# zyj0021200/simpleImageCaptionZoo

Measured on AMD Instinct MI355X. Metric: captions/sec (SCST step), BUTDDetection COCO14-size vocab, higher is better.
Workload: dtype f32

## Files before the change

### include/icz.h

```cpp
#ifndef ICZ_H_
#define ICZ_H_
#include <stddef.h>
#include <stdint.h>

#ifdef __cplusplus
extern "C" {
#endif

typedef enum {
    ICZ_OK = 0,
    ICZ_ERR_INVALID = -1,
    ICZ_ERR_HIP = -2,
    ICZ_ERR_STATE = -3,
    ICZ_ERR_NOMEM = -4
} icz_status;

const char* icz_last_error(void);
const char* icz_version(void);

typedef struct icz_butd icz_butd_t;

typedef struct {
    int32_t R;
    int32_t D;
// ... 105 lines not shown
                       const icz_rng* rng, int32_t train, float* packed_logits_out, void* stream);
int icz_nic_xe_backward(icz_nic_t* h, float smoothing, const icz_nic_params* grads, float* dfeatures_out, float* loss_out,
                        float n_tokens_global, void* stream);
int icz_nic_set_norm_global(icz_nic_t* h, const float* norm_dev, void* stream);
int icz_nic_set_option(icz_nic_t* h, const char* name, int32_t value);
int icz_nic_set_scheduled_sampling(icz_nic_t* h, float ss_prob, const float* gate_uniforms, const float* draw_uniforms);
int icz_nic_beam_search(icz_nic_t* h, const float* features, int32_t n_img, int32_t beam, int32_t max_steps, float* seqs_out,
                        int32_t* lens_out, void* stream);
int icz_nic_beam_search_opts(icz_nic_t* h, const float* features, int32_t n_img, int32_t beam, int32_t max_steps,
                             const icz_beam_opts* opts, float* seqs_out, int32_t* lens_out, float* scores_out, void* stream);
int icz_nic_beam_search_diverse(icz_nic_t* h, const float* features, int32_t n_img, int32_t beam, int32_t max_steps,
                                const icz_beam_opts* opts, const icz_beam_diversity* div, float* seqs_out, int32_t* lens_out,
                                float* scores_out, void* stream);

typedef struct icz_aoa icz_aoa_t;
typedef struct { int32_t R, D, Hd, E, V, NH, max_rows, max_len; } icz_aoa_dims;
typedef struct {
    float *q_w, *q_b, *k_w, *k_b, *v_w, *v_b, *aoa_w, *aoa_b, *ln_g, *ln_b;
} icz_aoa_block;
typedef struct {
    float *proj_w, *proj_b;
    icz_aoa_block layer[6];
    float *ref_ln_g, *ref_ln_b;
    float *lstm_w_ih, *lstm_w_hh, *lstm_b_ih, *lstm_b_hh;
    icz_aoa_block dec;
    float* embed_weight;
    float *predict_v, *predict_g, *predict_b;
} icz_aoa_params;
typedef struct {
    uint64_t seed;
    const float* uniforms;
    const uint8_t *proj_mask, *ref_att_mask, *ref_aoa_mask, *ref_sc_mask, *emb_mask, *ctx_mask, *att_mask, *out_mask;
} icz_aoa_rng;
int icz_aoa_create(const icz_aoa_dims* dims, icz_aoa_t** out);
int icz_aoa_destroy(icz_aoa_t* h);
int icz_aoa_bind_params(icz_aoa_t* h, const icz_aoa_params* params);
int icz_aoa_refresh_weights(icz_aoa_t* h, void* stream);
int icz_aoa_set_regions(icz_aoa_t* h, int32_t regions, const int32_t* counts_dev, const int32_t* counts_host, int32_t n_img);
int icz_aoa_set_option(icz_aoa_t* h, const char* name, int32_t value);
int icz_aoa_refine(icz_aoa_t* h, const float* feats, int32_t B, float* refined_out, void* stream);
int icz_aoa_greedy(icz_aoa_t* h, const float* feats, int32_t B, int32_t max_len, int64_t* ids_out, void* stream);
int icz_aoa_beam_search(icz_aoa_t* h, const float* feats, int32_t n_img, int32_t beam, int32_t max_steps, float* seqs_out,
                        int32_t* lens_out, void* stream);
int icz_aoa_beam_search_opts(icz_aoa_t* h, const float* feats, int32_t n_img, int32_t beam, int32_t max_steps,
                             const icz_beam_opts* opts, float* seqs_out, int32_t* lens_out, float* scores_out, void* stream);
int icz_aoa_beam_search_diverse(icz_aoa_t* h, const float* feats, int32_t n_img, int32_t beam, int32_t max_steps,
                                const icz_beam_opts* opts, const icz_beam_diversity* div, float* seqs_out, int32_t* lens_out,
                                float* scores_out, void* stream);
int icz_aoa_sample(icz_aoa_t* h, const float* feats, int32_t B, int32_t max_len, const icz_aoa_rng* rng, int64_t* seq_out,
                   float* logprobs_out, void* stream);
int icz_aoa_scst_rollouts(icz_aoa_t* h, const float* feats, int32_t B, int32_t max_len, const icz_aoa_rng* rng, int64_t* ids_out,
                          int64_t* seq_out, float* logprobs_out, void* stream);
int icz_aoa_sample_backward(icz_aoa_t* h, const float* reward, const icz_aoa_params* grads, float* loss_out, float* mask_sum_out,
                            float mask_sum_global, void* stream);
int icz_aoa_xe_forward(icz_aoa_t* h, const float* feats, const int64_t* captions, int32_t B, int32_t L, const int32_t* lengths_host,
                       const icz_aoa_rng* rng, int32_t train, float* packed_logits_out, void* stream);
int icz_aoa_xe_backward(icz_aoa_t* h, float smoothing, const icz_aoa_params* grads, float* loss_out, float n_tokens_global,
                        void* stream);
int icz_aoa_set_norm_global(icz_aoa_t* h, const float* norm_dev, void* stream);
int icz_aoa_set_grad_callback(icz_aoa_t* h, icz_grad_ready_cb cb, void* user);
int icz_aoa_saved_alphas(icz_aoa_t* h, float* alphas_out, void* stream);
int icz_aoa_set_scheduled_sampling(icz_aoa_t* h, float ss_prob, const float* gate_uniforms, const float* draw_uniforms);

typedef struct icz_ensemble icz_ensemble_t;
int icz_ensemble_create(const int32_t* kinds, void* const* members, const float* weights, int32_t M, icz_ensemble_t** out);
int icz_ensemble_destroy(icz_ensemble_t* h);
int icz_ensemble_greedy(icz_ensemble_t* h, const float* const* feats, int32_t B, int32_t max_len, int64_t* ids_out, void* stream);
int icz_ensemble_beam_search_diverse(icz_ensemble_t* h, const float* const* feats, int32_t n_img, int32_t beam, int32_t max_steps,
                                     const icz_beam_opts* opts, const icz_beam_diversity* div, float* seqs_out, int32_t* lens_out,
                                     float* scores_out, void* stream);
int icz_ensemble_logprob(int32_t M, const float* const* logits, const float* const* bias, const int32_t* nsplit, const int32_t* ld,
                         const float* weights, int32_t rows, int32_t V, float* lp_out, int32_t ldo, int64_t* argmax_out, void* stream);

typedef struct {
    float temperature;
    int32_t top_k;
    float top_p;
} icz_sample_opts;
int icz_sample_decode_check(const icz_sample_opts* opts, int32_t n_img, int32_t n, int32_t V, int32_t max_rows);
int icz_butd_sample_decode(icz_butd_t* h, const float* feats, int32_t n_img, int32_t n, int32_t max_len, const icz_sample_opts* opts,
                           uint64_t seed, const float* uniforms, int64_t* ids_out, float* logp_out, float* score_out, void* stream);
int icz_aoa_sample_decode(icz_aoa_t* h, const float* feats, int32_t n_img, int32_t n, int32_t max_len, const icz_sample_opts* opts,
                          uint64_t seed, const float* uniforms, int64_t* ids_out, float* logp_out, float* score_out, void* stream);
int icz_nic_sample_decode(icz_nic_t* h, const float* features, int32_t n_img, int32_t n, int32_t max_len, const icz_sample_opts* opts,
                          uint64_t seed, const float* uniforms, int64_t* ids_out, float* logp_out, float* score_out, void* stream);
int icz_sample_filter_draw(const float* logits, const float* bias, int32_t nsplit, int32_t ld, int32_t rows, int32_t V,
                           const icz_sample_opts* opts, const float* uniforms, int64_t* tok_out, float* logp_out, uint8_t* keep_out,
                           void* stream);

int icz_adam_clamp_step(float* param, const float* grad, float* exp_avg, float* exp_avg_sq, int64_t n,
                        float lr, float clip, int32_t step, void* stream);
int icz_adam_clamp_multi(int32_t count, float* const* params, const float* const* grads, float* const* exp_avg,
                         float* const* exp_avg_sq, const int64_t* numel, float lr, float clip, int32_t step, void* stream);

typedef struct icz_ciderd icz_ciderd_t;

int icz_ciderd_create(const int32_t* df_keys, const double* df_idf, int64_t cap, double default_idf,
                      const double* penalty, icz_ciderd_t** out);
int icz_ciderd_destroy(icz_ciderd_t* h);

int icz_ciderd_reward(icz_ciderd_t* h, const int64_t* gen, const int64_t* greedy, int32_t B, int32_t T,
                      const int32_t* img_ref_ptr, const int32_t* ref_ent_ptr, const int32_t* ent_key,
                      const int32_t* ent_order, const double* ent_w, const double* ref_norm,
                      const int32_t* ref_len, float* reward_out, double* scores_out, void* stream);
int icz_ciderd_cook_host(const int32_t* df_keys_host, const double* df_idf_host, int64_t cap, double default_idf,
                         const int32_t* tokens, const int32_t* ref_tok_ptr, int32_t n_refs, int64_t max_ent,
                         int32_t* ent_key_out, int32_t* ent_order_out, double* ent_w_out, int32_t* ref_ent_ptr_out,
                         double* ref_norm_out, int32_t* ref_len_out, int64_t* n_ent_out);
typedef struct icz_ciderd_vocab icz_ciderd_vocab_t;
int icz_ciderd_vocab_create(const char* words, const int64_t* word_off, const int32_t* word_id, int32_t n_words, int32_t V,
                            icz_ciderd_vocab_t** out);
int icz_ciderd_vocab_destroy(icz_ciderd_vocab_t* v);
int icz_ciderd_vocab_oov_id(icz_ciderd_vocab_t* v, const char* word, int32_t len, int32_t* id_out);
int icz_ciderd_cook_text(icz_ciderd_vocab_t* vocab, const int32_t* df_keys_host, const double* df_idf_host, int64_t cap, double default_idf,
                         const char* text, int64_t text_len, int32_t n_refs, int64_t max_ent,
                         int32_t* ent_key_out, int32_t* ent_order_out, double* ent_w_out, int32_t* ref_ent_ptr_out,
                         double* ref_norm_out, int32_t* ref_len_out, int64_t* n_ent_out);
int icz_ciderd_reward_indexed(icz_ciderd_t* h, const int64_t* gen, const int64_t* greedy, int32_t B, int32_t T,
                              const int32_t* img_slot, const int32_t* img_ref_ptr, const int32_t* ref_ent_ptr,
                              const int32_t* ent_key, const int32_t* ent_order, const double* ent_w, const double* ref_norm,
                              const int32_t* ref_len, float* reward_out, double* scores_out, void* stream);
int icz_ciderd_reward_loo(icz_ciderd_t* h, const int64_t* gen, int32_t B, int32_t K, int32_t T, const int32_t* img_slot,
                          const int32_t* img_ref_ptr, const int32_t* ref_ent_ptr, const int32_t* ent_key, const int32_t* ent_order,
                          const double* ent_w, const double* ref_norm, const int32_t* ref_len, float* reward_out, double* scores_out,
                          void* stream);

int icz_ciderd_cook_device(icz_ciderd_t* h, const int32_t* tok, const int32_t* ptr, int32_t n_cand, int32_t* ent_key_out,
                           int32_t* ent_order_out, double* ent_w_out, int32_t* ent_ptr_out, double* norm_out, int32_t* len_out, void* stream);
size_t icz_ciderd_pairwise_workspace_bytes(int32_t n_img, int32_t K);
int icz_ciderd_pairwise(icz_ciderd_t* h, const int32_t* tok, const int32_t* ptr, int32_t n_img, int32_t K, double* pair_out,
                        double* consensus_out, int32_t* best_out, void* workspace, size_t workspace_bytes, void* stream);
int icz_ciderd_scores_csr(icz_ciderd_t* h, const int32_t* tok, const int32_t* ptr, int32_t n_img, int32_t K, const int32_t* img_slot,
                          const int32_t* img_ref_ptr, const int32_t* ref_ent_ptr, const int32_t* ent_key, const int32_t* ent_order,
                          const double* ent_w, const double* ref_norm, const int32_t* ref_len, double* scores_out, void* stream);
int icz_ngram_diversity(const int32_t* tok, const int32_t* ptr, int32_t n_img, int32_t K, int32_t* counts_out, void* stream);

int icz_bleu_stats(const int32_t* hyp_tok, const int32_t* hyp_ptr, const int32_t* ref_tok, const int32_t* ref_ptr,
                   const int32_t* img_ref_ptr, int32_t n_img, int32_t* stats_out, void* stream);
int icz_rouge_lcs(const int32_t* hyp_tok, const int32_t* hyp_ptr, const int32_t* ref_tok, const int32_t* ref_ptr,
                  const int32_t* img_ref_ptr, int32_t n_img, int32_t* lcs_out, void* stream);

int icz_gemm_f32(int32_t layout, const float* X, int32_t ldx, const float* W, int32_t ldw, const float* bias,
                 float* C, int32_t ldc, int32_t M, int32_t N, int32_t K, int32_t nsplit, float* workspace,
                 size_t workspace_floats, void* stream);
size_t icz_gemm_workspace_floats(int32_t M, int32_t N);
int icz_gemm_set_big_cfg(int32_t cfg);
int icz_gemm_big_cfg_for(int32_t layout, int32_t M, int32_t N, int32_t K, int32_t nsplit);
int icz_gemm_tn_grouped(const float* dY, int32_t ldy, int32_t M, int32_t K, int32_t ngroups, const float* const* X, const int32_t* ldx,
                        const int32_t* cols, float* const* out, const int32_t* ldo, const int32_t* rows_live, void* stream);
int icz_gemm_tn_split_pick(int32_t M, int32_t N, int32_t K);
int icz_gemm_tn_split(const float* dY, int32_t ldy, int32_t M, const float* X, int32_t ldx, int32_t N, int32_t K, float* out, int32_t ldo,
                      float* workspace, size_t workspace_floats, const int32_t* rows_live, void* stream);
int icz_gemm_route_for(int32_t layout, int32_t M, int32_t N, int32_t nseg, const int32_t* K, int32_t nsplit);
int icz_gemm_tn_grouped_fits(int32_t M, int32_t K, int32_t ngroups, const int32_t* cols);
int icz_prof_begin(void);
int icz_prof_select(int32_t which);
int icz_prof_pair_overhead(void* stream, int32_t n, double* avg_us);
int icz_prof_end(double* avg_us, double* bytes_per_launch, double* flops_per_launch, long long* launches);
int icz_kprof_begin(void);
int icz_kprof_end(int32_t group, double* avg_us, long long* pairs);
int icz_prof_stream_rate(const void* buf, size_t bytes, int32_t reps, void* stream, double* gbs);

#ifdef __cplusplus
}
#endif
#endif
```

### simpleimagecaptionzoo_amd/_lib.py

```python
import ctypes as C
import os

_HERE = os.path.dirname(os.path.abspath(__file__))
LIB_PATH = os.path.join(_HERE, "libicz.so")


class IczError(RuntimeError):
    pass


GRAD_READY_CB = C.CFUNCTYPE(None, C.c_void_p, C.c_int32)


class ButdDims(C.Structure):
    _fields_ = [(n, C.c_int32) for n in ("R", "D", "H", "E", "A", "V", "max_rows", "max_len")]


BUTD_PARAM_FIELDS = (
    "embed_weight",
    "td_w_ih", "td_w_hh", "td_b_ih", "td_b_hh",
    "lm_w_ih", "lm_w_hh", "lm_b_ih", "lm_b_hh",
    "enc_att_v", "enc_att_g", "enc_att_b",
    "dec_att_v", "dec_att_g", "dec_att_b",
    "affine_v", "affine_g", "affine_b",
# ... 42 lines not shown
    _fields_ = [("p%d" % i, C.c_void_p) for i in range(len(AOA_PARAM_KEYS))]


class AoaRng(C.Structure):
    _fields_ = [("seed", C.c_uint64), ("uniforms", C.c_void_p)] + [(n, C.c_void_p) for n in (
        "proj_mask", "ref_att_mask", "ref_aoa_mask", "ref_sc_mask", "emb_mask", "ctx_mask", "att_mask", "out_mask")]


class NicParams(C.Structure):
    _fields_ = [(n, C.c_void_p) for n in NIC_PARAM_FIELDS]


class ButdParams(C.Structure):
    _fields_ = [(n, C.c_void_p) for n in BUTD_PARAM_FIELDS]


class Rng(C.Structure):
    _fields_ = [("seed", C.c_uint64), ("uniforms", C.c_void_p), ("emb_mask", C.c_void_p),
                ("att_mask", C.c_void_p), ("out_mask", C.c_void_p)]


class BeamOpts(C.Structure):
    _fields_ = [("n_best", C.c_int32), ("block_ngram", C.c_int32), ("lp_kind", C.c_int32), ("lp_alpha", C.c_float)]


class BeamDiversity(C.Structure):
    _fields_ = [("groups", C.c_int32), ("diversity", C.c_float)]


class SampleOpts(C.Structure):
    _fields_ = [("temperature", C.c_float), ("top_k", C.c_int32), ("top_p", C.c_float)]


_lib = None


def lib():
    global _lib
    if _lib is not None:
        return _lib
    if not os.path.exists(LIB_PATH):
        raise IczError("libicz.so not found at %s -- the HIP extension is required (no fallback); run "
                       "__graft_entry__.build()" % LIB_PATH)
    import torch
    L = C.CDLL(LIB_PATH)
    vp, i32, i64, f32 = C.c_void_p, C.c_int32, C.c_int64, C.c_float
    sig = {
        "icz_last_error": (C.c_char_p, []),
        "icz_version": (C.c_char_p, []),
        "icz_butd_create": (C.c_int, [C.POINTER(ButdDims), C.POINTER(vp)]),
        "icz_butd_destroy": (C.c_int, [vp]),
        "icz_butd_bind_params": (C.c_int, [vp, C.POINTER(ButdParams)]),
        "icz_butd_set_option": (C.c_int, [vp, C.c_char_p, i32]),
        "icz_butd_set_grad_callback": (C.c_int, [vp, GRAD_READY_CB, vp]),
        "icz_aoa_set_grad_callback": (C.c_int, [vp, GRAD_READY_CB, vp]),
        "icz_butd_set_mask_sum_global": (C.c_int, [vp, vp, vp]),
        "icz_butd_refresh_weights": (C.c_int, [vp, vp]),
        "icz_butd_greedy": (C.c_int, [vp, vp, i32, i32, vp, vp, vp]),
        "icz_butd_step": (C.c_int, [vp, vp, i32, vp, vp, vp, vp, vp, vp, vp, vp, vp]),
        "icz_butd_sample": (C.c_int, [vp, vp, i32, i32, C.POINTER(Rng), vp, vp, vp]),
        "icz_butd_scst_rollouts": (C.c_int, [vp, vp, i32, i32, C.POINTER(Rng), vp, vp, vp, vp]),
        "icz_butd_sample_n": (C.c_int, [vp, vp, i32, i32, i32, C.POINTER(Rng), vp, vp, vp]),
        "icz_butd_sample_backward": (C.c_int, [vp, vp, C.POINTER(ButdParams), vp, vp, f32, vp]),
        "icz_butd_sample_backward_dlogp": (C.c_int, [vp, vp, C.POINTER(ButdParams), vp]),
        "icz_butd_xe_backward_dlogits": (C.c_int, [vp, vp, C.POINTER(ButdParams), vp]),
        "icz_butd_beam_search": (C.c_int, [vp, vp, i32, i32, i32, vp, vp, vp]),
        "icz_butd_beam_search_opts": (C.c_int, [vp, vp, i32, i32, i32, C.POINTER(BeamOpts), vp, vp, vp, vp]),
        "icz_butd_beam_search_diverse": (C.c_int, [vp, vp, i32, i32, i32, C.POINTER(BeamOpts), C.POINTER(BeamDiversity), vp, vp, vp, vp]),
        "icz_butd_sample_mask_sum": (C.c_int, [vp, vp, vp]),
        "icz_butd_xe_forward": (C.c_int, [vp, vp, vp, i32, i32, C.POINTER(i32), C.POINTER(Rng), i32, vp, vp]),
        "icz_butd_xe_backward": (C.c_int, [vp, f32, C.POINTER(ButdParams), vp, f32, vp]),
        "icz_butd_set_scheduled_sampling": (C.c_int, [vp, f32, vp, vp]),
        "icz_nic_set_scheduled_sampling": (C.c_int, [vp, f32, vp, vp]),
        "icz_aoa_set_scheduled_sampling": (C.c_int, [vp, f32, vp, vp]),
        "icz_adam_clamp_step": (C.c_int, [vp, vp, vp, vp, i64, f32, f32, i32, vp]),
        "icz_nic_create": (C.c_int, [C.POINTER(NicDims), C.POINTER(vp)]),
        "icz_nic_destroy": (C.c_int, [vp]),
        "icz_nic_bind_params": (C.c_int, [vp, C.POINTER(NicParams)]),
        "icz_nic_refresh_weights": (C.c_int, [vp, vp]),
        "icz_nic_greedy": (C.c_int, [vp, vp, i32, i32, vp, vp]),
        "icz_nic_sample": (C.c_int, [vp, vp, i32, i32, C.POINTER(Rng), vp, vp, vp]),
        "icz_nic_sample_backward": (C.c_int, [vp, vp, C.POINTER(NicParams), vp, vp, vp, f32, vp]),
        "icz_nic_xe_forward": (C.c_int, [vp, vp, vp, i32, i32, C.POINTER(i32), C.POINTER(Rng), i32, vp, vp]),
        "icz_nic_xe_backward": (C.c_int, [vp, f32, C.POINTER(NicParams), vp, vp, f32, vp]),
        "icz_butd_saved_alphas": (C.c_int, [vp, vp, vp]),
        "icz_aoa_saved_alphas": (C.c_int, [vp, vp, vp]),
        "icz_nic_set_norm_global": (C.c_int, [vp, vp, vp]),
        "icz_aoa_set_norm_global": (C.c_int, [vp, vp, vp]),
        "icz_nic_beam_search": (C.c_int, [vp, vp, i32, i32, i32, vp, vp, vp]),
        "icz_nic_beam_search_opts": (C.c_int, [vp, vp, i32, i32, i32, C.POINTER(BeamOpts), vp, vp, vp, vp]),
        "icz_nic_beam_search_diverse": (C.c_int, [vp, vp, i32, i32, i32, C.POINTER(BeamOpts), C.POINTER(BeamDiversity), vp, vp, vp, vp]),
        "icz_aoa_create": (C.c_int, [C.POINTER(AoaDims), C.POINTER(vp)]),
        "icz_aoa_destroy": (C.c_int, [vp]),
        "icz_aoa_bind_params": (C.c_int, [vp, C.POINTER(AoaParams)]),
        "icz_aoa_refresh_weights": (C.c_int, [vp, vp]),
        "icz_aoa_set_regions": (C.c_int, [vp, i32, vp, vp, i32]),
        "icz_aoa_set_option": (C.c_int, [vp, C.c_char_p, i32]),
        "icz_nic_set_option": (C.c_int, [vp, C.c_char_p, i32]),
        "icz_aoa_refine": (C.c_int, [vp, vp, i32, vp, vp]),
        "icz_aoa_greedy": (C.c_int, [vp, vp, i32, i32, vp, vp]),
        "icz_aoa_beam_search": (C.c_int, [vp, vp, i32, i32, i32, vp, vp, vp]),
        "icz_aoa_beam_search_opts": (C.c_int, [vp, vp, i32, i32, i32, C.POINTER(BeamOpts), vp, vp, vp, vp]),
        "icz_aoa_beam_search_diverse": (C.c_int, [vp, vp, i32, i32, i32, C.POINTER(BeamOpts), C.POINTER(BeamDiversity), vp, vp, vp, vp]),
        "icz_ensemble_create": (C.c_int, [C.POINTER(i32), C.POINTER(vp), C.POINTER(f32), i32, C.POINTER(vp)]),
        "icz_ensemble_destroy": (C.c_int, [vp]),
        "icz_ensemble_greedy": (C.c_int, [vp, C.POINTER(vp), i32, i32, vp, vp]),
        "icz_ensemble_beam_search_diverse": (C.c_int, [vp, C.POINTER(vp), i32, i32, i32, C.POINTER(BeamOpts), C.POINTER(BeamDiversity), vp, vp,
                                                       vp, vp]),
        "icz_ensemble_logprob": (C.c_int, [i32, C.POINTER(vp), C.POINTER(vp), C.POINTER(i32), C.POINTER(i32), C.POINTER(f32), i32, i32, vp, i32,
                                           vp, vp]),
        "icz_sample_decode_check": (C.c_int, [C.POINTER(SampleOpts), i32, i32, i32, i32]),
        "icz_butd_sample_decode": (C.c_int, [vp, vp, i32, i32, i32, C.POINTER(SampleOpts), C.c_uint64, vp, vp, vp, vp, vp]),
        "icz_aoa_sample_decode": (C.c_int, [vp, vp, i32, i32, i32, C.POINTER(SampleOpts), C.c_uint64, vp, vp, vp, vp, vp]),
        "icz_nic_sample_decode": (C.c_int, [vp, vp, i32, i32, i32, C.POINTER(SampleOpts), C.c_uint64, vp, vp, vp, vp, vp]),
        "icz_sample_filter_draw": (C.c_int, [vp, vp, i32, i32, i32, i32, C.POINTER(SampleOpts), vp, vp, vp, vp, vp]),
        "icz_aoa_sample": (C.c_int, [vp, vp, i32, i32, C.POINTER(AoaRng), vp, vp, vp]),
        "icz_aoa_scst_rollouts": (C.c_int, [vp, vp, i32, i32, C.POINTER(AoaRng), vp, vp, vp, vp]),
        "icz_aoa_sample_backward": (C.c_int, [vp, vp, C.POINTER(AoaParams), vp, vp, f32, vp]),
        "icz_aoa_xe_forward": (C.c_int, [vp, vp, vp, i32, i32, C.POINTER(i32), C.POINTER(AoaRng), i32, vp, vp]),
        "icz_aoa_xe_backward": (C.c_int, [vp, f32, C.POINTER(AoaParams), vp, f32, vp]),
        "icz_ciderd_create": (C.c_int, [vp, vp, i64, C.c_double, vp, C.POINTER(vp)]),
        "icz_ciderd_destroy": (C.c_int, [vp]),
        "icz_ciderd_reward": (C.c_int, [vp, vp, vp, i32, i32, vp, vp, vp, vp, vp, vp, vp, vp, vp, vp]),
        "icz_ciderd_cook_host": (C.c_int, [vp, vp, i64, C.c_double, vp, vp, i32, i64, vp, vp, vp, vp, vp, vp, C.POINTER(i64)]),
        "icz_ciderd_vocab_create": (C.c_int, [C.c_char_p, vp, vp, i32, i32, C.POINTER(vp)]),
        "icz_ciderd_vocab_destroy": (C.c_int, [vp]),
        "icz_ciderd_vocab_oov_id": (C.c_int, [vp, C.c_char_p, i32, C.POINTER(i32)]),
        "icz_ciderd_cook_text": (C.c_int, [vp, vp, vp, i64, C.c_double, C.c_char_p, i64, i32, i64, vp, vp, vp, vp, vp, vp, C.POINTER(i64)]),
        "icz_ciderd_reward_indexed": (C.c_int, [vp, vp, vp, i32, i32, vp, vp, vp, vp, vp, vp, vp, vp, vp, vp, vp]),
        "icz_ciderd_reward_loo": (C.c_int, [vp, vp, i32, i32, i32, vp, vp, vp, vp, vp, vp, vp, vp, vp, vp, vp]),
        "icz_ciderd_cook_device": (C.c_int, [vp, vp, vp, i32, vp, vp, vp, vp, vp, vp, vp]),
        "icz_ciderd_pairwise_workspace_bytes": (C.c_size_t, [i32, i32]),
        "icz_ciderd_pairwise": (C.c_int, [vp, vp, vp, i32, i32, vp, vp, vp, vp, C.c_size_t, vp]),
        "icz_ciderd_scores_csr": (C.c_int, [vp, vp, vp, i32, i32, vp, vp, vp, vp, vp, vp, vp, vp, vp, vp]),
        "icz_ngram_diversity": (C.c_int, [vp, vp, i32, i32, vp, vp]),
        "icz_bleu_stats": (C.c_int, [vp, vp, vp, vp, vp, i32, vp, vp]),
        "icz_rouge_lcs": (C.c_int, [vp, vp, vp, vp, vp, i32, vp, vp]),
        "icz_prof_begin": (C.c_int, []),
        "icz_prof_select": (C.c_int, [i32]),
        "icz_prof_pair_overhead": (C.c_int, [vp, i32, C.POINTER(C.c_double)]),
        "icz_prof_end": (C.c_int, [C.POINTER(C.c_double), C.POINTER(C.c_double), C.POINTER(C.c_double), C.POINTER(C.c_longlong)]),
        "icz_kprof_begin": (C.c_int, []),
        "icz_kprof_end": (C.c_int, [i32, C.POINTER(C.c_double), C.POINTER(C.c_longlong)]),
        "icz_prof_stream_rate": (C.c_int, [vp, C.c_size_t, i32, vp, C.POINTER(C.c_double)]),
        "icz_adam_clamp_multi": (C.c_int, [i32, C.POINTER(vp), C.POINTER(vp), C.POINTER(vp), C.POINTER(vp), C.POINTER(i64), f32, f32, i32, vp]),
        "icz_gemm_f32": (C.c_int, [i32, vp, i32, vp, i32, vp, vp, i32, i32, i32, i32, i32, vp, C.c_size_t, vp]),
        "icz_gemm_workspace_floats": (C.c_size_t, [i32, i32]),
        "icz_gemm_set_big_cfg": (C.c_int, [i32]),
        "icz_gemm_big_cfg_for": (C.c_int, [i32, i32, i32, i32, i32]),
        "icz_gemm_tn_grouped": (C.c_int, [vp, i32, i32, i32, i32, vp, vp, vp, vp, vp, vp, vp]),
        "icz_gemm_tn_split_pick": (C.c_int, [i32, i32, i32]),
        "icz_gemm_tn_split": (C.c_int, [vp, i32, i32, vp, i32, i32, i32, vp, i32, vp, C.c_size_t, vp, vp]),
        "icz_gemm_route_for": (C.c_int, [i32, i32, i32, i32, vp, i32]),
        "icz_gemm_tn_grouped_fits": (C.c_int, [i32, i32, i32, vp]),
    }
    for name, (res, args) in sig.items():
        try:
            fn = getattr(L, name)
        except AttributeError as e:
            raise IczError("libicz.so lacks symbol %s (stale build?)" % name) from e
        fn.restype, fn.argtypes = res, args
    _lib = L
    return L


def check(status):
    if status != 0:
        raise IczError("libicz status %d: %s" % (status, lib().icz_last_error().decode()))


def ptr(t):
    return None if t is None else C.c_void_p(t.data_ptr())


def stream_ptr():
    import torch
    return C.c_void_p(torch.cuda.current_stream().cuda_stream)
```

### simpleimagecaptionzoo_amd/csrc/butd.hip

```cpp
#include <vector>

#include "butd_impl.h"

namespace icz {

int Butd::init(const icz_butd_dims& d) {
    dims = d;
    ICZ_REQUIRE(d.R > 0 && d.R <= 64, "butd: R=%d must be in 1..64 (36 boxes / 49 grid cells)", d.R);
    ICZ_REQUIRE(d.D % 4 == 0 && d.H % 4 == 0 && d.E % 4 == 0 && d.A % 4 == 0, "butd: D,H,E,A must be multiples of 4");
    ICZ_REQUIRE(d.V > 3 && d.max_rows > 0 && d.max_len > 0, "butd: bad V/max_rows/max_len");
    const size_t rows = d.max_rows, H = d.H, D = d.D, E = d.E, A = d.A, V = d.V, R = d.R;
    ICZ_TRY(alloc((void**)&w_enc, sizeof(float) * A * D));
    ICZ_TRY(alloc((void**)&w_dec, sizeof(float) * A * H));
    ICZ_TRY(alloc((void**)&w_aff, sizeof(float) * A));
    const size_t Vp = pad_vocab(d.V);
    ICZ_TRY(alloc((void**)&w_pred, sizeof(float) * Vp * H));
    ICZ_TRY(alloc((void**)&n_enc, sizeof(float) * A));
    ICZ_TRY(alloc((void**)&n_dec, sizeof(float) * A));
    ICZ_TRY(alloc((void**)&n_aff, sizeof(float) * 4));
    ICZ_TRY(alloc((void**)&n_pred, sizeof(float) * V));
    ICZ_TRY(alloc((void**)&mean, sizeof(float) * rows * D));
    ICZ_TRY(alloc((void**)&premean, sizeof(float) * rows * 4 * H));
    ICZ_TRY(alloc((void**)&enc_ctx, sizeof(float) * rows * R * A));
    for (int i = 0; i < 2; ++i) {
        ICZ_TRY(alloc((void**)&h1[i], sizeof(float) * rows * H));
        ICZ_TRY(alloc((void**)&c1[i], sizeof(float) * rows * H));
        ICZ_TRY(alloc((void**)&h2[i], sizeof(float) * rows * H));
        ICZ_TRY(alloc((void**)&c2[i], sizeof(float) * rows * H));
    }
    ICZ_TRY(alloc((void**)&emb, sizeof(float) * rows * E));
    ICZ_TRY(alloc((void**)&ctx, sizeof(float) * rows * D));
    ICZ_TRY(alloc((void**)&scores, sizeof(float) * rows * R));
    ICZ_TRY(alloc((void**)&alpha, sizeof(float) * rows * R));
    ICZ_TRY(alloc((void**)&h2drop, sizeof(float) * rows * H));
    ICZ_TRY(alloc((void**)&logits, sizeof(float) * rows * Vp));
    ICZ_TRY(alloc((void**)&amax_val, sizeof(float) * rows * ARGMAX_PARTS));
    ICZ_TRY(alloc((void**)&amax_idx, sizeof(int) * rows * ARGMAX_PARTS));
    ICZ_TRY(alloc((void**)&it, sizeof(int64_t) * rows));
    ICZ_TRY(alloc_scalars(mem));
    size_t nmax = 4 * H;
    if (A > nmax) nmax = A;
    if (V > nmax) nmax = V;
    ws_floats = (size_t)TARGET_WGS * 4096 * 2 + rows * nmax;
    {
        const size_t kmax = 2 * H + (E > D ? E : D), r128 = rows < 128 ? rows : 128;
        const size_t need = (kmax / 256 + 1) * r128 * 4 * H;
        if (need > ws_floats) ws_floats = need;
    }
    ICZ_TRY(alloc((void**)&ws, sizeof(float) * ws_floats));
    ICZ_TRY(mem.synced());
    if (const char* e = getenv("ICZ_EARLY_OUT")) early_out = atoi(e) != 0;
    if (const char* e = getenv("ICZ_MERGE_SMALL")) { const int n = atoi(e); if (n >= 0 && n <= 32) merge_small = n; }
    return ICZ_OK;
}

int Butd::refresh(hipStream_t st) {
    ICZ_REQUIRE(bound, "butd: parameters not bound");
    const int A = dims.A, D = dims.D, H = dims.H, V = dims.V;
    WeightNormTable wt = {};
    int nb = 0;
    auto add = [&](const float* v, const float* g, float* w, float* norm, int rows, int cols) {
        wt.j[wt.count++] = {v, g, w, norm, rows, cols, nb};
        nb += cdiv(rows, 4);
    };
    add(P.enc_att_v, P.enc_att_g, w_enc, n_enc, A, D);
    add(P.dec_att_v, P.dec_att_g, w_dec, n_dec, A, H);
    add(P.affine_v, P.affine_g, w_aff, n_aff, 1, A);
    add(P.predict_v, P.predict_g, w_pred, n_pred, V, H);
    hipLaunchKernelGGL(weight_norm_multi_kernel, dim3(nb), dim3(256), 0, st, wt);
    ICZ_CHECK_HIP(hipGetLastError());
    fresh = true;
    wt_fresh = false;
    return ICZ_OK;
}

bool Butd::wt_possible() const {
    GemmArgs g = {};
    g.nseg = 1;
    g.seg[0] = {w_enc, w_enc, 4 * dims.H, 4 * dims.H, 4 * dims.H, nullptr};
    g.M = 64; g.N = dims.D + dims.H;
    GemmArgs p = g, q = g;
    p.N = q.N = dims.H;
    p.nseg = 2; p.seg[1] = p.seg[0];
    return dims.H % 64 == 0 && dims.D % 64 == 0 && gemm_resident_x3_fits(g) && gemm_resident_x3_pair_fits(p, q);
}

int Butd::refresh_transposes(hipStream_t st) {
    ICZ_REQUIRE(bound && wt_lm_ih, "butd: no transposed weight buffers");
    const int H = dims.H, D = dims.D, E = dims.E;
    TransposeTable tt = {};
    int nb = 0;
    auto add = [&](const float* src, int ld, int cols, float* dst) {
        tt.j[tt.count++] = {src, ld, 4 * H, cols, dst, nb};
        nb += (4 * H / 64) * (cols / 64);
    };
    add(P.lm_w_ih, D + H, D + H, wt_lm_ih);
    add(P.lm_w_hh, H, H, wt_lm_hh);
    add(P.td_w_ih, H + D + E, H, wt_td_ih_h2);
    add(P.td_w_hh, H, H, wt_td_hh);
    hipLaunchKernelGGL(transpose_multi_kernel, dim3(nb), dim3(256), 0, st, tt);
    ICZ_CHECK_HIP(hipGetLastError());
    wt_fresh = true;
    return ICZ_OK;
}

int Butd::gemm_nt(GemmArgs& g, int* nsplit_out, hipStream_t st) {
    g.nsplit = gemm_fit_split(GEMM_NT, g, gemm_pick_split(g, TARGET_WGS), ws_floats);
    if (g.nsplit > 1) {
        ICZ_REQUIRE(gemm_slab_floats(g.M, g.N, g.nsplit) <= ws_floats, "butd: workspace too small for %dx%dx%d slabs", g.nsplit, g.M, g.N);
        g.out = ws;
        g.bias = nullptr;
    }
    *nsplit_out = g.nsplit;
    return gemm_f32(GEMM_NT, g, st);
}

int Butd::prologue(const float* feats, int n_img, hipStream_t st) {
    const int R = dims.R, D = dims.D, H = dims.H, E = dims.E, A = dims.A;
    ICZ_REQUIRE(fresh, "butd: call icz_butd_refresh_weights after binding/updating parameters");
    ICZ_REQUIRE(n_img > 0 && n_img <= dims.max_rows, "butd: %d images exceed capacity %d", n_img, dims.max_rows);
    hipLaunchKernelGGL(mean_feats_kernel, dim3(cdiv(D, 1024), n_img), dim3(256), 0, st, feats, mean, R, D);
    {
        GemmArgs g = {};
        g.nseg = 1;
        g.seg[0] = {mean, P.td_w_ih + H, D, H + D + E, D, nullptr};
        g.M = n_img; g.N = 4 * H; g.out = premean; g.ldo = 4 * H;
        int ns;
        ICZ_TRY(gemm_nt(g, &ns, st));
        if (ns > 1) {
            size_t MN = (size_t)n_img * 4 * H;
            hipLaunchKernelGGL(slab_reduce_kernel, dim3(cdiv((int)(MN / 4), 256)), dim3(256), 0, st, ws, ns, MN, 4 * H, (const float*)nullptr, premean);
        }
    }
    {
        GemmArgs g = {};
        g.nseg = 1;
        g.seg[0] = {feats, w_enc, D, D, D, nullptr};
        g.M = n_img * R; g.N = A; g.out = enc_ctx; g.ldo = A; g.bias = P.enc_att_b;
        int ns;
        const float* bias = g.bias;
        ICZ_TRY(gemm_nt(g, &ns, st));
        if (ns > 1) {
            size_t MN = (size_t)n_img * R * A;
            hipLaunchKernelGGL(slab_reduce_kernel, dim3(cdiv((int)(MN / 4), 256)), dim3(256), 0, st, ws, ns, MN, A, bias, enc_ctx);
        }
    }
    ICZ_CHECK_HIP(hipGetLastError());
    return ICZ_OK;
}

int Butd::step(const StepIO& s, hipStream_t st) {
    const int R = dims.R, D = dims.D, H = dims.H, E = dims.E, A = dims.A, V = dims.V;
    const int Vp = pad_vocab(V);
    const int rows = s.rows;
    float* const ws = s.ws_alt ? s.ws_alt : this->ws;
    float* const scores = s.scores_alt ? s.scores_alt : this->scores;
    DropCfg off = {0, nullptr, nullptr, 0, 0};
    if (!s.emb_ready)
        hipLaunchKernelGGL(embed_kernel, dim3(cdiv(E, 1024), rows), dim3(256), 0, st, P.embed_weight, s.it, s.emb_out ? s.emb_out : emb, rows, E, s.drop_emb);
    const float* embp = s.emb_out ? s.emb_out : emb;
    int ns;
    {
        GemmArgs g = {};
        g.nseg = 3;
        g.seg[0] = {s.h2_in, P.td_w_ih, H, H + D + E, H, nullptr};
        g.seg[1] = {embp, P.td_w_ih + H + D, E, H + D + E, E, nullptr};
        g.seg[2] = {s.h1_in, P.td_w_hh, H, H, H, nullptr};
        g.M = rows; g.N = 4 * H; g.out = ws; g.ldo = 4 * H;
        g.live = s.live;
        const size_t ws_cap = s.ws_alt ? (tb.xfloats < ws_floats ? tb.xfloats : ws_floats) : ws_floats;
        g.nsplit = gemm_fit_split(GEMM_NT, g, gemm_pick_split(g, STEP_WGS), ws_cap);
        ns = g.nsplit;
        ICZ_REQUIRE(gemm_slab_floats(rows, 4 * H, ns) <= ws_cap && (size_t)rows * 4 * H <= ws_cap, "butd: workspace too small");
        if (ns == 1) { g.out = ws; }
        ICZ_TRY(gemm_f32(GEMM_NT, g, st));
        LstmPointArgs a = {ws, ns, premean, s.img_of_row, P.td_b_ih, P.td_b_hh, s.c1_in, s.h1_out, s.c1_out, s.gates_td_out, nullptr, rows, H, s.live};
        kprof_mark(KP_LSTM_POINT, true, st);
        launch_lstm_point(a, off, st);
        kprof_mark(KP_LSTM_POINT, false, st);
    }
    {
        kprof_mark(KP_ATTENTION, true, st);
        GemmArgs g = {};
        g.nseg = 1;
        g.seg[0] = {s.h1_out, w_dec, H, H, H, nullptr};
        g.M = rows; g.N = A; g.out = ws; g.ldo = A;
        g.live = s.live;
        g.nsplit = gemm_pick_split(g, STEP_WGS);
        ns = g.nsplit;
        ICZ_TRY(gemm_f32(GEMM_NT, g, st));
        AttScoreArgs a = {enc_ctx, s.img_of_row, ws, ns, P.dec_att_b, w_aff, P.affine_b, s.dec_ctx_out, scores, rows, R, A, s.live};
        const int G = s.rows_per_img;
        const bool grouped = G > 1 && G <= ATT_CTX_MAX_G && rows % G == 0 && sizeof(float) * A * G <= 60 * 1024;
        if (grouped && s.drop_att.mode == 0 && !s.live)
            hipLaunchKernelGGL(att_scores_group_kernel, dim3(rows / G, ATT_PARTS), dim3(256), sizeof(float) * A * G, st, a, G);
        else if (grouped)
            hipLaunchKernelGGL(att_scores_group_train_kernel, dim3(rows / G, ATT_PARTS), dim3(256), sizeof(float) * A * G, st, a, s.drop_att, G);
        else
            hipLaunchKernelGGL(att_scores_kernel, dim3(rows, ATT_PARTS), dim3(256), sizeof(float) * A, st, a, s.drop_att);
        if (G > 1 && G <= ATT_CTX_MAX_G && rows % G == 0 && !s.alpha_out2)
            hipLaunchKernelGGL(att_ctx_group_kernel, dim3(rows / G, cdiv(D, 512)), dim3(256), 0, st, s.feats, (const float*)scores,
                               s.alpha_out ? s.alpha_out : alpha, s.ctx_out ? s.ctx_out : ctx, R, D, G, s.live);
        else
            hipLaunchKernelGGL(att_ctx_kernel, dim3(rows, cdiv(D, 512)), dim3(256), 0, st, s.feats, s.img_of_row, (const float*)scores,
                               s.alpha_out ? s.alpha_out : alpha, s.alpha_out2, s.alpha2_stride, s.ctx_out ? s.ctx_out : ctx, R, D, s.live);
        kprof_mark(KP_ATTENTION, false, st);
    }
    const float* ctxp = s.ctx_out ? s.ctx_out : ctx;
    {
        GemmArgs g = {};
        g.nseg = 3;
        g.seg[0] = {ctxp, P.lm_w_ih, D, D + H, D, nullptr};
        g.seg[1] = {s.h1_out, P.lm_w_ih + D, H, D + H, H, nullptr};
        g.seg[2] = {s.h2_in, P.lm_w_hh, H, H, H, nullptr};
        g.M = rows; g.N = 4 * H; g.out = ws; g.ldo = 4 * H;
        g.live = s.live;
        const size_t ws_cap = s.ws_alt ? (tb.xfloats < ws_floats ? tb.xfloats : ws_floats) : ws_floats;
        g.nsplit = gemm_fit_split(GEMM_NT, g, gemm_pick_split(g, STEP_WGS), ws_cap);
        ns = g.nsplit;
        ICZ_REQUIRE(gemm_slab_floats(rows, 4 * H, ns) <= ws_cap && (size_t)rows * 4 * H <= ws_cap, "butd: workspace too small");
        ICZ_TRY(gemm_f32(GEMM_NT, g, st));
        LstmPointArgs a = {ws, ns, nullptr, nullptr, P.lm_b_ih, P.lm_b_hh, s.c2_in, s.h2_out, s.c2_out, s.gates_lm_out,
                           s.h2drop_out ? s.h2drop_out : h2drop, rows, H, s.live};
        launch_lstm_point(a, s.drop_out, st);
    }
    if (!s.skip_predict) {
        const size_t ws_cap = s.ws_alt ? (tb.xfloats < ws_floats ? tb.xfloats : ws_floats) : ws_floats;
        ICZ_TRY(gemm_predict(s.h2drop_out ? s.h2drop_out : h2drop, H, w_pred, P.predict_b, rows, V, Vp, s.logits_out ? s.logits_out : logits,
                             s.logits_ld ? s.logits_ld : Vp, ws, ws_cap, s.pred_nsplit, st, s.live));
    }
    ICZ_CHECK_HIP(hipGetLastError());
    return ICZ_OK;
}

int Butd::zero_state(int rows, int which, hipStream_t st) {
    ZeroList z = {{h1[which], c1[which], h2[which], c2[which]}, 4};
    const size_t n = (size_t)rows * dims.H;
    hipLaunchKernelGGL(zero_bufs_kernel, dim3(cdiv((int)(n / 4), 256)), dim3(256), 0, st, z, n);
    return ICZ_OK;
}

int Butd::greedy(const float* feats, int B, int max_len, int64_t* ids_out, float* alphas_out, hipStream_t st) {
    ICZ_REQUIRE(feats && ids_out && B > 0 && B <= dims.max_rows && max_len > 0, "butd greedy: bad arguments");
    ICZ_REQUIRE(fresh, "butd: call icz_butd_refresh_weights after binding/updating parameters");
    if (!use_graphs) return greedy_impl(feats, B, max_len, ids_out, alphas_out, st);
    const std::vector<uintptr_t> key = {1, (uintptr_t)feats, (uintptr_t)B, (uintptr_t)max_len, (uintptr_t)ids_out, (uintptr_t)alphas_out, opt_bits()};
    return gc.run(key, st, [&](hipStream_t s) { return greedy_impl(feats, B, max_len, ids_out, alphas_out, s); });
}

int Butd::greedy_impl(const float* feats, int B, int max_len, int64_t* ids_out, float* alphas_out, hipStream_t st) {
    ICZ_TRY(prologue(feats, B, st));
    return greedy_chain(feats, B, max_len, ids_out, alphas_out, st);
}

int Butd::greedy_chain(const float* feats, int B, int max_len, int64_t* ids_out, float* alphas_out, hipStream_t st, bool scst) {
    ICZ_TRY(zero_state(B, 0, st));
    int* const gn = (scst && early_out && gnunf && tb.T >= max_len && tb.B >= B) ? gnunf : nullptr;
    hipLaunchKernelGGL(greedy_init_kernel, dim3(cdiv(B > max_len ? B : max_len, 256)), dim3(256), 0, st, it, B, gn, max_len);
    int cur = 0;
    const int Vp = pad_vocab(dims.V);
    bool track = false;
    for (int t = 0; t < max_len; ++t) {
        StepIO s = {};
        s.rows = B; s.feats = feats; s.it = it;
        s.emb_ready = t > 0;
        s.h1_in = h1[cur]; s.c1_in = c1[cur]; s.h2_in = h2[cur]; s.c2_in = c2[cur];
        s.h1_out = h1[cur ^ 1]; s.c1_out = c1[cur ^ 1]; s.h2_out = h2[cur ^ 1]; s.c2_out = c2[cur ^ 1];
        if (alphas_out) { s.alpha_out2 = alphas_out + (size_t)t * dims.R; s.alpha2_stride = max_len * dims.R; }
        int pns = 1;
        s.pred_nsplit = &pns;
        if (track && t > 0) s.live = gn + (t - 1);
        ICZ_TRY(step(s, st));
        if (t == 0) track = gn && pns > 1;
        kprof_mark(KP_GREEDY_SELECT, true, st);
        launch_greedy_select(logits_view(ws, P.predict_b, logits, B, Vp, pns), emb_slot(), B, dims.V, amax_val, amax_idx, it, ids_out, max_len, t,
                             track ? gunf : nullptr, track ? gn : nullptr, st);
        kprof_mark(KP_GREEDY_SELECT, false, st);
        cur ^= 1;
    }
    ICZ_CHECK_HIP(hipGetLastError());
    return ICZ_OK;
}

int Butd::prologue(const float* feats, int n_img, int k, const int32_t*, hipStream_t st) {
    ICZ_TRY(prologue(feats, n_img, st));
    seam_feats = feats;
    return zero_state(n_img * k, 0, st);
}

int Butd::step(int rows, const int64_t* it_, const int32_t* img_of_row, int rows_per_img, int cur, bool slabs, LogitsView* out,
               hipStream_t st) {
    StepIO s = {};
    s.rows = rows; s.feats = seam_feats; s.img_of_row = img_of_row; s.it = it_;
    s.rows_per_img = rows_per_img;
    s.emb_ready = seam_emb_ready; s.live = seam_live;
    s.h1_in = h1[cur]; s.c1_in = c1[cur]; s.h2_in = h2[cur]; s.c2_in = c2[cur];
    s.h1_out = h1[cur ^ 1]; s.c1_out = c1[cur ^ 1]; s.h2_out = h2[cur ^ 1]; s.c2_out = c2[cur ^ 1];
    int pns = 1;
    if (slabs) s.pred_nsplit = &pns;
    ICZ_TRY(step(s, st));
    if (out) *out = logits_view(ws, P.predict_b, logits, rows, pad_vocab(dims.V), pns);
    return ICZ_OK;
}

void Butd::gather(const int32_t* src_row, int rows, int fan, hipStream_t st) {
    hipLaunchKernelGGL(beam_gather_kernel, dim3(cdiv(dims.H, 1024), rows), dim3(256), 0, st, src_row, dims.H, h1[1], c1[1], h2[1], c2[1],
                       h1[0], c1[0], h2[0], c2[0], fan);
}

DecodeMember* butd_member(void* handle) { return static_cast<DecodeMember*>(reinterpret_cast<Butd*>(handle)); }

}

using namespace icz;

extern "C" {

int icz_butd_create(const icz_butd_dims* dims, icz_butd_t** out) { return abi_create<Butd>("icz_butd_create", dims, out); }

int icz_butd_destroy(icz_butd_t* h) {
    delete reinterpret_cast<Butd*>(h);
    return ICZ_OK;
}

int icz_butd_bind_params(icz_butd_t* h, const icz_butd_params* p) {
    ICZ_REQUIRE(h && p, "icz_butd_bind_params: null argument");
    ICZ_TRY(check_param_table("icz_butd_bind_params", p, sizeof(*p), (1u << 16) | (1u << 17)));
    Butd* b = reinterpret_cast<Butd*>(h);
    if (b->bound && memcmp(&b->P, p, sizeof(*p)) != 0) {
        ICZ_CHECK_HIP(hipDeviceSynchronize());
        b->gc.clear();
    }
    b->P = *p;
    b->bound = true;
    b->fresh = false;
    return ICZ_OK;
}

int icz_butd_set_option(icz_butd_t* h, const char* name, int32_t value) {
    ICZ_REQUIRE(h && name, "icz_butd_set_option: null argument");
    Butd* b = reinterpret_cast<Butd*>(h);
    if (strcmp(name, "graphs") == 0) { b->use_graphs = value != 0; return ICZ_OK; }
    if (strcmp(name, "concurrent") == 0) { b->concurrent = value != 0; return ICZ_OK; }
    if (strcmp(name, "early_out") == 0) { b->early_out = value != 0; return ICZ_OK; }
    if (strcmp(name, "small_nt") == 0) { b->small_nt = value != 0; return ICZ_OK; }
    if (strcmp(name, "group_att") == 0) { b->group_att = value != 0; return ICZ_OK; }
    if (strcmp(name, "merge_small") == 0) {
        ICZ_REQUIRE(value >= 0 && value <= 32, "icz_butd_set_option: merge_small %d outside 0..32", value);
        b->merge_small = value;
        return ICZ_OK;
    }
    set_error("icz_butd_set_option: unknown option '%s'", name);
// ... 48 lines not shown
```

### simpleimagecaptionzoo_amd/csrc/butd_kernels.h

```cpp
#pragma once
#include <stdlib.h>

#include "icz_common.h"
#include "rng.h"

namespace icz {
namespace {

__global__ __launch_bounds__(256) void weight_norm_kernel(const float* __restrict__ v, const float* __restrict__ g,
                                                          float* __restrict__ w, float* __restrict__ norm,
                                                          int rows, int cols) {
    const int lane = threadIdx.x & 63;
    const int row = blockIdx.x * 4 + (threadIdx.x >> 6);
    if (row >= rows) return;
    const float* vr = v + (size_t)row * cols;
    float ss = 0.f;
    for (int c = lane * 4; c < cols; c += 256) {
        f32x4 x = *reinterpret_cast<const f32x4*>(vr + c);
        ss += x[0] * x[0] + x[1] * x[1] + x[2] * x[2] + x[3] * x[3];
    }
    ss = wave_sum(ss);
    const float nrm = sqrtf(ss);
    const float s = g[row] / nrm;
    float* wr = w + (size_t)row * cols;
    for (int c = lane * 4; c < cols; c += 256) {
        f32x4 x = *reinterpret_cast<const f32x4*>(vr + c);
        *reinterpret_cast<f32x4*>(wr + c) = x * s;
    }
    if (lane == 0) norm[row] = nrm;
}

struct WeightNormJob { const float* v; const float* g; float* w; float* norm; int rows, cols, block0; };
struct WeightNormTable { WeightNormJob j[4]; int count; };
__global__ __launch_bounds__(256) void weight_norm_multi_kernel(WeightNormTable tab) {
    int k = 0;
#pragma unroll 1
    for (int i = 1; i < tab.count; ++i)
        if ((int)blockIdx.x >= tab.j[i].block0) k = i;
    const WeightNormJob& jb = tab.j[k];
    const int lane = threadIdx.x & 63;
    const int row = ((int)blockIdx.x - jb.block0) * 4 + (threadIdx.x >> 6);
    if (row >= jb.rows) return;
    const float* vr = jb.v + (size_t)row * jb.cols;
    float ss = 0.f;
    for (int c = lane * 4; c < jb.cols; c += 256) {
        f32x4 x = *reinterpret_cast<const f32x4*>(vr + c);
        ss += x[0] * x[0] + x[1] * x[1] + x[2] * x[2] + x[3] * x[3];
    }
    ss = wave_sum(ss);
    const float nrm = sqrtf(ss);
    const float s = jb.g[row] / nrm;
    float* wr = jb.w + (size_t)row * jb.cols;
    for (int c = lane * 4; c < jb.cols; c += 256) {
        f32x4 x = *reinterpret_cast<const f32x4*>(vr + c);
        *reinterpret_cast<f32x4*>(wr + c) = x * s;
    }
    if (lane == 0) jb.norm[row] = nrm;
}

__global__ __launch_bounds__(256) void mean_feats_kernel(const float* __restrict__ feats, float* __restrict__ mean,
                                                         int R, int D) {
    const int b = blockIdx.y;
    const int d = (blockIdx.x * 256 + threadIdx.x) * 4;
    if (d >= D) return;
    const float* f = feats + (size_t)b * R * D + d;
    f32x4 s = {0.f, 0.f, 0.f, 0.f};
    for (int r = 0; r < R; ++r) s += *reinterpret_cast<const f32x4*>(f + (size_t)r * D);
    const float fr = (float)R;
    f32x4 o = {s[0] / fr, s[1] / fr, s[2] / fr, s[3] / fr};
    *reinterpret_cast<f32x4*>(mean + (size_t)b * D + d) = o;
}

__global__ __launch_bounds__(256) void slab_reduce_kernel(const float* __restrict__ slab, int nsplit, size_t MN, int N,
                                                          const float* __restrict__ bias, float* __restrict__ out) {
    size_t i = ((size_t)blockIdx.x * 256 + threadIdx.x) * 4;
    if (i >= MN) return;
    f32x4 s = *reinterpret_cast<const f32x4*>(slab + i);
    for (int z = 1; z < nsplit; ++z) s += *reinterpret_cast<const f32x4*>(slab + (size_t)z * MN + i);
    if (bias) {
        int n = (int)(i % N);
        s += *reinterpret_cast<const f32x4*>(bias + n);
    }
    *reinterpret_cast<f32x4*>(out + i) = s;
}

__global__ __launch_bounds__(256) void embed_kernel(const float* __restrict__ table, const int64_t* __restrict__ it,
                                                    float* __restrict__ emb, int rows, int E, DropCfg dc, int relu = 1,
                                                    const int* __restrict__ live = nullptr) {
    if (step_dead(live)) return;
    const int row = blockIdx.y;
    const int e = (blockIdx.x * 256 + threadIdx.x) * 4;
    if (e >= E) return;
    f32x4 x = *reinterpret_cast<const f32x4*>(table + (size_t)it[row] * E + e);
    const int drow = row - dc.row0;
    if (drow < 0) dc.mode = 0;
    uint32_t k = dc.mode ? dc.keep4((uint64_t)drow * E + e) : 0xFu;
    const float sc = dc.mode ? 2.0f : 1.0f;
#pragma unroll
    for (int j = 0; j < 4; ++j) x[j] = ((k >> j) & 1u) ? (relu ? fmaxf(x[j], 0.f) : x[j]) * sc : 0.f;
    *reinterpret_cast<f32x4*>(emb + (size_t)row * E + e) = x;
}

constexpr int EMB_MAX_T = 128;
struct EmbRows { int n[EMB_MAX_T]; };
__global__ __launch_bounds__(256) void embed_steps_kernel(const float* __restrict__ table, const int64_t* __restrict__ tok,
                                                          float* __restrict__ emb, int B, int E, EmbRows rows, DropCfg dc) {
    const int t = blockIdx.y / B, b = blockIdx.y % B;
    if (b >= rows.n[t]) return;
    const int e = (blockIdx.x * 256 + threadIdx.x) * 4;
    if (e >= E) return;
    dc.step = (uint32_t)t;
    if (dc.mode == 1) dc.mask += (size_t)t * B * E;
    f32x4 x = *reinterpret_cast<const f32x4*>(table + (size_t)tok[blockIdx.y] * E + e);
    uint32_t k = dc.mode ? dc.keep4((uint64_t)b * E + e) : 0xFu;
    const float sc = dc.mode ? 2.0f : 1.0f;
#pragma unroll
    for (int j = 0; j < 4; ++j) x[j] = ((k >> j) & 1u) ? fmaxf(x[j], 0.f) * sc : 0.f;
    *reinterpret_cast<f32x4*>(emb + (size_t)blockIdx.y * E + e) = x;
}

struct LstmPointArgs {
    const float* slab; int nsplit;
    const float* pre; const int32_t* pre_row;
    const float* b_ih; const float* b_hh;
    const float* c_prev; float* h_out; float* c_out;
    float* gates_out;
    float* hdrop_out;
    int rows, H;
    const int* live;
};
__device__ __forceinline__ float sum_slabs1(const float* __restrict__ p, int ns, size_t stride, size_t off) {
    float s = 0.f;
    int z = 0;
    for (; z + 4 <= ns; z += 4) {
        const float a = p[(size_t)z * stride + off], b = p[(size_t)(z + 1) * stride + off];
        const float c = p[(size_t)(z + 2) * stride + off], d = p[(size_t)(z + 3) * stride + off];
        s += a; s += b; s += c; s += d;
    }
    for (; z < ns; ++z) s += p[(size_t)z * stride + off];
    return s;
}

__global__ __launch_bounds__(256) void lstm_point_kernel(LstmPointArgs a, DropCfg dc) {
    if (step_dead(a.live)) return;
    const int row = blockIdx.y;
    const int j = blockIdx.x * 256 + threadIdx.x;
    if (j >= a.H) return;
    const int H = a.H, G = 4 * H;
    const size_t MN = (size_t)a.rows * G;
    float gt[4];
    const int pr = (a.pre && a.pre_row) ? a.pre_row[row] : row;
#pragma unroll
    for (int q = 0; q < 4; ++q) {
        const size_t off = (size_t)row * G + q * H + j;
        float s = sum_slabs1(a.slab, a.nsplit, MN, off);
        if (a.pre) s += a.pre[(size_t)pr * G + q * H + j];
        s += a.b_ih[q * H + j];
        s += a.b_hh[q * H + j];
        gt[q] = s;
    }
    const float cp = a.c_prev[(size_t)row * H + j];
    const float gi = sigmoidf_(gt[0]), gf = sigmoidf_(gt[1]), gg = tanhf(gt[2]), go = sigmoidf_(gt[3]);
    const float cn = gf * cp + gi * gg;
    const float hn = go * tanhf(cn);
    a.h_out[(size_t)row * H + j] = hn;
    a.c_out[(size_t)row * H + j] = cn;
    if (a.gates_out) {
        float* go_ = a.gates_out + (size_t)row * G + j;
        go_[0] = gi; go_[H] = gf; go_[2 * H] = gg; go_[3 * H] = go;
    }
    if (a.hdrop_out) {
        float hd = hn;
        const int drow = row - dc.row0;
        if (dc.mode && drow >= 0) hd = dc.keep((uint64_t)drow * H + j) ? hn * 2.0f : 0.f;
        a.hdrop_out[(size_t)row * H + j] = hd;
    }
}

__global__ __launch_bounds__(256) void lstm_point_gw_kernel(LstmPointArgs a, DropCfg dc) {
    __shared__ __attribute__((aligned(16))) float sg[4][256];
    const int row = blockIdx.y, tid = threadIdx.x, lane = tid & 63, q = tid >> 6;
    const int H = a.H, G = 4 * H;
    const int j0 = blockIdx.x * 256, j4 = j0 + lane * 4;
    const size_t MN = (size_t)a.rows * G;
    const int lflag = live_flag(a.live);
    bool tested = false;
#define ICZ_LIVE_TEST() do { if (!tested) { if (flag_dead(lflag)) return; tested = true; } } while (0)
    if (j4 < H) {
        const size_t off = (size_t)row * G + (size_t)q * H + j4;
        const float* p = a.slab + off;
        f32x4 s = {0.f, 0.f, 0.f, 0.f};
        int z = 0;
        for (; z + 8 <= a.nsplit; z += 8) {
            f32x4 v[8];
#pragma unroll
            for (int i = 0; i < 8; ++i) v[i] = *reinterpret_cast<const f32x4*>(p + (size_t)(z + i) * MN);
            ICZ_LIVE_TEST();
#pragma unroll
            for (int i = 0; i < 8; ++i) s += v[i];
        }
        for (; z + 4 <= a.nsplit; z += 4) {
            f32x4 v[4];
#pragma unroll
            for (int i = 0; i < 4; ++i) v[i] = *reinterpret_cast<const f32x4*>(p + (size_t)(z + i) * MN);
            ICZ_LIVE_TEST();
#pragma unroll
            for (int i = 0; i < 4; ++i) s += v[i];
        }
        for (; z < a.nsplit; ++z) {
            const f32x4 v = *reinterpret_cast<const f32x4*>(p + (size_t)z * MN);
            ICZ_LIVE_TEST();
            s += v;
        }
        if (a.pre) {
            const int pr = a.pre_row ? a.pre_row[row] : row;
            s += *reinterpret_cast<const f32x4*>(a.pre + (size_t)pr * G + (size_t)q * H + j4);
        }
        s += *reinterpret_cast<const f32x4*>(a.b_ih + (size_t)q * H + j4);
        s += *reinterpret_cast<const f32x4*>(a.b_hh + (size_t)q * H + j4);
        *reinterpret_cast<f32x4*>(&sg[q][lane * 4]) = s;
    }
    ICZ_LIVE_TEST();
#undef ICZ_LIVE_TEST
    __syncthreads();
    const int j = j0 + tid;
    if (j >= H) return;
    const float cp = a.c_prev[(size_t)row * H + j];
    const float gi = sigmoidf_(sg[0][tid]), gf = sigmoidf_(sg[1][tid]), gg = tanhf(sg[2][tid]), go = sigmoidf_(sg[3][tid]);
    const float cn = gf * cp + gi * gg;
    const float hn = go * tanhf(cn);
    a.h_out[(size_t)row * H + j] = hn;
    a.c_out[(size_t)row * H + j] = cn;
    if (a.gates_out) {
        float* go_ = a.gates_out + (size_t)row * G + j;
        go_[0] = gi; go_[H] = gf; go_[2 * H] = gg; go_[3 * H] = go;
    }
    if (a.hdrop_out) {
        float hd = hn;
        const int drow = row - dc.row0;
        if (dc.mode && drow >= 0) hd = dc.keep((uint64_t)drow * H + j) ? hn * 2.0f : 0.f;
        a.hdrop_out[(size_t)row * H + j] = hd;
    }
}

inline void launch_lstm_point(const LstmPointArgs& a, const DropCfg& dc, hipStream_t st) {
    const dim3 grid(cdiv(a.H, 256), a.rows);
    if (a.H % 4 != 0) hipLaunchKernelGGL(lstm_point_kernel, grid, dim3(256), 0, st, a, dc);
    else hipLaunchKernelGGL(lstm_point_gw_kernel, grid, dim3(256), 0, st, a, dc);
}

struct AttScoreArgs {
    const float* enc_ctx;
    const int32_t* img_of_row;
    const float* dec_slab; int nsplit;
    const float* b_dec;
    const float* w_aff;
    const float* b_aff;
    float* dec_ctx_out;
    float* scores;
    int rows, R, A;
    const int* live;
};
__global__ __launch_bounds__(256) void att_scores_kernel(AttScoreArgs a, DropCfg dc) {
    extern __shared__ __attribute__((aligned(16))) float sdec[];
    const int lflag = live_flag(a.live);
    const int row = blockIdx.x, part = blockIdx.y, nparts = gridDim.y;
    const int tid = threadIdx.x, lane = tid & 63, wave = tid >> 6;
    const size_t MN = (size_t)a.rows * a.A;
    const int img = a.img_of_row ? a.img_of_row[row] : row;
    constexpr int NB = 3;
    f32x4 xf[NB][4];
    if (part + nparts * wave < a.R) {
#pragma unroll
        for (int b = 0; b < NB; ++b) {
            const int r = part + nparts * (wave + 4 * b);
            const float* e = a.enc_ctx + ((size_t)img * a.R + (r < a.R ? r : part + nparts * wave)) * a.A;
#pragma unroll
            for (int u = 0; u < 4; ++u) xf[b][u] = *reinterpret_cast<const f32x4*>(e + min(lane * 4 + 256 * u, a.A - 4));
        }
    }
    if (flag_dead(lflag)) return;
    for (int c = tid * 4; c < a.A; c += 1024) {
        const size_t off = (size_t)row * a.A + c;
        f32x4 s = *reinterpret_cast<const f32x4*>(a.dec_slab + off);
        for (int z = 1; z < a.nsplit; ++z) s += *reinterpret_cast<const f32x4*>(a.dec_slab + (size_t)z * MN + off);
        s += *reinterpret_cast<const f32x4*>(a.b_dec + c);
        *reinterpret_cast<f32x4*>(sdec + c) = s;
        if (a.dec_ctx_out && part == 0) *reinterpret_cast<f32x4*>(a.dec_ctx_out + off) = s;
    }
    __syncthreads();
    const float baff = a.b_aff[0];
    const int drow = row - dc.row0;
    if (drow < 0) dc.mode = 0;
    const float sc = dc.mode ? 2.0f : 1.0f;
    const bool shared_bits = dc.mode == 2 && (a.A & 255) == 0;
    for (int i0 = wave; part + nparts * i0 < a.R; i0 += 4 * NB) {
        int rr[NB];
        bool ok[NB];
        const float* e[NB];
        float acc[NB];
#pragma unroll
        for (int b = 0; b < NB; ++b) {
            const int r = part + nparts * (i0 + 4 * b);
            ok[b] = r < a.R;
            rr[b] = ok[b] ? r : part + nparts * i0;
            e[b] = a.enc_ctx + ((size_t)img * a.R + rr[b]) * a.A;
            acc[b] = 0.f;
        }
        for (int c0 = lane * 4; c0 < a.A; c0 += 1024) {
            f32x4 x[NB][4];
            if (i0 == wave && c0 == lane * 4) {
#pragma unroll
                for (int b = 0; b < NB; ++b)
#pragma unroll
                    for (int u = 0; u < 4; ++u) x[b][u] = xf[b][u];
            } else {
#pragma unroll
                for (int b = 0; b < NB; ++b)
#pragma unroll
                    for (int u = 0; u < 4; ++u) x[b][u] = *reinterpret_cast<const f32x4*>(e[b] + min(c0 + 256 * u, a.A - 4));
            }
            uint32_t kq[NB][4];
            if (shared_bits) {
                const int pb = lane >> 3, pg = lane & 7;
                const int pr = pb == 0 ? rr[0] : (pb == 1 ? rr[1] : rr[NB - 1]);
                const uint64_t g = (((uint64_t)drow * a.R + pr) * a.A + (c0 - lane * 4) + 128 * pg) >> 7;
                const uint64_t seed = *dc.seed_p;
                uint4_ ctr = {(uint32_t)g, (uint32_t)(g >> 32), dc.step, dc.stream};
                const uint4_ pw = philox4x32_10(ctr, (uint32_t)seed, (uint32_t)(seed >> 32));
#pragma unroll
                for (int b = 0; b < NB; ++b)
#pragma unroll
                    for (int u = 0; u < 4; ++u) {
                        const int src = 8 * b + 2 * u + (lane >> 5);
                        const uint32_t w0 = __shfl(pw.x, src), w1 = __shfl(pw.y, src), w2 = __shfl(pw.z, src), w3 = __shfl(pw.w, src);
                        const int wi = (lane >> 3) & 3;
                        const uint32_t ww = wi == 0 ? w0 : (wi == 1 ? w1 : (wi == 2 ? w2 : w3));
                        kq[b][u] = (ww >> ((4 * lane) & 31)) & 0xFu;
                    }
            }
#pragma unroll
            for (int u = 0; u < 4; ++u) {
                const int c = c0 + 256 * u;
                if (c < a.A) {
                    const f32x4 d = *reinterpret_cast<const f32x4*>(sdec + c);
                    const f32x4 w = *reinterpret_cast<const f32x4*>(a.w_aff + c);
#pragma unroll
                    for (int b = 0; b < NB; ++b) {
                        const uint32_t k = shared_bits ? kq[b][u] : (dc.mode ? dc.keep4(((uint64_t)drow * a.R + rr[b]) * a.A + c) : 0xFu);
#pragma unroll
                        for (int j = 0; j < 4; ++j) {
                            float zv = fmaxf(x[b][u][j] + d[j], 0.f);
                            zv = ((k >> j) & 1u) ? zv * sc : 0.f;
                            acc[b] += zv * w[j];
                        }
                    }
                }
            }
        }
#pragma unroll
        for (int b = 0; b < NB; ++b) {
            const float v = wave_sum(acc[b]);
            if (lane == 0 && ok[b]) a.scores[(size_t)row * a.R + rr[b]] = v + baff;
        }
    }
}

constexpr int ATT_CTX_MAX_G = 8;
__global__ __launch_bounds__(256) void att_scores_group_kernel(AttScoreArgs a, int G) {
    extern __shared__ __attribute__((aligned(16))) float sdec[];
    const int img = blockIdx.x, part = blockIdx.y, nparts = gridDim.y;
    const int tid = threadIdx.x, lane = tid & 63, wave = tid >> 6;
    const size_t MN = (size_t)a.rows * a.A;
    for (int g = 0; g < G; ++g) {
        const int row = img * G + g;
        for (int c = tid * 4; c < a.A; c += 1024) {
            const size_t off = (size_t)row * a.A + c;
            f32x4 s = *reinterpret_cast<const f32x4*>(a.dec_slab + off);
            for (int z = 1; z < a.nsplit; ++z) s += *reinterpret_cast<const f32x4*>(a.dec_slab + (size_t)z * MN + off);
            s += *reinterpret_cast<const f32x4*>(a.b_dec + c);
            *reinterpret_cast<f32x4*>(sdec + (size_t)g * a.A + c) = s;
            if (a.dec_ctx_out && part == 0) *reinterpret_cast<f32x4*>(a.dec_ctx_out + off) = s;
        }
    }
    __syncthreads();
    const float baff = a.b_aff[0];
    for (int i0 = wave; part + nparts * i0 < a.R; i0 += 4) {
        const int r = part + nparts * i0;
        const float* e = a.enc_ctx + ((size_t)img * a.R + r) * a.A;
        float acc[ATT_CTX_MAX_G];
#pragma unroll
        for (int g = 0; g < ATT_CTX_MAX_G; ++g) acc[g] = 0.f;
        for (int c0 = lane * 4; c0 < a.A; c0 += 1024) {
            f32x4 x[4];
#pragma unroll
            for (int u = 0; u < 4; ++u) x[u] = *reinterpret_cast<const f32x4*>(e + min(c0 + 256 * u, a.A - 4));
#pragma unroll
            for (int u = 0; u < 4; ++u) {
                const int c = c0 + 256 * u;
                if (c < a.A) {
                    const f32x4 w = *reinterpret_cast<const f32x4*>(a.w_aff + c);
#pragma unroll
                    for (int g = 0; g < ATT_CTX_MAX_G; ++g)
                        if (g < G) {
                            const f32x4 d = *reinterpret_cast<const f32x4*>(sdec + (size_t)g * a.A + c);
#pragma unroll
                            for (int j = 0; j < 4; ++j) acc[g] += fmaxf(x[u][j] + d[j], 0.f) * w[j];
                        }
                }
            }
        }
#pragma unroll
        for (int g = 0; g < ATT_CTX_MAX_G; ++g)
            if (g < G) {
                const float v = wave_sum(acc[g]);
                if (lane == 0) a.scores[(size_t)(img * G + g) * a.R + r] = v + baff;
            }
    }
}

__global__ __launch_bounds__(256) void att_scores_group_train_kernel(AttScoreArgs a, DropCfg dc, int G) {
    extern __shared__ __attribute__((aligned(16))) float sdec[];
    const int lflag = live_flag(a.live);
    const int img = blockIdx.x, part = blockIdx.y, nparts = gridDim.y;
    const int tid = threadIdx.x, lane = tid & 63, wave = tid >> 6;
    const size_t MN = (size_t)a.rows * a.A;
    if (flag_dead(lflag)) return;
    for (int g = 0; g < G; ++g) {
        const int row = img * G + g;
        for (int c = tid * 4; c < a.A; c += 1024) {
            const size_t off = (size_t)row * a.A + c;
            f32x4 s = *reinterpret_cast<const f32x4*>(a.dec_slab + off);
            for (int z = 1; z < a.nsplit; ++z) s += *reinterpret_cast<const f32x4*>(a.dec_slab + (size_t)z * MN + off);
            s += *reinterpret_cast<const f32x4*>(a.b_dec + c);
            *reinterpret_cast<f32x4*>(sdec + (size_t)g * a.A + c) = s;
            if (a.dec_ctx_out && part == 0) *reinterpret_cast<f32x4*>(a.dec_ctx_out + off) = s;
        }
    }
    __syncthreads();
    const float baff = a.b_aff[0];
    const float sc = dc.mode ? 2.0f : 1.0f;
    for (int i0 = wave; part + nparts * i0 < a.R; i0 += 4) {
        const int r = part + nparts * i0;
        const float* e = a.enc_ctx + ((size_t)img * a.R + r) * a.A;
        float acc[ATT_CTX_MAX_G];
#pragma unroll
        for (int g = 0; g < ATT_CTX_MAX_G; ++g) acc[g] = 0.f;
        for (int c0 = lane * 4; c0 < a.A; c0 += 1024) {
            f32x4 x[4];
#pragma unroll
            for (int u = 0; u < 4; ++u) x[u] = *reinterpret_cast<const f32x4*>(e + min(c0 + 256 * u, a.A - 4));
#pragma unroll
            for (int u = 0; u < 4; ++u) {
                const int c = c0 + 256 * u;
                if (c < a.A) {
                    const f32x4 w = *reinterpret_cast<const f32x4*>(a.w_aff + c);
#pragma unroll
                    for (int g = 0; g < ATT_CTX_MAX_G; ++g)
                        if (g < G) {
                            const f32x4 d = *reinterpret_cast<const f32x4*>(sdec + (size_t)g * a.A + c);
                            const uint64_t drow = (uint64_t)(img * G + g - dc.row0);
                            const uint32_t k = dc.mode ? dc.keep4((drow * a.R + r) * a.A + c) : 0xFu;
#pragma unroll
                            for (int j = 0; j < 4; ++j) {
                                float zv = fmaxf(x[u][j] + d[j], 0.f);
                                zv = ((k >> j) & 1u) ? zv * sc : 0.f;
                                acc[g] += zv * w[j];
                            }
                        }
                }
            }
        }
#pragma unroll
        for (int g = 0; g < ATT_CTX_MAX_G; ++g)
            if (g < G) {
                const float v = wave_sum(acc[g]);
                if (lane == 0) a.scores[(size_t)(img * G + g) * a.R + r] = v + baff;
            }
    }
}

__global__ __launch_bounds__(256) void att_ctx_kernel(const float* __restrict__ feats, const int32_t* __restrict__ img_of_row,
                                                      const float* __restrict__ scores, float* __restrict__ alpha_out,
                                                      float* __restrict__ alpha_out2, int alpha2_stride,
                                                      float* __restrict__ ctx, int R, int D, const int* __restrict__ live) {
    __shared__ float sal[64];
    __shared__ __attribute__((aligned(16))) float spart[128 * 4];
    const int lflag = live_flag(live);
    const int row = blockIdx.x, tid = threadIdx.x, lane = tid & 63;
    const int cg = tid & 127, half = tid >> 7;
    const int d = blockIdx.y * 512 + cg * 4;
    const bool valid = d < D;
    const int img = img_of_row ? img_of_row[row] : row;
    const int Rh = (R + 1) / 2;
    const int r_lo = half ? Rh : 0, r_hi = half ? R : Rh;
    const float* f = feats + (size_t)img * R * D + (valid ? d : 0);
    constexpr int RB = 9;
    f32x4 x0[RB], x1[RB];
#pragma unroll
    for (int u = 0; u < RB; ++u) x0[u] = *reinterpret_cast<const f32x4*>(f + (size_t)min(r_lo + u, r_hi - 1) * D);
#pragma unroll
    for (int u = 0; u < RB; ++u) x1[u] = *reinterpret_cast<const f32x4*>(f + (size_t)min(r_lo + RB + u, r_hi - 1) * D);
    if (flag_dead(lflag)) return;
    const float scv = lane < R ? scores[(size_t)row * R + lane] : -INFINITY;
    const float mx = wave_max(scv);
    const float ex = lane < R ? expf(scv - mx) : 0.f;
    const float sum = wave_sum(ex);
    const float al = ex / sum;
    if (tid < 64) {
        sal[tid] = al;
        if (blockIdx.y == 0 && tid < R) {
            alpha_out[(size_t)row * R + tid] = al;
            if (alpha_out2) alpha_out2[(size_t)row * alpha2_stride + tid] = al;
        }
    }
    __syncthreads();
    f32x4 acc = {0.f, 0.f, 0.f, 0.f};
    if (valid) {
#pragma unroll
        for (int u = 0; u < RB; ++u)
            if (r_lo + u < r_hi) acc += x0[u] * sal[r_lo + u];
#pragma unroll
        for (int u = 0; u < RB; ++u)
            if (r_lo + RB + u < r_hi) acc += x1[u] * sal[r_lo + RB + u];
        for (int r0 = r_lo + 2 * RB; r0 < r_hi; r0 += RB) {
            f32x4 x[RB];
#pragma unroll
            for (int u = 0; u < RB; ++u) x[u] = *reinterpret_cast<const f32x4*>(f + (size_t)min(r0 + u, r_hi - 1) * D);
#pragma unroll
            for (int u = 0; u < RB; ++u)
                if (r0 + u < r_hi) acc += x[u] * sal[r0 + u];
        }
    }
    if (half) *reinterpret_cast<f32x4*>(spart + cg * 4) = acc;
    __syncthreads();
    if (!half && valid) *reinterpret_cast<f32x4*>(ctx + (size_t)row * D + d) = acc + *reinterpret_cast<const f32x4*>(spart + cg * 4);
}

__global__ __launch_bounds__(256) void att_ctx_group_kernel(const float* __restrict__ feats, const float* __restrict__ scores,
                                                            float* __restrict__ alpha_out, float* __restrict__ ctx, int R, int D, int G,
                                                            const int* __restrict__ live) {
    __shared__ float sal[ATT_CTX_MAX_G][64];
    __shared__ __attribute__((aligned(16))) float spart[ATT_CTX_MAX_G][128 * 4];
    if (step_dead(live)) return;
    const int img = blockIdx.x, tid = threadIdx.x, lane = tid & 63, wave = tid >> 6;
    for (int g = wave; g < G; g += 4) {
        const int row = img * G + g;
        const float scv = lane < R ? scores[(size_t)row * R + lane] : -INFINITY;
        const float mx = wave_max(scv);
        const float ex = lane < R ? expf(scv - mx) : 0.f;
        const float sum = wave_sum(ex);
        const float al = ex / sum;
        sal[g][lane] = al;
        if (blockIdx.y == 0 && lane < R) alpha_out[(size_t)row * R + lane] = al;
    }
    __syncthreads();
    const int cg = tid & 127, half = tid >> 7;
    const int d = blockIdx.y * 512 + cg * 4;
    const bool valid = d < D;
    const int Rh = (R + 1) / 2;
    const int r_lo = half ? Rh : 0, r_hi = half ? R : Rh;
    const float* f = feats + (size_t)img * R * D + (valid ? d : 0);
    f32x4 acc[ATT_CTX_MAX_G];
#pragma unroll
    for (int g = 0; g < ATT_CTX_MAX_G; ++g) acc[g] = (f32x4){0.f, 0.f, 0.f, 0.f};
    if (valid) {
        constexpr int RB = 9;
        for (int r0 = r_lo; r0 < r_hi; r0 += RB) {
            f32x4 x[RB];
#pragma unroll
            for (int u = 0; u < RB; ++u) x[u] = *reinterpret_cast<const f32x4*>(f + (size_t)min(r0 + u, r_hi - 1) * D);
#pragma unroll
            for (int g = 0; g < ATT_CTX_MAX_G; ++g)
                if (g < G) {
#pragma unroll
                    for (int u = 0; u < RB; ++u)
                        if (r0 + u < r_hi) acc[g] += x[u] * sal[g][r0 + u];
                }
        }
    }
    if (half) {
#pragma unroll
        for (int g = 0; g < ATT_CTX_MAX_G; ++g)
            if (g < G) *reinterpret_cast<f32x4*>(spart[g] + cg * 4) = acc[g];
    }
    __syncthreads();
    if (!half && valid) {
#pragma unroll
        for (int g = 0; g < ATT_CTX_MAX_G; ++g)
            if (g < G) *reinterpret_cast<f32x4*>(ctx + (size_t)(img * G + g) * D + d) = acc[g] + *reinterpret_cast<const f32x4*>(spart[g] + cg * 4);
    }
}

__device__ __forceinline__ f32x4 sum_slabs4(const float* p, int ns, size_t slab_stride, size_t off) {
    f32x4 s = {0.f, 0.f, 0.f, 0.f};
    if (!p) return s;
    s = *reinterpret_cast<const f32x4*>(p + off);
    for (int z = 1; z < ns; ++z) s += *reinterpret_cast<const f32x4*>(p + (size_t)z * slab_stride + off);
    return s;
}

__device__ __forceinline__ void argmax_combine(float& best, int& bi, float ob, int oi) {
    if (ob > best || (ob == best && oi < bi)) { best = ob; bi = oi; }
}
__global__ __launch_bounds__(256) void argmax_part_kernel(const float* __restrict__ logits, int V, int ldl, int P,
                                                          float* __restrict__ part_val, int* __restrict__ part_idx,
                                                          int ns = 1, size_t slab_stride = 0, const float* __restrict__ bias = nullptr) {
    __shared__ float sv[4];
    __shared__ int si[4];
    const int row = blockIdx.x, p = blockIdx.y, tid = threadIdx.x, lane = tid & 63, wave = tid >> 6;
    const int per = ((V + P - 1) / P + 3) & ~3;
    const int v0 = p * per, v1 = min(V, v0 + per);
    const float* l = logits + (size_t)row * ldl;
    float best = -INFINITY;
    int bi = 0x7fffffff;
    if (ns > 1) {
        const bool vec = ((ldl | (int)(slab_stride & 3)) & 3) == 0 && (((uintptr_t)logits | (uintptr_t)bias) & 15) == 0;
        const int v1v = vec ? v0 + ((v1 - v0) & ~3) : v0;
        for (int v = v0 + tid * 4; v < v1v; v += 1024) {
            f32x4 x = *reinterpret_cast<const f32x4*>(l + v);
            for (int z = 1; z < ns; ++z) x += *reinterpret_cast<const f32x4*>(l + (size_t)z * slab_stride + v);
            x += *reinterpret_cast<const f32x4*>(bias + v);
#pragma unroll
            for (int j = 0; j < 4; ++j)
                if (x[j] > best) { best = x[j]; bi = v + j; }
        }
        for (int v = v1v + tid; v < v1; v += 256) {
            float x = l[v];
            for (int z = 1; z < ns; ++z) x += l[(size_t)z * slab_stride + v];
            x += bias[v];
            if (x > best || (x == best && v < bi)) { best = x; bi = v; }
        }
    } else {
        for (int v = v0 + tid; v < v1; v += 256) {
            const float x = l[v];
            if (x > best) { best = x; bi = v; }
        }
    }
#pragma unroll
    for (int o = 32; o > 0; o >>= 1) argmax_combine(best, bi, __shfl_xor(best, o, 64), __shfl_xor(bi, o, 64));
    if (lane == 0) { sv[wave] = best; si[wave] = bi; }
    __syncthreads();
    if (tid == 0) {
#pragma unroll
        for (int w = 1; w < 4; ++w) argmax_combine(best, bi, sv[w], si[w]);
        part_val[row * P + p] = best;
        part_idx[row * P + p] = bi;
    }
}
__global__ __launch_bounds__(256) void embed_argmax_kernel(const float* __restrict__ part_val, const int* __restrict__ part_idx, int P,
                                                           const float* __restrict__ table, int E, float* __restrict__ emb,
                                                           int64_t* __restrict__ it_next, int64_t* __restrict__ ids_out,
                                                           int ids_stride, int t, int relu = 1) {
    const int row = blockIdx.y;
    float best = part_val[row * P];
    int bi = part_idx[row * P];
    for (int p = 1; p < P; ++p) argmax_combine(best, bi, part_val[row * P + p], part_idx[row * P + p]);
    if (blockIdx.x == 0 && threadIdx.x == 0) {
        it_next[row] = bi;
        if (ids_out) ids_out[(size_t)row * ids_stride + t] = bi;
    }
    const int e = (blockIdx.x * 256 + threadIdx.x) * 4;
    if (e >= E) return;
    f32x4 x = *reinterpret_cast<const f32x4*>(table + (size_t)bi * E + e);
#pragma unroll
    for (int j = 0; j < 4; ++j) x[j] = relu ? fmaxf(x[j], 0.f) : x[j];
    *reinterpret_cast<f32x4*>(emb + (size_t)row * E + e) = x;
}

__global__ __launch_bounds__(1024) void greedy_select_kernel(const float* __restrict__ logits, int V, int ldl, int ns, size_t slab_stride,
                                                            const float* __restrict__ bias, const float* __restrict__ table, int E,
                                                            float* __restrict__ emb, int64_t* __restrict__ it_next,
                                                            int64_t* __restrict__ ids_out, int ids_stride, int t, int relu = 1,
                                                            uint8_t* __restrict__ unfinished = nullptr, int* __restrict__ n_unfinished = nullptr) {
    __shared__ float sv[16];
    __shared__ int si[16];
    const int row = blockIdx.x, tid = threadIdx.x, lane = tid & 63, wave = tid >> 6;
    if (n_unfinished && t > 0 && n_unfinished[t - 1] == 0) {
        if (tid == 0 && ids_out) ids_out[(size_t)row * ids_stride + t] = 0;
        return;
    }
    const float* l = logits + (size_t)row * ldl;
    float best = -INFINITY;
    int bi = 0x7fffffff;
    const bool vec = ((ldl | (int)(slab_stride & 3)) & 3) == 0 && (((uintptr_t)logits | (uintptr_t)bias) & 15) == 0;
    const int Vv = vec ? (V & ~3) : 0;
    for (int v = tid * 4; v < Vv; v += 4096) {
        f32x4 x = *reinterpret_cast<const f32x4*>(l + v);
        for (int z = 1; z < ns; ++z) x += *reinterpret_cast<const f32x4*>(l + (size_t)z * slab_stride + v);
        if (bias) x += *reinterpret_cast<const f32x4*>(bias + v);
#pragma unroll
        for (int j = 0; j < 4; ++j)
            if (x[j] > best) { best = x[j]; bi = v + j; }
    }
    for (int v = Vv + tid; v < V; v += 1024) {
        float x = l[v];
        for (int z = 1; z < ns; ++z) x += l[(size_t)z * slab_stride + v];
        if (bias) x += bias[v];
        if (x > best || (x == best && v < bi)) { best = x; bi = v; }
    }
#pragma unroll
    for (int o = 32; o > 0; o >>= 1) argmax_combine(best, bi, __shfl_xor(best, o, 64), __shfl_xor(bi, o, 64));
    if (lane == 0) { sv[wave] = best; si[wave] = bi; }
    __syncthreads();
    best = sv[0]; bi = si[0];
#pragma unroll
    for (int w = 1; w < 16; ++w) argmax_combine(best, bi, sv[w], si[w]);
    if ((unsigned)bi >= (unsigned)V) bi = 0;
    if (tid == 0) {
        it_next[row] = bi;
        if (ids_out) ids_out[(size_t)row * ids_stride + t] = bi;
        if (n_unfinished) {
            const bool unf = (t == 0 || unfinished[row] != 0) && bi != 2;
            unfinished[row] = unf ? 1 : 0;
            if (unf) atomicAdd(&n_unfinished[t], 1);
        }
    }
    for (int e = tid * 4; e < E; e += 4096) {
        f32x4 x = *reinterpret_cast<const f32x4*>(table + (size_t)bi * E + e);
#pragma unroll
        for (int j = 0; j < 4; ++j) x[j] = relu ? fmaxf(x[j], 0.f) : x[j];
        *reinterpret_cast<f32x4*>(emb + (size_t)row * E + e) = x;
    }
}

__global__ void set_scalars_kernel(uint64_t* seed_p, uint64_t seed, float* f_p, float f) {
    if (seed_p) *seed_p = seed;
    if (f_p) *f_p = f;
}

struct TransposeJob { const float* src; int ld, rows, cols; float* dst; int block0; };
struct TransposeTable { TransposeJob j[4]; int count; };
__global__ __launch_bounds__(256) void transpose_multi_kernel(TransposeTable tab) {
    __shared__ float tile[64][65];
    int ji = 0;
    for (int k = 1; k < tab.count; ++k) if ((int)blockIdx.x >= tab.j[k].block0) ji = k;
    const TransposeJob& jb = tab.j[ji];
    const int b = blockIdx.x - jb.block0, ntc = jb.cols / 64;
    const int r0 = (b / ntc) * 64, c0 = (b % ntc) * 64;
    const int tx = threadIdx.x & 15, ty = threadIdx.x >> 4;
#pragma unroll
    for (int i = 0; i < 4; ++i) {
        const int r = ty + 16 * i;
        const f32x4 v = *reinterpret_cast<const f32x4*>(jb.src + (size_t)(r0 + r) * jb.ld + c0 + 4 * tx);
#pragma unroll
        for (int e = 0; e < 4; ++e) tile[r][4 * tx + e] = v[e];
    }
    __syncthreads();
#pragma unroll
    for (int i = 0; i < 4; ++i) {
        const int c = ty + 16 * i;
        f32x4 v;
#pragma unroll
        for (int e = 0; e < 4; ++e) v[e] = tile[4 * tx + e][c];
        *reinterpret_cast<f32x4*>(jb.dst + (size_t)(c0 + c) * jb.rows + r0 + 4 * tx) = v;
    }
}

struct ZeroList { float* p[8]; int count; };
__global__ __launch_bounds__(256) void zero_bufs_kernel(ZeroList z, size_t n) {
    const size_t i = ((size_t)blockIdx.x * 256 + threadIdx.x) * 4;
    if (i >= n) return;
    const f32x4 zero = {0.f, 0.f, 0.f, 0.f};
    for (int k = 0; k < z.count; ++k) *reinterpret_cast<f32x4*>(z.p[k] + i) = zero;
}

__global__ void saved_alphas_kernel(const float* __restrict__ src, int T, int B, int NH, int R, float* __restrict__ out) {
    const int i = blockIdx.x * blockDim.x + threadIdx.x;
    if (i >= B * T * R) return;
    const int r = i % R, t = (i / R) % T, b = i / (R * T);
    const float* p = src + ((size_t)(t * B + b) * NH) * R + r;
    float s = 0.f;
    for (int h = 0; h < NH; ++h) s += p[(size_t)h * R];
    out[i] = s / (float)NH;
}

__global__ void greedy_init_kernel(int64_t* it, int rows, int* n_unfinished, int T) {
    const int i = blockIdx.x * blockDim.x + threadIdx.x;
    if (i < rows) it[i] = 1;
    if (n_unfinished && i < T) n_unfinished[i] = 0;
}
__global__ void fill_i64_kernel(int64_t* p, int64_t v, int n) {
    int i = blockIdx.x * blockDim.x + threadIdx.x;
    if (i < n) p[i] = v;
}

__global__ __launch_bounds__(256) void beam_gather_kernel(const int32_t* __restrict__ src_row, int H,
                                                          const float* __restrict__ a0, const float* __restrict__ a1,
                                                          const float* __restrict__ a2, const float* __restrict__ a3,
                                                          float* __restrict__ o0, float* __restrict__ o1,
                                                          float* __restrict__ o2, float* __restrict__ o3, int src_div) {
    const int row = blockIdx.y;
    const int j = (blockIdx.x * 256 + threadIdx.x) * 4;
    if (j >= H) return;
    const size_t s = (size_t)(src_row[row] / src_div) * H + j, d = (size_t)row * H + j;
    *reinterpret_cast<f32x4*>(o0 + d) = *reinterpret_cast<const f32x4*>(a0 + s);
    *reinterpret_cast<f32x4*>(o1 + d) = *reinterpret_cast<const f32x4*>(a1 + s);
    *reinterpret_cast<f32x4*>(o2 + d) = *reinterpret_cast<const f32x4*>(a2 + s);
    *reinterpret_cast<f32x4*>(o3 + d) = *reinterpret_cast<const f32x4*>(a3 + s);
}

__global__ __launch_bounds__(256) void beam_expand_rows_kernel(const float* __restrict__ in, const int32_t* __restrict__ img_of_row, int E,
                                                               float* __restrict__ out) {
    const int row = blockIdx.y;
    const int e = (blockIdx.x * 256 + threadIdx.x) * 4;
    if (e >= E) return;
    *reinterpret_cast<f32x4*>(out + (size_t)row * E + e) = *reinterpret_cast<const f32x4*>(in + (size_t)img_of_row[row] * E + e);
}

}
}

namespace icz {
namespace {

__device__ __forceinline__ float block_max_256(float v, float* sm) {
    v = wave_max(v);
    if ((threadIdx.x & 63) == 0) sm[threadIdx.x >> 6] = v;
    __syncthreads();
    float r = fmaxf(fmaxf(sm[0], sm[1]), fmaxf(sm[2], sm[3]));
    __syncthreads();
    return r;
}
__device__ __forceinline__ float block_sum_256(float v, float* sm) {
    v = wave_sum(v);
    if ((threadIdx.x & 63) == 0) sm[threadIdx.x >> 6] = v;
    __syncthreads();
    float r = (sm[0] + sm[1]) + (sm[2] + sm[3]);
    __syncthreads();
    return r;
}

struct SampleSelArgs {
    const float* logits; int V; int ldl;
    const float* uniforms;
    const uint64_t* seed_p; int t; int T;
    uint8_t* unfinished;
    int* n_unfinished;
    int64_t* seq_out; float* logp_out;
    int64_t* it_next;
    int32_t* draw_out;
    float* lse_out;
    const float* emb_table; float* emb_next; int E; DropCfg emb_drop;
    int ns; size_t slab_stride; const float* bias; float* logits_store;
    int* live_rows;
    int row0; int64_t* ids_out; uint8_t* g_unfinished; int* n_any;
};
constexpr int SEL_THREADS = 1024;
__device__ __forceinline__ float block_max_n(float v, float* sm, int nw) {
    v = wave_max(v);
    if ((threadIdx.x & 63) == 0) sm[threadIdx.x >> 6] = v;
    __syncthreads();
    float r = sm[0];
    for (int w = 1; w < nw; ++w) r = fmaxf(r, sm[w]);
    __syncthreads();
    return r;
}
__device__ __forceinline__ float block_sum_n(float v, float* sm, int nw) {
    v = wave_sum(v);
    if ((threadIdx.x & 63) == 0) sm[threadIdx.x >> 6] = v;
    __syncthreads();
    float r = sm[0];
    for (int w = 1; w < nw; ++w) r += sm[w];
    __syncthreads();
    return r;
}
__device__ __forceinline__ int block_inverse_cdf(const float* srow, int V, float u, double* smd, int* smi) {
    constexpr int NW = SEL_THREADS / 64;
    const int tid = threadIdx.x;
    const int per = (V + SEL_THREADS - 1) / SEL_THREADS;
    const int v0 = min(V, tid * per), v1 = min(V, v0 + per);
    double loc = 0.0;
    for (int v = v0; v < v1; ++v) loc += (double)srow[v];
    double inc = loc;
#pragma unroll
    for (int o = 1; o < 64; o <<= 1) {
        const double up = __shfl_up(inc, o, 64);
        if ((tid & 63) >= o) inc += up;
    }
    if ((tid & 63) == 63) smd[tid >> 6] = inc;
    __syncthreads();
    double wave_off = 0.0, total = 0.0;
    for (int w = 0; w < NW; ++w) {
        if (w < (tid >> 6)) wave_off += smd[w];
        total += smd[w];
    }
    const double prefix = wave_off + inc - loc;
    const double target = (double)u * total;
    int cand = 0x7fffffff;
    {
        double run = prefix;
        for (int v = v0; v < v1; ++v) {
            run += (double)srow[v];
            if (run > target) { cand = v; break; }
        }
    }
#pragma unroll
    for (int o = 32; o > 0; o >>= 1) cand = min(cand, __shfl_xor(cand, o, 64));
    if ((tid & 63) == 0) smi[tid >> 6] = cand;
    __syncthreads();
    int d = 0;
    if (tid == 0) {
        d = smi[0];
        for (int w = 1; w < NW; ++w) d = min(d, smi[w]);
        if (d > V - 1) d = V - 1;
    }
    return d;
}

struct SsSelArgs {
    const float* logits_prev;
    int ldl, V, t;
    float ss_prob;
    const float* gate;
    const float* draw;
    const uint64_t* seed_p;
    int64_t* tok;
};
__global__ __launch_bounds__(SEL_THREADS) void ss_select_kernel(SsSelArgs a) {
    extern __shared__ __attribute__((aligned(16))) float srow[];
    __shared__ float smf[16];
    __shared__ double smd[16];
    __shared__ int smi[16];
    constexpr int NW = SEL_THREADS / 64;
    const int row = blockIdx.x, tid = threadIdx.x;
    const float g = a.gate ? a.gate[row] : rng_uniform(*a.seed_p, (uint32_t)a.t, (uint64_t)row, RNG_SS_GATE);
    if (!(g < a.ss_prob)) return;
    const float* l = a.logits_prev + (size_t)row * a.ldl;
    float mx = -INFINITY;
    for (int v = tid; v < a.V; v += SEL_THREADS) { const float x = l[v]; srow[v] = x; mx = fmaxf(mx, x); }
    mx = block_max_n(mx, smf, NW);
    float se = 0.f;
    for (int v = tid; v < a.V; v += SEL_THREADS) { const float e = expf(srow[v] - mx); srow[v] = e; se += e; }
    se = block_sum_n(se, smf, NW);
    for (int v = tid; v < a.V; v += SEL_THREADS) srow[v] = srow[v] / se;
    __syncthreads();
    const float u = a.draw ? a.draw[row] : rng_uniform(*a.seed_p, (uint32_t)a.t, (uint64_t)row, RNG_SS_DRAW);
    const int d = block_inverse_cdf(srow, a.V, u, smd, smi);
    if (tid == 0) a.tok[row] = d;
}
inline int ss_select_launch(hipStream_t st, int rows, const float* logits_prev, int ldl, int V, int t, int B, float ss_prob,
                            const float* gate, const float* draw, const uint64_t* seed_p, int64_t* tok_t) {
    static bool lds_set = false;
    if (!lds_set) {
        ICZ_CHECK_HIP(hipFuncSetAttribute(reinterpret_cast<const void*>(ss_select_kernel), hipFuncAttributeMaxDynamicSharedMemorySize, 160 * 1024 - 1024));
        lds_set = true;
    }
    ICZ_REQUIRE(sizeof(float) * (size_t)V <= 159 * 1024, "scheduled sampling: a row of %d logits does not fit in LDS", V);
    SsSelArgs sa = {};
    sa.logits_prev = logits_prev; sa.ldl = ldl; sa.V = V; sa.t = t; sa.ss_prob = ss_prob;
    sa.gate = gate ? gate + (size_t)t * B : nullptr;
    sa.draw = draw ? draw + (size_t)t * B : nullptr;
    sa.seed_p = seed_p; sa.tok = tok_t;
    hipLaunchKernelGGL(ss_select_kernel, dim3(rows), dim3(SEL_THREADS), sizeof(float) * V, st, sa);
    return ICZ_OK;
}
template <bool MG>
__global__ __launch_bounds__(SEL_THREADS) void sample_select_kernel(SampleSelArgs a) {
    extern __shared__ __attribute__((aligned(16))) float srow[];
    __shared__ float smf[16];
    __shared__ double smd[16];
    __shared__ int smi[16];
    constexpr int NW = SEL_THREADS / 64;
    const int row = blockIdx.x, tid = threadIdx.x, lane = tid & 63, wave = tid >> 6;
    const int sr = MG ? row - a.row0 : row;
    const bool greedy_row = MG && sr < 0;
    const float sc = a.emb_drop.mode ? 2.0f : 1.0f;
    const int* const gate = MG ? a.n_any : a.n_unfinished;
    const bool all_dead = a.t > 0 && gate[a.t - 1] == 0;
    if (all_dead || (MG && !greedy_row && a.t > 0 && a.n_unfinished[a.t - 1] == 0)) {
        if (tid == 0) {
            if (greedy_row) a.ids_out[(size_t)row * a.T + a.t] = 0;
            else { a.seq_out[(size_t)sr * a.T + a.t] = 0; a.logp_out[(size_t)sr * a.T + a.t] = 0.f; }
            a.it_next[row] = 0;
            a.draw_out[row] = -1;
            a.lse_out[row] = 0.f;
        }
        if (MG && !all_dead && a.emb_next)
            for (int e = tid * 4; e < a.E; e += 4 * SEL_THREADS) {
                f32x4 x = *reinterpret_cast<const f32x4*>(a.emb_table + e);
#pragma unroll
                for (int j = 0; j < 4; ++j) x[j] = fmaxf(x[j], 0.f);
                *reinterpret_cast<f32x4*>(a.emb_next + (size_t)row * a.E + e) = x;
            }
        return;
    }
    if (a.live_rows && sr == 0 && tid == 0) *a.live_rows = (a.t + 1) * (int)gridDim.x;
    const float* l = a.logits + (size_t)row * a.ldl;
    const float u = greedy_row ? 0.f : (a.uniforms ? a.uniforms[sr] : rng_uniform(*a.seed_p, (uint32_t)a.t, (uint64_t)sr));
    const bool was_unf = greedy_row ? (a.t == 0 || a.g_unfinished[row] != 0) : a.unfinished[sr] != 0;
    float mx = -INFINITY;
    if (a.ns > 1) {
        float* ls = a.logits_store + (size_t)row * a.ldl;
        const bool vec = ((a.ldl | (int)(a.slab_stride & 3)) & 3) == 0 &&
                         (((uintptr_t)a.logits | (uintptr_t)a.bias | (uintptr_t)a.logits_store) & 15) == 0;
        const int Vv = vec ? (a.V & ~3) : 0;
        for (int v = tid * 4; v < Vv; v += 4 * SEL_THREADS) {
            f32x4 x = *reinterpret_cast<const f32x4*>(l + v);
            for (int z = 1; z < a.ns; ++z) x += *reinterpret_cast<const f32x4*>(l + (size_t)z * a.slab_stride + v);
            x += *reinterpret_cast<const f32x4*>(a.bias + v);
            *reinterpret_cast<f32x4*>(ls + v) = x;
            *reinterpret_cast<f32x4*>(srow + v) = x;
            mx = fmaxf(mx, fmaxf(fmaxf(x[0], x[1]), fmaxf(x[2], x[3])));
        }
        for (int v = Vv + tid; v < a.V; v += SEL_THREADS) {
            float x = l[v];
            for (int z = 1; z < a.ns; ++z) x += l[(size_t)z * a.slab_stride + v];
            x += a.bias[v];
            ls[v] = x; srow[v] = x; mx = fmaxf(mx, x);
        }
    } else {
        for (int v = tid; v < a.V; v += SEL_THREADS) { const float x = l[v]; srow[v] = x; mx = fmaxf(mx, x); }
    }
    mx = block_max_n(mx, smf, NW);
    if (greedy_row) {
        const int per = (a.V + SEL_THREADS - 1) / SEL_THREADS;
        const int v0 = min(a.V, tid * per), v1 = min(a.V, v0 + per);
        int cand = 0x7fffffff;
        for (int v = v0; v < v1; ++v)
            if (srow[v] == mx) { cand = v; break; }
#pragma unroll
        for (int o = 32; o > 0; o >>= 1) cand = min(cand, __shfl_xor(cand, o, 64));
        if (lane == 0) smi[wave] = cand;
        __syncthreads();
        int bi = smi[0];
#pragma unroll
        for (int w = 1; w < NW; ++w) bi = min(bi, smi[w]);
        if ((unsigned)bi >= (unsigned)a.V) bi = 0;
        if (tid == 0) {
            const bool unf = was_unf && bi != 2;
            a.g_unfinished[row] = unf ? 1 : 0;
            a.ids_out[(size_t)row * a.T + a.t] = bi;
            a.it_next[row] = bi;
            a.draw_out[row] = -1;
            a.lse_out[row] = 0.f;
            if (unf) atomicAdd(&a.n_any[a.t], 1);
        }
        if (a.emb_next)
            for (int e = tid * 4; e < a.E; e += 4 * SEL_THREADS) {
                f32x4 x = *reinterpret_cast<const f32x4*>(a.emb_table + (size_t)bi * a.E + e);
#pragma unroll
                for (int j = 0; j < 4; ++j) x[j] = fmaxf(x[j], 0.f);
                *reinterpret_cast<f32x4*>(a.emb_next + (size_t)row * a.E + e) = x;
            }
        return;
    }
    const int per = (a.V + SEL_THREADS - 1) / SEL_THREADS;
    const int v0 = min(a.V, tid * per), v1 = min(a.V, v0 + per);
    float se = 0.f;
    for (int v = v0; v < v1; ++v) se += expf(srow[v] - mx);
    se = block_sum_n(se, smf, NW);
    const float lse = logf(se);
    double loc = 0.0;
    for (int v = v0; v < v1; ++v) loc += (double)expf((srow[v] - mx) - lse);
    double inc = loc;
#pragma unroll
    for (int o = 1; o < 64; o <<= 1) {
        const double up = __shfl_up(inc, o, 64);
        if (lane >= o) inc += up;
    }
    if (lane == 63) smd[wave] = inc;
    __syncthreads();
    double wave_off = 0.0, total = 0.0;
#pragma unroll
    for (int w = 0; w < NW; ++w) {
        const double t = smd[w];
        if (w < wave) wave_off += t;
        total += t;
    }
    const double target = (double)u * total;
    int cand = 0x7fffffff;
    {
        const double prev = __shfl_up(inc, 1, 64);
        double run = wave_off + (lane ? prev : 0.0);
        if (run <= target && wave_off + inc > target) {
            cand = v1 - 1;
            for (int v = v0; v < v1 - 1; ++v) {
                run += (double)expf((srow[v] - mx) - lse);
                if (run > target) { cand = v; break; }
            }
        }
    }
#pragma unroll
    for (int o = 32; o > 0; o >>= 1) cand = min(cand, __shfl_xor(cand, o, 64));
    if (lane == 0) smi[wave] = cand;
    __syncthreads();
    int tok = 0;
    {
        int d = smi[0];
#pragma unroll
        for (int w = 1; w < NW; ++w) d = min(d, smi[w]);
        if (d > a.V - 1) d = a.V - 1;
        const bool unf = was_unf && (d != 2);
        tok = unf ? d : 0;
        if (tid == 0) {
            a.unfinished[sr] = unf ? 1 : 0;
            a.seq_out[(size_t)sr * a.T + a.t] = tok;
            a.logp_out[(size_t)sr * a.T + a.t] = (srow[d] - mx) - lse;
            a.it_next[row] = tok;
            a.draw_out[row] = d;
            a.lse_out[row] = mx + lse;
            if (unf) {
                atomicAdd(&a.n_unfinished[a.t], 1);
                if (MG) atomicAdd(&a.n_any[a.t], 1);
            }
        }
    }
    if (a.emb_next)
        for (int e = tid * 4; e < a.E; e += 4 * SEL_THREADS) {
            f32x4 x = *reinterpret_cast<const f32x4*>(a.emb_table + (size_t)tok * a.E + e);
            const uint32_t k = a.emb_drop.mode ? a.emb_drop.keep4((uint64_t)sr * a.E + e) : 0xFu;
#pragma unroll
            for (int j = 0; j < 4; ++j) x[j] = ((k >> j) & 1u) ? fmaxf(x[j], 0.f) * sc : 0.f;
            *reinterpret_cast<f32x4*>(a.emb_next + (size_t)row * a.E + e) = x;
        }
}
inline void launch_sample_select(hipStream_t st, int rows, const SampleSelArgs& a) {
    if (a.row0 > 0) hipLaunchKernelGGL(sample_select_kernel<true>, dim3(rows), dim3(SEL_THREADS), sizeof(float) * a.V, st, a);
    else hipLaunchKernelGGL(sample_select_kernel<false>, dim3(rows), dim3(SEL_THREADS), sizeof(float) * a.V, st, a);
}

__global__ __launch_bounds__(256) void reinforce_loss_kernel(const float* __restrict__ logp, const int64_t* __restrict__ seq,
                                                             const float* __restrict__ reward, int B, int T,
                                                             const float* __restrict__ mask_sum_global_p, float* __restrict__ coef,
                                                             float* __restrict__ loss_out, float* __restrict__ mask_sum_out) {
    __shared__ float smf[4];
    const int tid = threadIdx.x;
    float ms = 0.f, ls = 0.f;
    for (int i = tid; i < B * T; i += 256) {
        const int t = i % T;
        const float m = (t == 0) ? 1.f : (seq[i - 1] > 0 ? 1.f : 0.f);
        ms += m;
        ls += -logp[i] * reward[i] * m;
    }
    ms = block_sum_256(ms, smf);
    ls = block_sum_256(ls, smf);
    const float msg = mask_sum_global_p ? mask_sum_global_p[0] : 0.f;
    const float denom = msg > 0.f ? msg : ms;
    for (int i = tid; i < B * T; i += 256) {
        const int t = i % T;
        const float m = (t == 0) ? 1.f : (seq[i - 1] > 0 ? 1.f : 0.f);
        coef[i] = -reward[i] * m / denom;
    }
    if (tid == 0) {
        if (loss_out) loss_out[0] = ls / denom;
        if (mask_sum_out) mask_sum_out[0] = ms;
    }
}

__global__ __launch_bounds__(256) void reinforce_dlogits_kernel(float* __restrict__ logits, int V, int ldl,
                                                                const int32_t* __restrict__ draw, const float* __restrict__ lse,
                                                                const float* __restrict__ coef, int B, int T, int Bs = 0, int row0 = 0) {
    const int row = blockIdx.y;
    const int v = blockIdx.x * 256 + threadIdx.x;
    if (v >= ldl) return;
    const int stride = Bs > 0 ? Bs : B;
    const int t = row / stride, b = row % stride - row0;
    float* l = logits + (size_t)row * ldl;
    const float c = b >= 0 ? coef[(size_t)b * T + t] : 0.f;
    const int d = draw[row];
    float g = 0.f;
    if (v < V && d >= 0 && c != 0.f) g = c * ((v == d ? 1.f : 0.f) - expf(l[v] - lse[row]));
    l[v] = g;
}

constexpr int XE_MAX_T = 128;
struct XeRows { int n[XE_MAX_T]; };
__global__ __launch_bounds__(256) void xe_loss_dlogits_kernel(float* __restrict__ logits, int V, int ldl,
                                                              const int64_t* __restrict__ captions, int L, int B, XeRows rows,
                                                              float smoothing, float inv_n_host, const float* __restrict__ n_dev,
                                                              float* __restrict__ loss_rows) {
    __shared__ float smf[4];
    const int b = blockIdx.x, t = blockIdx.y, tid = threadIdx.x;
    if (b >= rows.n[t]) {
        float* z = logits + (size_t)(t * B + b) * ldl;
        for (int v = tid; v < ldl; v += 256) z[v] = 0.f;
        return;
    }
    const float inv_n = (n_dev && n_dev[0] > 0.f) ? 1.0f / n_dev[0] : inv_n_host;
    const int row = t * B + b;
    float* l = logits + (size_t)row * ldl;
    float mx = -INFINITY;
    for (int v = tid; v < V; v += 256) mx = fmaxf(mx, l[v]);
    mx = block_max_256(mx, smf);
    float se = 0.f;
    for (int v = tid; v < V; v += 256) se += expf(l[v] - mx);
    se = block_sum_256(se, smf);
    const float lse = mx + logf(se);
    const int tg = (int)captions[(size_t)b * L + t + 1];
    const float conf = 1.f - smoothing, low = smoothing / (float)(V - 1);
    const float lconf = conf > 0.f ? logf(conf) : 0.f, llow = low > 0.f ? logf(low) : 0.f;
    float ls = 0.f;
    for (int v = tid; v < ldl; v += 256) {
        float g = 0.f;
        if (v < V) {
            const float lp = l[v] - lse;
            const float tr = (v == tg) ? conf : low;
            if (tr > 0.f) ls += tr * (((v == tg) ? lconf : llow) - lp);
            g = (expf(lp) - tr) * inv_n;
        }
        l[v] = g;
    }
    ls = block_sum_256(ls, smf);
    if (tid == 0) loss_rows[row] = ls;
}

__global__ __launch_bounds__(256) void sum_scale_kernel(const float* __restrict__ x, int n, float scale_host, const float* __restrict__ n_dev,
                                                        float* __restrict__ out) {
    __shared__ float smf[4];
    const float scale = (n_dev && n_dev[0] > 0.f) ? 1.0f / n_dev[0] : scale_host;
    float s = 0.f;
    for (int i = threadIdx.x; i < n; i += 256) s += x[i];
    s = block_sum_256(s, smf);
    if (threadIdx.x == 0) out[0] = s * scale;
}

struct LstmBwdArgs {
    const float* dh_a; int ns_a;
    int lda_a;
    const float* dh_b; int ns_b; int lda_b;
    const float* dh_c; int ns_c; int lda_c;
    const float* dhdrop;
    const float* dc_in;
    const float* gates;
    const float* c_prev;
    const float* c_cur;
    float* dgates;
    float* dc_prev;
    int rows, H;
    int rows_a, rows_b, rows_c;
    int dc_in_rows;
    const int* live;
    const int* carry_live;
};
__global__ __launch_bounds__(256) void lstm_bwd_point_kernel(LstmBwdArgs a, DropCfg dc) {
    const int row = blockIdx.y;
    const int j = blockIdx.x * 256 + threadIdx.x;
    if (j >= a.H) return;
    const int H = a.H, G = 4 * H;
    const int lflag = live_flag(a.live), cflag = live_flag(a.carry_live);
    const float* g = a.gates + (size_t)row * G + j;
    const float gi = g[0], gf = g[H], gg = g[2 * H], go = g[3 * H];
    const float cc = a.c_cur[(size_t)row * H + j];
    const float cp = a.c_prev ? a.c_prev[(size_t)row * H + j] : 0.f;
    float dhd = 0.f;
    if (a.dhdrop) dhd = a.dhdrop[(size_t)row * H + j];
    if (flag_dead(lflag)) {
        float* o = a.dgates + (size_t)row * G + j;
        o[0] = 0.f; o[H] = 0.f; o[2 * H] = 0.f; o[3 * H] = 0.f;
        return;
    }
    const bool carry = cflag != 0;
    float dh = 0.f;
    if (a.dh_a && carry && row < a.rows_a) dh += sum_slabs1(a.dh_a, a.ns_a, (size_t)a.rows_a * a.lda_a, (size_t)row * a.lda_a + j);
    if (a.dh_b && row < a.rows_b) dh += sum_slabs1(a.dh_b, a.ns_b, (size_t)a.rows_b * a.lda_b, (size_t)row * a.lda_b + j);
    if (a.dh_c && row < a.rows_c) dh += sum_slabs1(a.dh_c, a.ns_c, (size_t)a.rows_c * a.lda_c, (size_t)row * a.lda_c + j);
    if (a.dhdrop) {
        float d = dhd;
        if (dc.mode) d = dc.keep((uint64_t)row * H + j) ? d * 2.0f : 0.f;
        dh += d;
    }
    const float dcin = (a.dc_in && carry && row < a.dc_in_rows) ? a.dc_in[(size_t)row * H + j] : 0.f;
    const float tc = tanhf(cc);
    const float dcv = dcin + dh * go * (1.f - tc * tc);
    float* o = a.dgates + (size_t)row * G + j;
    o[0] = dcv * gg * gi * (1.f - gi);
    o[H] = dcv * cp * gf * (1.f - gf);
    o[2 * H] = dcv * gi * (1.f - gg * gg);
    o[3 * H] = dh * tc * go * (1.f - go);
    a.dc_prev[(size_t)row * H + j] = dcv * gf;
}

// ... 644 lines not shown
```

### simpleimagecaptionzoo_amd/csrc/decoder_core.hip

```cpp
#include <stdarg.h>

#include "decoder_core.h"

namespace icz {

static thread_local char g_err[1024] = "";
void set_error(const char* fmt, ...) {
    va_list ap;
    va_start(ap, fmt);
    vsnprintf(g_err, sizeof(g_err), fmt, ap);
    va_end(ap);
}

__global__ void captions_to_tok_kernel(const int64_t* __restrict__ cap, int B, int L, int T, int64_t* __restrict__ tok) {
    int i = blockIdx.x * blockDim.x + threadIdx.x;
    if (i >= T * B) return;
    int t = i / B, b = i % B;
    tok[i] = cap[(size_t)b * L + t];
}
__global__ void gather_packed_kernel(const float* __restrict__ logit, int V, int ldl, int B, const int* __restrict__ row_off,
                                     const int* __restrict__ rows_t, int T, float* __restrict__ out) {
    const int tb_ = blockIdx.y, t = tb_ / B, b = tb_ % B;
    if (b >= rows_t[t]) return;
    const int v = blockIdx.x * 256 + threadIdx.x;
    if (v >= V) return;
    out[(size_t)(row_off[t] + b) * V + v] = logit[(size_t)tb_ * ldl + v];
}
__global__ void scatter_packed_kernel(const float* __restrict__ dpacked, int V, int ldl, int B, const int* __restrict__ row_off,
                                      const int* __restrict__ rows_t, int T, float* __restrict__ logit) {
    const int tb_ = blockIdx.y, t = tb_ / B, b = tb_ % B;
    const int v = blockIdx.x * 256 + threadIdx.x;
    if (v >= ldl) return;
    float g = 0.f;
    if (b < rows_t[t] && v < V) g = dpacked[(size_t)(row_off[t] + b) * V + v];
    logit[(size_t)tb_ * ldl + v] = g;
}

int CaptionHead::alloc_scalars(DeviceBuffers& m) {
    ICZ_TRY(m.alloc((void**)&d_seed, 16));
    return m.alloc((void**)&d_msum, 16);
}

int CaptionHead::alloc_loss_buffers(DeviceBuffers& m, size_t TB, size_t B, size_t T) {
    ICZ_TRY(m.alloc((void**)&coef, sizeof(float) * TB));
    ICZ_TRY(m.alloc((void**)&lse, sizeof(float) * TB));
    ICZ_TRY(m.alloc((void**)&loss_rows, sizeof(float) * TB));
    ICZ_TRY(m.alloc((void**)&draw, sizeof(int32_t) * TB));
    ICZ_TRY(m.alloc((void**)&unf, B));
    ICZ_TRY(m.alloc((void**)&nunf, sizeof(int) * T));
    ICZ_TRY(m.alloc((void**)&gunf, B));
    ICZ_TRY(m.alloc((void**)&gnunf, sizeof(int) * T));
    ICZ_TRY(m.alloc((void**)&live_rows, 16));
    ICZ_TRY(m.alloc((void**)&pack_idx, sizeof(int) * 2 * T));
    pack_cap = (int)(2 * T);
    return ICZ_OK;
}

void CaptionHead::drop_loss_buffers() {
    coef = lse = loss_rows = nullptr; draw = nullptr; unf = gunf = nullptr; nunf = gnunf = live_rows = pack_idx = nullptr;
    pack_cap = 0;
    mode = 0;
}

int CaptionHead::require_mode(int want, const char* who) const {
    ICZ_REQUIRE(mode == want, want == 1 ? "%s: no rollout stored (call icz_%s_sample first)" : "%s: no XE forward stored (call icz_%s_xe_forward first)",
                who, who);
    return ICZ_OK;
}

int CaptionHead::xe_steps(const char* who, const int32_t* lengths, int B, int L, int* T_out) {
    int T = 0;
    for (int b = 0; b < B; ++b) {
        ICZ_REQUIRE(lengths[b] >= 1 && lengths[b] <= L - 1, "%s xe_forward: length %d out of range 1..%d", who, lengths[b], L - 1);
        ICZ_REQUIRE(b == 0 || lengths[b] <= lengths[b - 1], "%s xe_forward: lengths must be sorted in decreasing order (Engine.py:179)", who);
        if (lengths[b] > T) T = lengths[b];
    }
    *T_out = T;
    return ICZ_OK;
}

void CaptionHead::begin_xe(const int32_t* lengths, int B, int T, int L, const int64_t* captions, bool train, uint64_t seed, hipStream_t st) {
    hipLaunchKernelGGL(set_scalars_kernel, dim3(1), dim3(1), 0, st, d_seed, seed, (float*)nullptr, 0.f);
    mode = 2; cur_B = B; cur_T = T; cur_L = L; cur_train = train; cur_captions = captions;
    rows_t.assign(T, 0);
    n_tokens = 0;
    for (int t = 0; t < T; ++t) {
        int c = 0;
        for (int b = 0; b < B; ++b) c += lengths[b] > t;
        rows_t[t] = c;
        n_tokens += c;
    }
}

void CaptionHead::captions_to_tok(int64_t* tok, hipStream_t st) const {
    hipLaunchKernelGGL(captions_to_tok_kernel, dim3(cdiv(cur_T * cur_B, 256)), dim3(256), 0, st, cur_captions, cur_B, cur_L, cur_T, tok);
}

int CaptionHead::upload_pack_index(hipStream_t st) {
    const int T = cur_T;
    std::vector<int> hostv(2 * T);
    int acc = 0;
    for (int t = 0; t < T; ++t) { hostv[t] = acc; hostv[T + t] = rows_t[t]; acc += rows_t[t]; }
    ICZ_REQUIRE(pack_idx && 2 * T <= pack_cap, "pack index capacity");
    ICZ_CHECK_HIP(hipMemcpyAsync(pack_idx, hostv.data(), sizeof(int) * 2 * T, hipMemcpyHostToDevice, st));
    ICZ_CHECK_HIP(hipStreamSynchronize(st));
    return ICZ_OK;
}

int CaptionHead::gather_packed(const float* logit, int V, int ldl, float* packed_out, hipStream_t st) {
    ICZ_TRY(upload_pack_index(st));
    const int T = cur_T;
    hipLaunchKernelGGL(gather_packed_kernel, dim3(cdiv(V, 256), T * cur_B), dim3(256), 0, st, logit, V, ldl, cur_B, pack_idx, pack_idx + T, T,
                       packed_out);
    return ICZ_OK;
}

int CaptionHead::scatter_packed(const float* dpacked, int V, int ldl, float* logit, hipStream_t st) {
    ICZ_TRY(upload_pack_index(st));
    const int T = cur_T;
    hipLaunchKernelGGL(scatter_packed_kernel, dim3(cdiv(ldl, 256), T * cur_B), dim3(256), 0, st, dpacked, V, ldl, cur_B, pack_idx, pack_idx + T, T,
                       logit);
    ICZ_CHECK_HIP(hipGetLastError());
    return ICZ_OK;
}

int CaptionHead::xe_loss(float smoothing, float n_tokens_global, float* logits, int V, int ldl, float* loss_out, hipStream_t st) {
    const int B = cur_B, T = cur_T;
    const float n = n_tokens_global > 0.f ? n_tokens_global : (float)n_tokens;
    const float* n_dev = n_tokens_global < 0.f ? d_msum : nullptr;
    ICZ_CHECK_HIP(hipMemsetAsync(loss_rows, 0, sizeof(float) * T * B, st));
    ICZ_REQUIRE(T <= XE_MAX_T, "xe_backward: %d steps exceed %d", T, XE_MAX_T);
    XeRows xr = {};
    for (int t = 0; t < T; ++t) xr.n[t] = rows_t[t];
    hipLaunchKernelGGL(xe_loss_dlogits_kernel, dim3(B, T), dim3(256), 0, st, logits, V, ldl, cur_captions, cur_L, B, xr, smoothing, 1.0f / n, n_dev,
                       loss_rows);
    if (loss_out) hipLaunchKernelGGL(sum_scale_kernel, dim3(1), dim3(256), 0, st, loss_rows, T * B, 1.0f / n, n_dev, loss_out);
    ICZ_CHECK_HIP(hipGetLastError());
    mode = 0;
    return ICZ_OK;
}

void CaptionHead::set_msum_global(float msum_global, hipStream_t st) const {
    if (msum_global >= 0.f)
        hipLaunchKernelGGL(set_scalars_kernel, dim3(1), dim3(1), 0, st, (uint64_t*)nullptr, (uint64_t)0, d_msum, msum_global);
}

int CaptionHead::reinforce(const float* reward, float* logits, int V, int ldl, float* loss_out, float* msum_out, hipStream_t st, int rows, int row0) {
    const int B = cur_B, T = cur_T;
    hipLaunchKernelGGL(reinforce_loss_kernel, dim3(1), dim3(256), 0, st, cur_logp, cur_seq, reward, B, T, (const float*)d_msum, coef, loss_out, msum_out);
    hipLaunchKernelGGL(reinforce_dlogits_kernel, dim3(cdiv(ldl, 256), T * (rows ? rows : B)), dim3(256), 0, st, logits, V, ldl, draw, lse, coef, B, T,
                       rows, row0);
    ICZ_CHECK_HIP(hipGetLastError());
    return ICZ_OK;
}

void launch_greedy_select(const LogitsView& lv, const DecodeMember::EmbSlot& e, int rows, int V, float* amax_val, int* amax_idx, int64_t* it,
                          int64_t* ids_out, int T, int t, uint8_t* gunf, int* gn, hipStream_t st) {
    if (lv.ns > 1)
        hipLaunchKernelGGL(greedy_select_kernel, dim3(rows), dim3(1024), 0, st, lv.p, V, lv.ld, lv.ns, lv.slab_stride, lv.bias, e.table, e.E, e.emb,
                           it, ids_out, T, t, e.relu, gunf, gn);
    else {
        hipLaunchKernelGGL(argmax_part_kernel, dim3(rows, ARGMAX_PARTS), dim3(256), 0, st, lv.p, V, lv.ld, ARGMAX_PARTS, amax_val, amax_idx);
        hipLaunchKernelGGL(embed_argmax_kernel, dim3(cdiv(e.E, 1024), rows), dim3(256), 0, st, (const float*)amax_val, (const int*)amax_idx,
                           ARGMAX_PARTS, e.table, e.E, e.emb, it, ids_out, T, t, e.relu);
    }
}

int check_param_table(const char* who, const void* params, size_t bytes, uint32_t unaligned_ok) {
    const float* const* q = reinterpret_cast<const float* const*>(params);
    for (size_t i = 0; i < bytes / sizeof(float*); ++i) {
        ICZ_REQUIRE(q[i] != nullptr, "%s: parameter pointer %zu is null", who, i);
        ICZ_REQUIRE(((uintptr_t)q[i] & 15) == 0 || ((unaligned_ok >> i) & 1), "%s: parameter %zu not 16-byte aligned", who, i);
    }
    return ICZ_OK;
}

int set_scheduled_sampling(const char* who, CaptionHead* h, float ss_prob, const float* gate, const float* draw) {
    ICZ_REQUIRE(h, "%s: null handle", who);
    ICZ_REQUIRE(ss_prob >= 0.f && ss_prob <= 1.f, "%s: ss_prob %g outside [0, 1]", who, (double)ss_prob);
    h->ss_prob = ss_prob; h->ss_gate = gate; h->ss_draw = draw;
    return ICZ_OK;
}

int set_norm_global(const char* who, CaptionHead* h, const float* norm_dev, void* stream) {
    ICZ_REQUIRE(h && norm_dev, "%s: null argument", who);
    ICZ_CHECK_HIP(hipMemcpyAsync(h->d_msum, norm_dev, sizeof(float), hipMemcpyDeviceToDevice, (hipStream_t)stream));
    return ICZ_OK;
}

}

extern "C" {
const char* icz_last_error(void) { return icz::g_err; }
const char* icz_version(void) { return "libicz 0.1 (gfx950)"; }
}
```

### simpleimagecaptionzoo_amd/csrc/gemm_f32.h

```cpp
#pragma once
#include "icz_common.h"

namespace icz {

constexpr int GEMM_MAX_SEG = 4;
constexpr int GEMM_BM = 64, GEMM_BN = 64, GEMM_BK = 64;

enum GemmLayout { GEMM_NT = 0, GEMM_NN = 1, GEMM_TN = 2 };

struct GemmSeg {
    const float* A;
    const float* B;
    int lda, ldb;
    int K;
    const int64_t* gather;
};

struct GemmArgs {
    GemmSeg seg[GEMM_MAX_SEG];
    int nseg;
    int M, N;
    float* out;
    int ldo;
    const float* bias;
    int nsplit;
    int chunks_per_split;
    int accumulate;
    int spread;
    const int* live;
    const int* rows_live;
};

int gemm_f32(GemmLayout layout, const GemmArgs& a, hipStream_t stream);
int gemm_route(GemmLayout layout, const GemmArgs& a);
int gemm_pick_split(const GemmArgs& a, int target_wgs, GemmLayout layout = GEMM_NT);
int gemm_pick_split_balanced(const GemmArgs& a, GemmLayout layout, size_t slab_capacity_floats);
size_t gemm_slab_floats(int M, int N, int nsplit);
int gemm_normalize_split(GemmLayout layout, const GemmArgs& a, int nsplit);
int gemm_fit_split(GemmLayout layout, const GemmArgs& a, int nsplit, size_t capacity_floats);

bool gemm_resident_x3_fits(const GemmArgs& a);
int gemm_resident_x3_stages(const GemmArgs& a);
int gemm_resident_x3_nsplit(const GemmArgs& a);
int gemm_resident_x3(const GemmArgs& a, hipStream_t stream);
bool gemm_resident_x3_pair_fits(const GemmArgs& a, const GemmArgs& b);
int gemm_resident_x3_pair(const GemmArgs& a, const GemmArgs& b, hipStream_t stream);
int gemm_predict(const float* x, int H, const float* w_pred, const float* bias, int rows, int V, int Vp, float* logits, int ldl,
                 float* ws, size_t ws_cap_floats, int* pred_nsplit, hipStream_t st, const int* live = nullptr);

int gemm_big_x3(GemmLayout layout, const GemmArgs& a, int cfg, hipStream_t stream);
int gemm_big_cfg(GemmLayout layout, const GemmArgs& a);
int gemm_big_switch();
void gemm_set_big_cfg(int cfg);
constexpr int GEMM_MAX_COLGROUPS = 4;
struct GemmColGroup { const float* B; int ldb; int cols; float* out; int ldo; };
bool gemm_tn_grouped_fits(int M, int K, const GemmColGroup* groups, int ngroups);
int gemm_tn_grouped(const float* dY, int ldy, int M, int K, const GemmColGroup* groups, int ngroups, const int* rows_live, hipStream_t stream);

int gemm_tn_split_pick(int M, int N, int K);
int gemm_tn_split(const float* dY, int ldy, int M, const float* X, int ldx, int N, int K, int nsplit, float* slabs, const int* rows_live, hipStream_t st);
struct GemmSwitches { bool tn_x3, nn_x3, nt_x3big, resident_x3, resident_m128, predict_slabs, resident_k512; unsigned prof_every; int big_cfg; };
const GemmSwitches& gemm_switches();

}
```

### simpleimagecaptionzoo_amd/csrc/gemm_f32.hip

```cpp
#include <stdlib.h>

#include <array>
#include <mutex>
#include <set>
#include <vector>

#include "gemm_f32.h"
#include "butd_kernels.h"

namespace icz {

static int total_chunks(const GemmArgs& a, int bk = GEMM_BK) {
    int t = 0;
    for (int s = 0; s < a.nseg; ++s) t += cdiv(a.seg[s].K, bk);
    return t;
}

template <int BK>
struct ChunkCursorT {
    int seg, k0;
    const float* A; const float* B;
    int lda, ldb, K;
    __device__ __forceinline__ void load_seg(const GemmArgs& a) {
        const GemmSeg& g = a.seg[seg];
// ... 694 lines not shown
        if (nst > 1) load_stage(ar1, br1);
        __syncthreads();
        auto iter = [&](int st, float (&arF)[IPT][8], float (&brF)[IPT][8], const float (&arN)[IPT][8], const float (&brN)[IPT][8]) {
            if (st + 2 < nst) load_stage(arF, brF);
            __builtin_amdgcn_sched_barrier(0);
            compute(NBUF == 2 ? (st & 1) : 0);
            if (NBUF == 1) __syncthreads();
            if (st + 1 < nst) store_stage(NBUF == 2 ? ((st + 1) & 1) : 0, arN, brN);
            __syncthreads();
        };
        int st = 0;
        for (; st + 2 <= nst; st += 2) {
            iter(st, ar0, br0, ar1, br1);
            iter(st + 1, ar1, br1, ar0, br0);
        }
        if (st < nst) iter(st, ar0, br0, ar1, br1);
    };
    if (a.nseg == 1) {
        const int kbeg = a.nsplit > 1 ? (int)blockIdx.z * a.chunks_per_split * 128 : 0;
        int kend = a.nsplit > 1 ? min(a.seg[0].K, kbeg + a.chunks_per_split * 128) : a.seg[0].K;
        if (!AROW && !BROW) kend = min(kend, rows_live);
        run_segment(a.seg[0], kbeg, kend);
    } else {
        const int gbeg = a.nsplit > 1 ? (int)blockIdx.z * a.chunks_per_split * 128 : 0;
        const int gend = a.nsplit > 1 ? gbeg + a.chunks_per_split * 128 : 0x7fffffff;
        int off = 0;
#pragma unroll 1
        for (int sgi = 0; sgi < a.nseg; ++sgi) {
            const int K = a.seg[sgi].K;
            const int kb = max(gbeg - off, 0), ke = min(gend - off, K);
            if (kb < ke) run_segment(a.seg[sgi], kb, ke);
            off += K;
        }
    }
    const bool direct = a.nsplit == 1;
    float* const outp = direct ? a.out : a.out + (size_t)blockIdx.z * a.M * a.N;
    const int ldo = direct ? a.ldo : a.N;
#pragma unroll
    for (int i = 0; i < 2; ++i)
#pragma unroll
        for (int u = 0; u < NU; ++u) {
            const int n = n0 + nbase + 32 * u + r;
            if (n >= a.N) continue;
            const float bias_n = (direct && a.bias) ? a.bias[n] : 0.f;
#pragma unroll
            for (int q = 0; q < 16; ++q) {
                const int m = m0 + mbase + 32 * i + (q & 3) + 8 * (q >> 2) + 4 * h;
                if (m < a.M) {
                    float* o = outp + (size_t)m * ldo + n;
                    const float v = acc[i][u][q] + bias_n;
                    *o = (direct && a.accumulate) ? (*o + v) : v;
                }
            }
        }
}

struct GemmProf {
    bool on = false;
    std::vector<hipEvent_t> ev;
    size_t used = 0;
    double bytes = 0.0, flops = 0.0;
    unsigned seen = 0, every = 1;
    int select = 0;
};
static GemmProf g_prof;
static thread_local bool g_capturing = false;
void gemm_set_capturing(bool on) { g_capturing = on; }

struct KProf { bool on = false; std::vector<hipEvent_t> ev[KP_GROUPS]; size_t used[KP_GROUPS] = {}; };
static KProf g_kprof;
void kprof_mark(int group, bool begin, hipStream_t st) {
    if (!g_kprof.on || g_capturing || group < 0 || group >= KP_GROUPS) return;
    std::vector<hipEvent_t>& ev = g_kprof.ev[group];
    size_t& u = g_kprof.used[group];
    if (begin) {
        if (u + 2 > ev.size()) {
            if (ev.size() >= 8192) return;
            hipEvent_t a = nullptr, b = nullptr;
            if (hipEventCreate(&a) != hipSuccess || hipEventCreate(&b) != hipSuccess) return;
            ev.push_back(a); ev.push_back(b);
        }
        (void)hipEventRecord(ev[u], st);
    } else if (u + 2 <= ev.size()) {
        (void)hipEventRecord(ev[u + 1], st);
        u += 2;
    }
}

static void prof_account(const GemmArgs& a) {
    double kb = 0.0, k = 0.0;
    for (int s = 0; s < a.nseg; ++s) { k += a.seg[s].K; }
    kb = ((double)a.M * k + (double)a.N * k + (double)a.M * a.N) * 4.0;
    g_prof.bytes += kb;
    g_prof.flops += 2.0 * a.M * a.N * k;
}

size_t gemm_slab_floats(int M, int N, int nsplit) { return nsplit > 1 ? (size_t)nsplit * M * N : 0; }

const GemmSwitches& gemm_switches() {
    static const GemmSwitches sw = [] {
        auto on = [](const char* name) { const char* e = getenv(name); return e ? atoi(e) != 0 : true; };
        GemmSwitches s;
        s.tn_x3 = on("ICZ_GEMM_TN_X3"); s.nn_x3 = on("ICZ_GEMM_NN_X3"); s.nt_x3big = on("ICZ_GEMM_NT_X3BIG");
        s.resident_x3 = on("ICZ_GEMM_RESIDENT_X3"); s.resident_m128 = on("ICZ_GEMM_RESIDENT_M128"); s.predict_slabs = on("ICZ_PREDICT_SLABS");
        s.resident_k512 = on("ICZ_GEMM_RESIDENT_K512");
        const char* e = getenv("ICZ_PROF_EVERY");
        s.prof_every = e && atoi(e) > 1 ? (unsigned)atoi(e) : 1u;
        const char* b = getenv("ICZ_GEMM_BIG");
        s.big_cfg = b ? atoi(b) : -1;
        return s;
    }();
    return sw;
}

static int g_big_override = -2;
void gemm_set_big_cfg(int cfg) { g_big_override = cfg; }
int gemm_big_switch() { return g_big_override != -2 ? g_big_override : gemm_switches().big_cfg; }

static int nt_stage_k(const GemmArgs& a) {
    if (gemm_resident_x3_fits(a)) return 64;
    if (a.M <= 32) return 64;
    for (int s = 0; s < a.nseg; ++s)
        if (a.seg[s].K % 128) return 64;
    return 128;
}
static int nn_stage_k(const GemmArgs& a) {
    for (int s = 0; s < a.nseg; ++s)
        if (a.seg[s].K % 128) return 64;
    return 128;
}
static bool nn_x3(const GemmArgs& a) {
    return gemm_switches().nn_x3 && a.nseg == 1 && a.M >= 128 && a.N >= 128 && a.seg[0].K % 128 == 0 && !a.bias && a.N % 4 == 0;
}
static int stage_k(GemmLayout layout, const GemmArgs& a) {
    return layout == GEMM_NT ? nt_stage_k(a) : (layout == GEMM_NN ? nn_stage_k(a) : GEMM_BK);
}

static bool nt_spread(const GemmArgs& a) { return a.M <= 64 || a.M >= 1024; }
static bool nt_x3big(const GemmArgs& a) {
    if (!gemm_switches().nt_x3big || a.M < 128 || a.N < 128 || gemm_resident_x3_fits(a)) return false;
    for (int s = 0; s < a.nseg; ++s)
        if (a.seg[s].K % 128) return false;
    const int tiles = cdiv(a.N, 128) * cdiv(a.M, 128);
    if (a.nseg == 1) {
        if (tiles * (a.seg[0].K / 512 > 0 ? a.seg[0].K / 512 : 1) >= 128) return true;
        return a.M >= 256 && tiles * (a.seg[0].K / 256) >= 64;
    }
    int tot = 0;
    for (int s = 0; s < a.nseg; ++s) tot += a.seg[s].K / 128;
    const int per = (a.M >= 256 && tiles < 128) ? 4 : 8;
    return tiles * (tot / per > 0 ? tot / per : 1) >= 128;
}
static int nt_tile_n(const GemmArgs& a) { return 64; }

int gemm_pick_split(const GemmArgs& a, int target_wgs, GemmLayout layout) {
    if (layout == GEMM_NT && gemm_resident_x3_fits(a)) return gemm_resident_x3_nsplit(a);
    if (layout == GEMM_NT && nt_x3big(a)) {
        const int tiles = cdiv(a.N, 128) * cdiv(a.M, 128);
        if (a.nseg > 1) {
            int tot = 0;
            for (int sg = 0; sg < a.nseg; ++sg) tot += a.seg[sg].K / 128;
            int s = 512 / (tiles > 0 ? tiles : 1);
            const int per = (a.M >= 256 && tiles < 128) ? 4 : 8;
            if (s > tot / per) s = tot / per;
            if (s < 1) s = 1;
            return cdiv(tot, cdiv(tot, s));
        }
        const int tot = a.seg[0].K / 128;
        int s = 896 / tiles;
        if (s > tot / 5) s = tot / 5;
        if (tiles < 128 && tot >= 4) s = (tot / 2 < 320 / tiles) ? tot / 2 : 320 / tiles;
        if (s < 1) s = 1;
        return cdiv(tot, cdiv(tot, s));
    }
    int tiles = cdiv(a.N, layout == GEMM_NT ? nt_tile_n(a) : GEMM_BN) * cdiv(a.M, GEMM_BM);
    int tot = total_chunks(a, stage_k(layout, a));
    int s = target_wgs / (tiles > 0 ? tiles : 1);
    if (s < 1) s = 1;
    if (s > tot) s = tot;
    if (s > 32) s = 32;
    int cps = cdiv(tot, s);
    return cdiv(tot, cps);
}

int gemm_pick_split_balanced(const GemmArgs& a, GemmLayout layout, size_t slab_capacity_floats) {
    if (layout == GEMM_NN && nn_x3(a)) {
        const int tiles = cdiv(a.N, 128) * cdiv(a.M, 128), tot = a.seg[0].K / 128;
        GemmArgs probe = a;
        probe.nsplit = 1;
        int s = (gemm_big_cfg(GEMM_NN, probe) == 4 ? 768 : 512) / (tiles > 0 ? tiles : 1);
        if (s > tot / 8) s = tot / 8;
        if (s < 1) s = 1;
        while (s > 1 && (size_t)s * a.M * a.N > slab_capacity_floats) --s;
        return cdiv(tot, cdiv(tot, s));
    }
    const int bk = stage_k(layout, a);
    const int tiles = cdiv(a.N, layout == GEMM_NT ? nt_tile_n(a) : GEMM_BN) * cdiv(a.M, GEMM_BM);
    const int tot = total_chunks(a, bk);
    const double fixed = 2.4 * 128.0 / bk;
    int best = 1;
    double best_cost = 1e30;
    for (int s = 1; s <= 32 && s <= tot; ++s) {
        const int cps = cdiv(tot, s);
        if (cdiv(tot, cps) != s) continue;
        if (s > 1 && (size_t)s * a.M * a.N > slab_capacity_floats) break;
        const int rounds = cdiv(tiles * s, 256);
        const double cost = rounds * (cps + fixed) + (s > 1 ? 0.25 * s : 0.0);
        if (cost < best_cost - 1e-9) { best_cost = cost; best = s; }
    }
    return best;
}

int gemm_fit_split(GemmLayout layout, const GemmArgs& a, int nsplit, size_t capacity_floats) {
    nsplit = gemm_normalize_split(layout, a, nsplit);
    while (nsplit > 1 && gemm_slab_floats(a.M, a.N, nsplit) > capacity_floats) nsplit = gemm_normalize_split(layout, a, nsplit - 1);
    return nsplit;
}
int gemm_normalize_split(GemmLayout layout, const GemmArgs& a, int nsplit) {
    const int tot = total_chunks(a, stage_k(layout, a));
    if (nsplit < 1) nsplit = 1;
    if (nsplit > tot) nsplit = tot;
    return cdiv(tot, cdiv(tot, nsplit));
}

static int check_args(GemmLayout layout, const GemmArgs& a) {
    ICZ_REQUIRE(a.nseg >= 1 && a.nseg <= GEMM_MAX_SEG, "gemm: nseg %d out of range", a.nseg);
    ICZ_REQUIRE(a.M > 0 && a.N > 0 && a.out, "gemm: bad M/N/out");
    ICZ_REQUIRE(a.nsplit >= 1, "gemm: nsplit %d", a.nsplit);
    ICZ_REQUIRE(a.nsplit == 1 || (!a.bias && !a.accumulate), "gemm: bias/accumulate need nsplit == 1");
    for (int s = 0; s < a.nseg; ++s) {
        const GemmSeg& g = a.seg[s];
        ICZ_REQUIRE(g.A && g.B && g.K > 0, "gemm: segment %d null operand or K<=0", s);
        ICZ_REQUIRE(((uintptr_t)g.A & 15) == 0 && ((uintptr_t)g.B & 15) == 0, "gemm: segment %d operands must be 16-byte aligned", s);
        ICZ_REQUIRE(g.lda % 4 == 0 && g.ldb % 4 == 0, "gemm: segment %d leading dims must be multiples of 4 (lda %d ldb %d)", s, g.lda, g.ldb);
        ICZ_REQUIRE(!g.gather, "gemm: row gather is not supported");
        if (layout == GEMM_NT) {
            ICZ_REQUIRE(g.K % 4 == 0, "gemm NT: segment %d K=%d must be a multiple of 4", s, g.K);
        } else if (layout == GEMM_NN) {
            ICZ_REQUIRE(g.K % 4 == 0 && a.N % 4 == 0, "gemm NN: K and N must be multiples of 4 (K %d N %d)", g.K, a.N);
            ICZ_REQUIRE(!g.gather, "gemm NN: gather unsupported");
        } else {
            ICZ_REQUIRE(a.M % 4 == 0 && a.N % 4 == 0, "gemm TN: M and N must be multiples of 4 (M %d N %d)", a.M, a.N);
            ICZ_REQUIRE(!g.gather, "gemm TN: gather unsupported");
        }
    }
    if (layout != GEMM_NT && a.nsplit == 1) {
        ICZ_REQUIRE(a.ldo % 4 == 0 && ((uintptr_t)a.out & 15) == 0, "gemm: output must be float4-aligned");
    }
    return ICZ_OK;
}

static void log_big_shape(GemmLayout layout, const GemmArgs& a) {
    static const bool on = [] { const char* e = getenv("ICZ_GEMM_LOG"); return e && atoi(e) > 0; }();
    if (!on) return;
    static std::mutex mu;
    static std::set<std::array<int, 6>> seen;
    int K = 0;
    for (int s = 0; s < a.nseg; ++s) K += a.seg[s].K;
    std::lock_guard<std::mutex> lk(mu);
    if (seen.insert({(int)layout, a.M, a.N, K, a.nseg, a.nsplit}).second)
        fprintf(stderr, "[icz gemm] %s M=%d N=%d K=%d nseg=%d nsplit=%d rows_live=%d\n", layout == GEMM_NT ? "nt" : (layout == GEMM_NN ? "nn" : "tn"), a.M, a.N, K, a.nseg, a.nsplit, a.rows_live ? 1 : 0);
}

int gemm_f32(GemmLayout layout, const GemmArgs& a_in, hipStream_t stream) {
    GemmArgs a = a_in;
    ICZ_TRY(check_args(layout, a));
    int tot = total_chunks(a, stage_k(layout, a));
    a.chunks_per_split = cdiv(tot, a.nsplit);
    ICZ_REQUIRE(cdiv(tot, a.chunks_per_split) == a.nsplit, "gemm: nsplit %d leaves empty splits (chunks %d)", a.nsplit, tot);
    dim3 block(256);
    bool tail = false;
    for (int s = 0; s < a.nseg; ++s) tail |= (a.seg[s].K % GEMM_BK) != 0;
    if (layout == GEMM_NT) {
        if (nt_x3big(a)) {
            static bool attr = false;
            if (!attr) {
                ICZ_CHECK_HIP(hipFuncSetAttribute(reinterpret_cast<const void*>(gemm_tn128_x3_kernel<1, 4, true, true>), hipFuncAttributeMaxDynamicSharedMemorySize, (int)t3_lds(1)));
                ICZ_CHECK_HIP(hipFuncSetAttribute(reinterpret_cast<const void*>(gemm_tn128_x3_kernel<2, 8, true, true>), hipFuncAttributeMaxDynamicSharedMemorySize, (int)t3_lds(2)));
                attr = true;
            }
            const dim3 g128(cdiv(a.N, 128), cdiv(a.M, 128), a.nsplit);
            log_big_shape(layout, a);
            if (const int bc = gemm_big_cfg(layout, a)) return gemm_big_x3(layout, a, bc, stream);
            if ((int)(g128.x * g128.y * g128.z) > 256) hipLaunchKernelGGL((gemm_tn128_x3_kernel<1, 4, true, true>), g128, block, t3_lds(1), stream, a);
            else hipLaunchKernelGGL((gemm_tn128_x3_kernel<2, 8, true, true>), g128, dim3(512), t3_lds(2), stream, a);
            ICZ_CHECK_HIP(hipGetLastError());
            return ICZ_OK;
        }
        int mt = a.M <= 16 ? 1 : (a.M <= 32 ? 2 : 4);
        const int bn = nt_tile_n(a);
        dim3 grid(cdiv(a.N, bn), cdiv(a.M, mt * 16), a.nsplit);
        hipEvent_t e0 = nullptr, e1 = nullptr;
        const bool resident = gemm_resident_x3_fits(a) && a.nsplit == gemm_resident_x3_nsplit(a) && a.chunks_per_split == gemm_resident_x3_stages(a);
        if (g_prof.on && (g_prof.select == 1 ? resident : (mt == 4 || resident)) && (g_prof.seen++ % g_prof.every) == 0) {
            if (g_prof.used + 2 <= g_prof.ev.size()) {
                e0 = g_prof.ev[g_prof.used]; e1 = g_prof.ev[g_prof.used + 1];
                g_prof.used += 2;
                prof_account(a);
                (void)hipEventRecord(e0, stream);
            }
        }
#define ICZ_NT(MT_, NTW_, BK_) do { if (tail) hipLaunchKernelGGL((gemm_nt_kernel<MT_, NTW_, true, BK_>), grid, block, 0, stream, a); \
                                    else hipLaunchKernelGGL((gemm_nt_kernel<MT_, NTW_, false, BK_>), grid, block, 0, stream, a); } while (0)
        if (resident) {
            const int st = gemm_resident_x3(a, stream);
            if (e1) (void)hipEventRecord(e1, stream);
            return st;
        }
        if (mt == 1) ICZ_NT(1, 1, 64);
        else if (mt == 2) ICZ_NT(2, 1, 64);
        else if (nt_stage_k(a) == 128 && nt_spread(a)) hipLaunchKernelGGL((gemm_nt_kernel<4, 1, false, 128, 4, true>), grid, block, 0, stream, a);
        else if (nt_stage_k(a) == 128) ICZ_NT(4, 1, 128);
        else ICZ_NT(4, 1, 64);
#undef ICZ_NT
        if (e1) (void)hipEventRecord(e1, stream);
    } else if (layout == GEMM_NN) {
        dim3 grid(cdiv(a.N, GEMM_BN), cdiv(a.M, GEMM_BM), a.nsplit);
        a.spread = 1;
        if (nn_x3(a)) {
            static bool attr = false;
            if (!attr) {
                ICZ_CHECK_HIP(hipFuncSetAttribute(reinterpret_cast<const void*>(gemm_tn128_x3_kernel<1, 4, true>), hipFuncAttributeMaxDynamicSharedMemorySize, (int)t3_lds(1)));
                ICZ_CHECK_HIP(hipFuncSetAttribute(reinterpret_cast<const void*>(gemm_tn128_x3_kernel<2, 8, true>), hipFuncAttributeMaxDynamicSharedMemorySize, (int)t3_lds(2)));
                attr = true;
            }
            const dim3 g128(cdiv(a.N, 128), cdiv(a.M, 128), a.nsplit);
            log_big_shape(layout, a);
            if (const int bc = gemm_big_cfg(layout, a)) return gemm_big_x3(layout, a, bc, stream);
            if ((int)(g128.x * g128.y * g128.z) > 256) hipLaunchKernelGGL((gemm_tn128_x3_kernel<1, 4, true>), g128, block, t3_lds(1), stream, a);
            else hipLaunchKernelGGL((gemm_tn128_x3_kernel<2, 8, true>), g128, dim3(512), t3_lds(2), stream, a);
        }
        else if (nn_stage_k(a) == 128) hipLaunchKernelGGL((gemm_nn_kernel<false, 128>), grid, block, 0, stream, a);
        else if (tail) hipLaunchKernelGGL(gemm_nn_kernel<true>, grid, block, 0, stream, a);
        else hipLaunchKernelGGL(gemm_nn_kernel<false>, grid, block, 0, stream, a);
    } else {
        if (a.nsplit == 1 && a.nseg == 1 && cdiv(a.M, 128) * cdiv(a.N, 128) >= 256 && a.seg[0].K % 32 == 0 && a.seg[0].K >= 64) {
            const bool x3 = gemm_switches().tn_x3;
            static bool attr = false;
            if (x3 && !attr) {
                ICZ_CHECK_HIP(hipFuncSetAttribute(reinterpret_cast<const void*>(gemm_tn128_x3_kernel<1, 4>), hipFuncAttributeMaxDynamicSharedMemorySize, (int)t3_lds(1)));
                ICZ_CHECK_HIP(hipFuncSetAttribute(reinterpret_cast<const void*>(gemm_tn128_x3_kernel<2, 8>), hipFuncAttributeMaxDynamicSharedMemorySize, (int)t3_lds(2)));
                attr = true;
            }
            const dim3 g128(cdiv(a.N, 128), cdiv(a.M, 128), 1);
            const int tiles = (int)(g128.x * g128.y);
            log_big_shape(layout, a);
            if (const int bc = x3 ? gemm_big_cfg(layout, a) : 0) return gemm_big_x3(layout, a, bc, stream);
            if (!x3) hipLaunchKernelGGL(gemm_tn128_kernel, g128, block, 0, stream, a);
            else if (tiles > 256) hipLaunchKernelGGL((gemm_tn128_x3_kernel<1, 4>), g128, block, t3_lds(1), stream, a);
            else hipLaunchKernelGGL((gemm_tn128_x3_kernel<2, 8>), g128, dim3(512), t3_lds(2), stream, a);
            ICZ_CHECK_HIP(hipGetLastError());
            return ICZ_OK;
        }
        dim3 grid(cdiv(a.N, GEMM_BN), cdiv(a.M, GEMM_BM), a.nsplit);
        if (tail) hipLaunchKernelGGL(gemm_tn_kernel<true>, grid, block, 0, stream, a);
        else hipLaunchKernelGGL(gemm_tn_kernel<false>, grid, block, 0, stream, a);
    }
    ICZ_CHECK_HIP(hipGetLastError());
    return ICZ_OK;
}

int gemm_route(GemmLayout layout, const GemmArgs& a_in) {
    GemmArgs a = a_in;
    const int tot = total_chunks(a, stage_k(layout, a));
    if (a.nsplit < 1 || a.nsplit > tot) return -1;
    a.chunks_per_split = cdiv(tot, a.nsplit);
    if (cdiv(tot, a.chunks_per_split) != a.nsplit) return -1;
    if (layout == GEMM_NT) {
        if (nt_x3big(a)) return gemm_big_cfg(layout, a) ? 7 : 6;
        if (gemm_resident_x3_fits(a) && a.nsplit == gemm_resident_x3_nsplit(a) && a.chunks_per_split == gemm_resident_x3_stages(a))
            return a.M > 64 ? 5 : (a.chunks_per_split == 8 ? 4 : 3);
        return a.M <= 16 ? 0 : (a.M <= 32 ? 1 : 2);
    }
    if (layout == GEMM_NN) {
        if (nn_x3(a)) return gemm_big_cfg(layout, a) ? 7 : 6;
        return 8;
    }
    if (a.nsplit == 1 && a.nseg == 1 && cdiv(a.M, 128) * cdiv(a.N, 128) >= 256 && a.seg[0].K % 32 == 0 && a.seg[0].K >= 64) {
        if (!gemm_switches().tn_x3) return 10;
        return gemm_big_cfg(layout, a) ? 7 : 6;
    }
    return 9;
}

bool gemm_prof_on() { return g_prof.on; }
void gemm_prof_select(int which) { g_prof.select = which; }
void gemm_prof_begin() {
    g_prof.on = true; g_prof.used = 0; g_prof.bytes = 0.0; g_prof.flops = 0.0; g_prof.seen = 0;
    while (g_prof.ev.size() < 8192) { hipEvent_t e; if (hipEventCreate(&e) != hipSuccess) break; g_prof.ev.push_back(e); }
    g_prof.every = gemm_switches().prof_every;
}
int gemm_prof_end(double* avg_us, double* bytes_per_launch, double* flops_per_launch, long long* launches) {
    g_prof.on = false;
    const size_t n = g_prof.used / 2;
    double tot_ms = 0.0;
    for (size_t i = 0; i < n; ++i) {
        ICZ_CHECK_HIP(hipEventSynchronize(g_prof.ev[2 * i + 1]));
        float ms = 0.f;
        ICZ_CHECK_HIP(hipEventElapsedTime(&ms, g_prof.ev[2 * i], g_prof.ev[2 * i + 1]));
        tot_ms += ms;
    }
    if (avg_us) *avg_us = n ? tot_ms * 1e3 / (double)n : 0.0;
    if (bytes_per_launch) *bytes_per_launch = n ? g_prof.bytes / (double)n : 0.0;
    if (flops_per_launch) *flops_per_launch = n ? g_prof.flops / (double)n : 0.0;
    if (launches) *launches = (long long)n;
    return ICZ_OK;
}

__global__ void prof_null_kernel(int* p) { if (p) *p = 0; }

int gemm_prof_pair_overhead(hipStream_t stream, int n, double* avg_us) {
    if (n < 1) n = 1;
    if (n > 256) n = 256;
    std::vector<hipEvent_t> ev(2 * n);
    for (auto& e : ev) ICZ_CHECK_HIP(hipEventCreate(&e));
    for (int i = 0; i < n; ++i) {
        hipLaunchKernelGGL(prof_null_kernel, dim3(256), dim3(256), 0, stream, (int*)nullptr);
        ICZ_CHECK_HIP(hipEventRecord(ev[2 * i], stream));
        hipLaunchKernelGGL(prof_null_kernel, dim3(1), dim3(1), 0, stream, (int*)nullptr);
        ICZ_CHECK_HIP(hipEventRecord(ev[2 * i + 1], stream));
    }
    double tot = 0.0;
    for (int i = 0; i < n; ++i) {
        ICZ_CHECK_HIP(hipEventSynchronize(ev[2 * i + 1]));
        float ms = 0.f;
        ICZ_CHECK_HIP(hipEventElapsedTime(&ms, ev[2 * i], ev[2 * i + 1]));
        tot += ms;
    }
    for (auto& e : ev) (void)hipEventDestroy(e);
    if (avg_us) *avg_us = tot * 1e3 / n;
    return ICZ_OK;
}

__global__ __launch_bounds__(256) void stream_rate_kernel(const f32x4* __restrict__ p, size_t nchunks, float* __restrict__ sink) {
    f32x4 acc = {0.f, 0.f, 0.f, 0.f};
    for (size_t c = blockIdx.x; c < nchunks; c += gridDim.x) {
        const f32x4* q = p + c * 4096 + threadIdx.x;
        f32x4 v[16];
#pragma unroll
        for (int i = 0; i < 16; ++i) v[i] = __builtin_nontemporal_load(q + i * 256);
#pragma unroll
        for (int i = 0; i < 16; ++i) acc += v[i];
    }
    if (acc.x + acc.y + acc.z + acc.w == 1.2345e-30f) sink[0] = acc.x;
}

}

extern "C" {
int icz_prof_stream_rate(const void* buf, size_t bytes, int32_t reps, void* stream, double* gbs) {
    ICZ_REQUIRE(buf && gbs && reps > 0 && bytes >= (size_t)65536 * 1024 && bytes % 65536 == 0, "icz_prof_stream_rate: bad arguments");
    hipStream_t st = (hipStream_t)stream;
    float* sink = nullptr;
    ICZ_CHECK_HIP(hipMalloc((void**)&sink, 16));
    hipEvent_t e0, e1;
    ICZ_CHECK_HIP(hipEventCreate(&e0));
    ICZ_CHECK_HIP(hipEventCreate(&e1));
    const size_t nchunks = bytes / 65536;
    const int grid = 256 * 8;
    for (int i = 0; i < 2; ++i) hipLaunchKernelGGL(icz::stream_rate_kernel, dim3(grid), dim3(256), 0, st, (const icz::f32x4*)buf, nchunks, sink);
    ICZ_CHECK_HIP(hipEventRecord(e0, st));
    for (int i = 0; i < reps; ++i) hipLaunchKernelGGL(icz::stream_rate_kernel, dim3(grid), dim3(256), 0, st, (const icz::f32x4*)buf, nchunks, sink);
    ICZ_CHECK_HIP(hipEventRecord(e1, st));
    ICZ_CHECK_HIP(hipEventSynchronize(e1));
    float ms = 0.f;
    ICZ_CHECK_HIP(hipEventElapsedTime(&ms, e0, e1));
    (void)hipEventDestroy(e0); (void)hipEventDestroy(e1); (void)hipFree(sink);
    *gbs = (double)bytes * reps / (ms * 1e-3) / 1e9;
    return ICZ_OK;
}
int icz_prof_pair_overhead(void* stream, int32_t n, double* avg_us) { return icz::gemm_prof_pair_overhead((hipStream_t)stream, n, avg_us); }
int icz_prof_begin(void) { icz::gemm_prof_begin(); return ICZ_OK; }
int icz_kprof_begin(void) {
    icz::g_kprof.on = true;
    for (size_t& u : icz::g_kprof.used) u = 0;
    return ICZ_OK;
}
int icz_kprof_end(int32_t group, double* avg_us, long long* pairs) {
    ICZ_REQUIRE(group >= 0 && group < icz::KP_GROUPS && avg_us && pairs, "icz_kprof_end: bad arguments");
    icz::g_kprof.on = false;
    ICZ_CHECK_HIP(hipDeviceSynchronize());
    const size_t n = icz::g_kprof.used[group] / 2;
    double tot = 0.0;
    for (size_t i = 0; i < n; ++i) {
        float ms = 0.f;
        ICZ_CHECK_HIP(hipEventElapsedTime(&ms, icz::g_kprof.ev[group][2 * i], icz::g_kprof.ev[group][2 * i + 1]));
        tot += ms;
    }
    *avg_us = n ? tot * 1e3 / (double)n : 0.0;
    *pairs = (long long)n;
    return ICZ_OK;
}
int icz_prof_select(int32_t which) {
    if (which < 0 || which > 1) { icz::set_error("icz_prof_select: %d (0 = all skinny forward GEMMs, 1 = resident-activation kernel)", which); return ICZ_ERR_INVALID; }
    icz::gemm_prof_select(which);
    return ICZ_OK;
}
int icz_prof_end(double* avg_us, double* bytes_per_launch, double* flops_per_launch, long long* launches) {
    return icz::gemm_prof_end(avg_us, bytes_per_launch, flops_per_launch, launches);
}

using namespace icz;
static constexpr int ABI_TARGET_WGS = 512;

size_t icz_gemm_workspace_floats(int32_t M, int32_t N) {
    const size_t base = (size_t)ABI_TARGET_WGS * 4096 * 2 + (size_t)M * N;
    const size_t m128 = (M > 64 && M <= 128) ? (size_t)32 * M * N : 0;
    return base > m128 ? base : m128;
}

int icz_gemm_f32(int32_t layout, const float* X, int32_t ldx, const float* W, int32_t ldw, const float* bias,
                 float* C, int32_t ldc, int32_t M, int32_t N, int32_t K, int32_t nsplit, float* workspace,
                 size_t workspace_floats, void* stream) {
    ICZ_REQUIRE(layout >= 0 && layout <= 2, "icz_gemm_f32: layout %d", layout);
    GemmArgs g = {};
    g.nseg = 1;
    g.seg[0] = {X, W, ldx, ldw, K, nullptr};
    g.M = M; g.N = N; g.out = C; g.ldo = ldc; g.bias = bias;
    g.nsplit = nsplit > 0 ? nsplit : gemm_fit_split((GemmLayout)layout, g, gemm_pick_split(g, ABI_TARGET_WGS, (GemmLayout)layout), workspace_floats);
    g.nsplit = gemm_normalize_split((GemmLayout)layout, g, g.nsplit);
    hipStream_t st = (hipStream_t)stream;
    if (g.nsplit > 1) {
        ICZ_REQUIRE(workspace, "icz_gemm_f32: split-K needs a workspace");
        ICZ_REQUIRE(gemm_slab_floats(M, N, g.nsplit) <= workspace_floats, "icz_gemm_f32: workspace of %zu floats too small for %d slabs of %dx%d", workspace_floats, g.nsplit, M, N);
        ICZ_REQUIRE(ldc == N, "icz_gemm_f32: split-K path needs ldc == N");
        g.out = workspace; g.bias = nullptr;
        ICZ_TRY(gemm_f32((GemmLayout)layout, g, st));
        size_t MN = (size_t)M * N;
        ICZ_REQUIRE(MN % 4 == 0, "icz_gemm_f32: M*N must be a multiple of 4 for the split-K reduce");
        hipLaunchKernelGGL(slab_reduce_kernel, dim3(cdiv((int)(MN / 4), 256)), dim3(256), 0, st, workspace, g.nsplit, MN, N, bias, C);
        ICZ_CHECK_HIP(hipGetLastError());
        return ICZ_OK;
    }
    return gemm_f32((GemmLayout)layout, g, st);
}

int icz_gemm_set_big_cfg(int32_t cfg) {
    ICZ_REQUIRE(cfg >= -2 && cfg <= 5, "icz_gemm_set_big_cfg: %d", cfg);
    gemm_set_big_cfg(cfg);
    return ICZ_OK;
}

int icz_gemm_big_cfg_for(int32_t layout, int32_t M, int32_t N, int32_t K, int32_t nsplit) {
    if (layout < 0 || layout > 2 || M <= 0 || N <= 0 || K <= 0) return -1;
    GemmArgs g = {};
    g.nseg = 1;
    g.seg[0].K = K;
    g.M = M; g.N = N; g.nsplit = nsplit > 0 ? nsplit : 1;
    return gemm_big_cfg((GemmLayout)layout, g);
}

int icz_gemm_tn_grouped_fits(int32_t M, int32_t K, int32_t ngroups, const int32_t* cols) {
    if (M <= 0 || K <= 0 || ngroups < 1 || ngroups > GEMM_MAX_COLGROUPS || !cols) return -1;
    GemmColGroup g[GEMM_MAX_COLGROUPS] = {};
    for (int j = 0; j < ngroups; ++j) g[j].cols = cols[j];
    return gemm_tn_grouped_fits(M, K, g, ngroups) ? 1 : 0;
}

int icz_gemm_route_for(int32_t layout, int32_t M, int32_t N, int32_t nseg, const int32_t* K, int32_t nsplit) {
    if (layout < 0 || layout > 2 || M <= 0 || N <= 0 || nseg < 1 || nseg > GEMM_MAX_SEG || !K || nsplit < 0) return -1;
    GemmArgs g = {};
    g.nseg = nseg;
    for (int s = 0; s < nseg; ++s) {
        if (K[s] <= 0) return -1;
        g.seg[s].K = K[s];
    }
    g.M = M; g.N = N;
    g.nsplit = nsplit > 0 ? nsplit : gemm_pick_split(g, 256, (GemmLayout)layout);
    return gemm_route((GemmLayout)layout, g);
}

int icz_gemm_tn_split_pick(int32_t M, int32_t N, int32_t K) {
    if (M <= 0 || N <= 0 || K <= 0) return -1;
    return gemm_tn_split_pick(M, N, K);
}

int icz_gemm_tn_split(const float* dY, int32_t ldy, int32_t M, const float* X, int32_t ldx, int32_t N, int32_t K, float* out, int32_t ldo,
                      float* workspace, size_t workspace_floats, const int32_t* rows_live, void* stream) {
    ICZ_REQUIRE(dY && X && out && M > 0 && N > 0 && K > 0 && ldy >= M && ldx >= N, "icz_gemm_tn_split: bad arguments");
    ICZ_REQUIRE(ldo == N, "icz_gemm_tn_split: the slab sum writes a dense output (ldo %d, N %d)", ldo, N);
    const int ns = gemm_tn_split_pick(M, N, K);
    ICZ_REQUIRE(ns > 1, "icz_gemm_tn_split: shape not taken (M %d N %d K %d): issue it through icz_gemm_f32", M, N, K);
    const size_t MN = (size_t)M * N;
    ICZ_REQUIRE(workspace && (size_t)ns * MN <= workspace_floats, "icz_gemm_tn_split: workspace of %zu floats too small for %d slabs of %d x %d", workspace_floats, ns, M, N);
    ICZ_REQUIRE(((uintptr_t)out & 15) == 0, "icz_gemm_tn_split: output must be 16-byte aligned");
    hipStream_t st = (hipStream_t)stream;
    ICZ_TRY(gemm_tn_split(dY, ldy, M, X, ldx, N, K, ns, workspace, rows_live, st));
    hipLaunchKernelGGL(slab_reduce_kernel, dim3(cdiv((int)(MN / 4), 256)), dim3(256), 0, st, (const float*)workspace, ns, MN, N, (const float*)nullptr, out);
    ICZ_CHECK_HIP(hipGetLastError());
    return ICZ_OK;
}

int icz_gemm_tn_grouped(const float* dY, int32_t ldy, int32_t M, int32_t K, int32_t ngroups, const float* const* X, const int32_t* ldx,
                        const int32_t* cols, float* const* out, const int32_t* ldo, const int32_t* rows_live, void* stream) {
    ICZ_REQUIRE(ngroups >= 1 && ngroups <= GEMM_MAX_COLGROUPS && X && ldx && cols && out && ldo, "icz_gemm_tn_grouped: bad arguments");
    GemmColGroup g[GEMM_MAX_COLGROUPS];
    for (int j = 0; j < ngroups; ++j) g[j] = {X[j], ldx[j], cols[j], out[j], ldo[j]};
    ICZ_REQUIRE(gemm_tn_grouped_fits(M, K, g, ngroups), "icz_gemm_tn_grouped: shape not taken (M %d, K %d)", M, K);
    return gemm_tn_grouped(dY, ldy, M, K, g, ngroups, rows_live, (hipStream_t)stream);
}
}
```

### simpleimagecaptionzoo_amd/csrc/icz_common.h

```cpp
#pragma once
#include <hip/hip_runtime.h>
#include <stdint.h>
#include <stdio.h>
#include <string.h>

#include "../../include/icz.h"

namespace icz {

void set_error(const char* fmt, ...);

#define ICZ_CHECK_HIP(expr)                                                                    \
    do {                                                                                       \
        hipError_t e_ = (expr);                                                                \
        if (e_ != hipSuccess) {                                                                \
            icz::set_error("%s:%d: %s -> %s", __FILE__, __LINE__, #expr, hipGetErrorString(e_)); \
            return ICZ_ERR_HIP;                                                                \
        }                                                                                      \
    } while (0)

#define ICZ_REQUIRE(cond, ...)                    \
    do {                                          \
        if (!(cond)) {                            \
            icz::set_error(__VA_ARGS__);          \
            return ICZ_ERR_INVALID;               \
        }                                         \
    } while (0)

#define ICZ_TRY(expr)                   \
    do {                                \
        int s_ = (expr);                \
        if (s_ != ICZ_OK) return s_;    \
    } while (0)

static inline int cdiv(int a, int b) { return (a + b - 1) / b; }
enum { KP_ATTENTION = 0, KP_GREEDY_SELECT = 1, KP_SAMPLE_SELECT = 2, KP_LSTM_POINT = 3, KP_GROUPS = 4 };
void kprof_mark(int group, bool begin, hipStream_t st);
static inline int pad_vocab(int V) { return (V + 63) & ~63; }

typedef float f32x4 __attribute__((ext_vector_type(4)));

__device__ __forceinline__ float wave_sum(float v) {
#pragma unroll
    for (int o = 32; o > 0; o >>= 1) v += __shfl_xor(v, o, 64);
    return v;
}
__device__ __forceinline__ float wave_max(float v) {
#pragma unroll
    for (int o = 32; o > 0; o >>= 1) v = fmaxf(v, __shfl_xor(v, o, 64));
    return v;
}
__device__ __forceinline__ double wave_sum_d(double v) {
#pragma unroll
    for (int o = 32; o > 0; o >>= 1) v += __shfl_xor(v, o, 64);
    return v;
}

__device__ __forceinline__ float sigmoidf_(float x) { return 1.0f / (1.0f + expf(-x)); }

__device__ __forceinline__ bool step_dead(const int* live) { return live != nullptr && *live == 0; }
__device__ __forceinline__ int live_flag(const int* live) { return live != nullptr ? *live : 1; }
__device__ __forceinline__ bool flag_dead(int flag) {
    asm volatile("" ::: "memory");
    return flag == 0;
}

}
```

Baseline: 11980.

## Add lean variants of per-step decode kernels with batched loads and narrow GEMM tiles

```diff
diff --git a/include/icz.h b/include/icz.h
--- a/include/icz.h
+++ b/include/icz.h
@@ -281,6 +281,7 @@
 int icz_gemm_tn_split(const float* dY, int32_t ldy, int32_t M, const float* X, int32_t ldx, int32_t N, int32_t K, float* out, int32_t ldo,
                       float* workspace, size_t workspace_floats, const int32_t* rows_live, void* stream);
 int icz_gemm_route_for(int32_t layout, int32_t M, int32_t N, int32_t nseg, const int32_t* K, int32_t nsplit);
+int icz_gemm_nt_narrow_fits(int32_t M, int32_t N, int32_t nseg, const int32_t* K, int32_t nsplit);
 int icz_gemm_tn_grouped_fits(int32_t M, int32_t K, int32_t ngroups, const int32_t* cols);
 int icz_prof_begin(void);
 int icz_prof_select(int32_t which);
diff --git a/simpleimagecaptionzoo_amd/_lib.py b/simpleimagecaptionzoo_amd/_lib.py
--- a/simpleimagecaptionzoo_amd/_lib.py
+++ b/simpleimagecaptionzoo_amd/_lib.py
@@ -218,6 +218,7 @@
         "icz_gemm_tn_split_pick": (C.c_int, [i32, i32, i32]),
         "icz_gemm_tn_split": (C.c_int, [vp, i32, i32, vp, i32, i32, i32, vp, i32, vp, C.c_size_t, vp, vp]),
         "icz_gemm_route_for": (C.c_int, [i32, i32, i32, i32, vp, i32]),
+        "icz_gemm_nt_narrow_fits": (C.c_int, [i32, i32, i32, vp, i32]),
         "icz_gemm_tn_grouped_fits": (C.c_int, [i32, i32, i32, vp]),
     }
     for name, (res, args) in sig.items():
diff --git a/simpleimagecaptionzoo_amd/csrc/butd.hip b/simpleimagecaptionzoo_amd/csrc/butd.hip
--- a/simpleimagecaptionzoo_amd/csrc/butd.hip
+++ b/simpleimagecaptionzoo_amd/csrc/butd.hip
@@ -119,7 +119,8 @@
     const int R = dims.R, D = dims.D, H = dims.H, E = dims.E, A = dims.A;
     ICZ_REQUIRE(fresh, "butd: call icz_butd_refresh_weights after binding/updating parameters");
     ICZ_REQUIRE(n_img > 0 && n_img <= dims.max_rows, "butd: %d images exceed capacity %d", n_img, dims.max_rows);
-    hipLaunchKernelGGL(mean_feats_kernel, dim3(cdiv(D, 1024), n_img), dim3(256), 0, st, feats, mean, R, D);
+    if (lean_step(LEAN_MEAN_FEATS)) hipLaunchKernelGGL(mean_feats_lean_kernel, dim3(cdiv(D, 256), n_img), dim3(64), 0, st, feats, mean, R, D ICZ_STAMPS_ARG(SS_MEAN_FEATS));
+    else hipLaunchKernelGGL(mean_feats_kernel, dim3(cdiv(D, 1024), n_img), dim3(256), 0, st, feats, mean, R, D ICZ_STAMPS_ARG(SS_MEAN_FEATS));
     {
         GemmArgs g = {};
         g.nseg = 1;
@@ -190,14 +191,21 @@
         ns = g.nsplit;
         ICZ_TRY(gemm_f32(GEMM_NT, g, st));
         AttScoreArgs a = {enc_ctx, s.img_of_row, ws, ns, P.dec_att_b, w_aff, P.affine_b, s.dec_ctx_out, scores, rows, R, A, s.live};
+#ifdef ICZ_DEV
+        a.stamps = step_stamps(SS_ATT_SCORES);
+#endif
         const int G = s.rows_per_img;
         const bool grouped = G > 1 && G <= ATT_CTX_MAX_G && rows % G == 0 && sizeof(float) * A * G <= 60 * 1024;
         if (grouped && s.drop_att.mode == 0 && !s.live)
             hipLaunchKernelGGL(att_scores_group_kernel, dim3(rows / G, ATT_PARTS), dim3(256), sizeof(float) * A * G, st, a, G);
         else if (grouped)
             hipLaunchKernelGGL(att_scores_group_train_kernel, dim3(rows / G, ATT_PARTS), dim3(256), sizeof(float) * A * G, st, a, s.drop_att, G);
+        else if (!lean_step(LEAN_ATT_SCORES))
+            hipLaunchKernelGGL((att_scores_kernel<true, false>), dim3(rows, ATT_PARTS), dim3(256), sizeof(float) * A, st, a, s.drop_att);
+        else if (s.drop_att.mode == 0)
+            hipLaunchKernelGGL((att_scores_kernel<false, true>), dim3(rows, ATT_PARTS), dim3(256), sizeof(float) * A, st, a, s.drop_att);
         else
-            hipLaunchKernelGGL(att_scores_kernel, dim3(rows, ATT_PARTS), dim3(256), sizeof(float) * A, st, a, s.drop_att);
+            hipLaunchKernelGGL((att_scores_kernel<true, true>), dim3(rows, ATT_PARTS), dim3(256), sizeof(float) * A, st, a, s.drop_att);
         if (G > 1 && G <= ATT_CTX_MAX_G && rows % G == 0 && !s.alpha_out2)
             hipLaunchKernelGGL(att_ctx_group_kernel, dim3(rows / G, cdiv(D, 512)), dim3(256), 0, st, s.feats, (const float*)scores,
                                s.alpha_out ? s.alpha_out : alpha, s.ctx_out ? s.ctx_out : ctx, R, D, G, s.live);
diff --git a/simpleimagecaptionzoo_amd/csrc/butd_kernels.h b/simpleimagecaptionzoo_amd/csrc/butd_kernels.h
--- a/simpleimagecaptionzoo_amd/csrc/butd_kernels.h
+++ b/simpleimagecaptionzoo_amd/csrc/butd_kernels.h
@@ -59,16 +59,44 @@
 }
 
 __global__ __launch_bounds__(256) void mean_feats_kernel(const float* __restrict__ feats, float* __restrict__ mean,
-                                                         int R, int D) {
+                                                         int R, int D ICZ_STAMPS_PARAM) {
     const int b = blockIdx.y;
     const int d = (blockIdx.x * 256 + threadIdx.x) * 4;
+    ICZ_STAMP(blockIdx.y * gridDim.x + blockIdx.x, 0);
     if (d >= D) return;
     const float* f = feats + (size_t)b * R * D + d;
     f32x4 s = {0.f, 0.f, 0.f, 0.f};
     for (int r = 0; r < R; ++r) s += *reinterpret_cast<const f32x4*>(f + (size_t)r * D);
+    ICZ_STAMP(blockIdx.y * gridDim.x + blockIdx.x, 3);
     const float fr = (float)R;
     f32x4 o = {s[0] / fr, s[1] / fr, s[2] / fr, s[3] / fr};
     *reinterpret_cast<f32x4*>(mean + (size_t)b * D + d) = o;
+    ICZ_STAMP(blockIdx.y * gridDim.x + blockIdx.x, 4);
+}
+
+constexpr int MEAN_RB = 36;
+__global__ __launch_bounds__(64) void mean_feats_lean_kernel(const float* __restrict__ feats, float* __restrict__ mean, int R, int D ICZ_STAMPS_PARAM) {
+    const int b = blockIdx.y;
+    const int d = (blockIdx.x * 64 + threadIdx.x) * 4;
+    ICZ_STAMP(blockIdx.y * gridDim.x + blockIdx.x, 0);
+    if (d >= D) return;
+    const float* f = feats + (size_t)b * R * D + d;
+    f32x4 s = {0.f, 0.f, 0.f, 0.f};
+    for (int r0 = 0; r0 < R; r0 += MEAN_RB) {
+        f32x4 x[MEAN_RB];
+#pragma unroll
+        for (int u = 0; u < MEAN_RB; ++u) x[u] = __builtin_nontemporal_load(reinterpret_cast<const f32x4*>(f + (size_t)min(r0 + u, R - 1) * D));
+        __builtin_amdgcn_sched_barrier(0);
+        if (r0 == 0) ICZ_STAMP(blockIdx.y * gridDim.x + blockIdx.x, 1);
+#pragma unroll
+        for (int u = 0; u < MEAN_RB; ++u)
+            if (r0 + u < R) s += x[u];
+    }
+    ICZ_STAMP(blockIdx.y * gridDim.x + blockIdx.x, 3);
+    const float fr = (float)R;
+    f32x4 o = {s[0] / fr, s[1] / fr, s[2] / fr, s[3] / fr};
+    *reinterpret_cast<f32x4*>(mean + (size_t)b * D + d) = o;
+    ICZ_STAMP(blockIdx.y * gridDim.x + blockIdx.x, 4);
 }
 
 __global__ __launch_bounds__(256) void slab_reduce_kernel(const float* __restrict__ slab, int nsplit, size_t MN, int N,
@@ -260,9 +288,33 @@
     float* scores;
     int rows, R, A;
     const int* live;
+#ifdef ICZ_DEV
+    unsigned long long* stamps;
+#endif
 };
+template <int N>
+__device__ __forceinline__ void slab_batch4(f32x4& s, const float* p, size_t stride, int& z) {
+    f32x4 v[N];
+#pragma unroll
+    for (int i = 0; i < N; ++i) v[i] = *reinterpret_cast<const f32x4*>(p + (size_t)(z + i) * stride);
+    __builtin_amdgcn_sched_barrier(0);
+    s = z == 0 ? v[0] : s + v[0];
+#pragma unroll
+    for (int i = 1; i < N; ++i) s += v[i];
+    z += N;
+}
+__device__ __forceinline__ float mul_then_add(float acc, float a, float b) {
+#pragma clang fp contract(off)
+    const float p = a * b;
+    return acc + p;
+}
+template <bool DROP, bool LEAN>
 __global__ __launch_bounds__(256) void att_scores_kernel(AttScoreArgs a, DropCfg dc) {
     extern __shared__ __attribute__((aligned(16))) float sdec[];
+#ifdef ICZ_DEV
+    unsigned long long* const stamps_ = a.stamps;
+#endif
+    ICZ_STAMP(blockIdx.y * gridDim.x + blockIdx.x, 0);
     const int lflag = live_flag(a.live);
     const int row = blockIdx.x, part = blockIdx.y, nparts = gridDim.y;
     const int tid = threadIdx.x, lane = tid & 63, wave = tid >> 6;
@@ -279,21 +331,41 @@
             for (int u = 0; u < 4; ++u) xf[b][u] = *reinterpret_cast<const f32x4*>(e + min(lane * 4 + 256 * u, a.A - 4));
         }
     }
+    f32x4 wf[4];
+    float baff = 0.f;
+    if (LEAN) {
+#pragma unroll
+        for (int u = 0; u < 4; ++u) wf[u] = *reinterpret_cast<const f32x4*>(a.w_aff + min(lane * 4 + 256 * u, a.A - 4));
+        baff = a.b_aff[0];
+    }
     if (flag_dead(lflag)) return;
+    ICZ_STAMP(blockIdx.y * gridDim.x + blockIdx.x, 1);
     for (int c = tid * 4; c < a.A; c += 1024) {
         const size_t off = (size_t)row * a.A + c;
-        f32x4 s = *reinterpret_cast<const f32x4*>(a.dec_slab + off);
-        for (int z = 1; z < a.nsplit; ++z) s += *reinterpret_cast<const f32x4*>(a.dec_slab + (size_t)z * MN + off);
-        s += *reinterpret_cast<const f32x4*>(a.b_dec + c);
+        f32x4 s = {0.f, 0.f, 0.f, 0.f};
+        if (LEAN) {
+            const f32x4 bd = *reinterpret_cast<const f32x4*>(a.b_dec + c);
+            int z = 0;
+            while (z + 8 <= a.nsplit) slab_batch4<8>(s, a.dec_slab + off, MN, z);
+            if (z + 4 <= a.nsplit) slab_batch4<4>(s, a.dec_slab + off, MN, z);
+            if (z + 2 <= a.nsplit) slab_batch4<2>(s, a.dec_slab + off, MN, z);
+            if (z < a.nsplit) slab_batch4<1>(s, a.dec_slab + off, MN, z);
+            s += bd;
+        } else {
+            s = *reinterpret_cast<const f32x4*>(a.dec_slab + off);
+            for (int z = 1; z < a.nsplit; ++z) s += *reinterpret_cast<const f32x4*>(a.dec_slab + (size_t)z * MN + off);
+            s += *reinterpret_cast<const f32x4*>(a.b_dec + c);
+        }
         *reinterpret_cast<f32x4*>(sdec + c) = s;
         if (a.dec_ctx_out && part == 0) *reinterpret_cast<f32x4*>(a.dec_ctx_out + off) = s;
     }
     __syncthreads();
-    const float baff = a.b_aff[0];
+    ICZ_STAMP(blockIdx.y * gridDim.x + blockIdx.x, 2);
+    if (!LEAN) baff = a.b_aff[0];
     const int drow = row - dc.row0;
-    if (drow < 0) dc.mode = 0;
+    if (!DROP || drow < 0) dc.mode = 0;
     const float sc = dc.mode ? 2.0f : 1.0f;
-    const bool shared_bits = dc.mode == 2 && (a.A & 255) == 0;
+    const bool shared_bits = DROP && dc.mode == 2 && (a.A & 255) == 0;
     for (int i0 = wave; part + nparts * i0 < a.R; i0 += 4 * NB) {
         int rr[NB];
         bool ok[NB];
@@ -320,8 +392,8 @@
 #pragma unroll
                     for (int u = 0; u < 4; ++u) x[b][u] = *reinterpret_cast<const f32x4*>(e[b] + min(c0 + 256 * u, a.A - 4));
             }
-            uint32_t kq[NB][4];
-            if (shared_bits) {
+            uint32_t kq[DROP ? NB : 1][4];
+            if (DROP && shared_bits) {
                 const int pb = lane >> 3, pg = lane & 7;
                 const int pr = pb == 0 ? rr[0] : (pb == 1 ? rr[1] : rr[NB - 1]);
                 const uint64_t g = (((uint64_t)drow * a.R + pr) * a.A + (c0 - lane * 4) + 128 * pg) >> 7;
@@ -344,26 +416,33 @@
                 const int c = c0 + 256 * u;
                 if (c < a.A) {
                     const f32x4 d = *reinterpret_cast<const f32x4*>(sdec + c);
-                    const f32x4 w = *reinterpret_cast<const f32x4*>(a.w_aff + c);
+                    const f32x4 w = (LEAN && i0 == wave && c0 == lane * 4) ? wf[u] : *reinterpret_cast<const f32x4*>(a.w_aff + c);
 #pragma unroll
                     for (int b = 0; b < NB; ++b) {
-                        const uint32_t k = shared_bits ? kq[b][u] : (dc.mode ? dc.keep4(((uint64_t)drow * a.R + rr[b]) * a.A + c) : 0xFu);
-#pragma unroll
-                        for (int j = 0; j < 4; ++j) {
-                            float zv = fmaxf(x[b][u][j] + d[j], 0.f);
-                            zv = ((k >> j) & 1u) ? zv * sc : 0.f;
-                            acc[b] += zv * w[j];
+                        if (DROP) {
+                            const uint32_t k = shared_bits ? kq[b][u] : (dc.mode ? dc.keep4(((uint64_t)drow * a.R + rr[b]) * a.A + c) : 0xFu);
+#pragma unroll
+                            for (int j = 0; j < 4; ++j) {
+                                float zv = fmaxf(x[b][u][j] + d[j], 0.f);
+                                zv = ((k >> j) & 1u) ? zv * sc : 0.f;
+                                acc[b] += zv * w[j];
+                            }
+                        } else {
+#pragma unroll
+                            for (int j = 0; j < 4; ++j) acc[b] = mul_then_add(acc[b], fmaxf(x[b][u][j] + d[j], 0.f), w[j]);
                         }
                     }
                 }
             }
         }
+        if (i0 == wave) ICZ_STAMP(blockIdx.y * gridDim.x + blockIdx.x, 3);
 #pragma unroll
         for (int b = 0; b < NB; ++b) {
             const float v = wave_sum(acc[b]);
             if (lane == 0 && ok[b]) a.scores[(size_t)row * a.R + rr[b]] = v + baff;
         }
     }
+    ICZ_STAMP(blockIdx.y * gridDim.x + blockIdx.x, 4);
 }
 
 constexpr int ATT_CTX_MAX_G = 8;
@@ -668,14 +747,54 @@
     *reinterpret_cast<f32x4*>(emb + (size_t)row * E + e) = x;
 }
 
+constexpr int SEL_IT = 3, SEL_NS = 4;
+__device__ __forceinline__ bool sel_strip_fits(bool vec, int ns, int Vv) { return vec && ns <= SEL_NS && Vv > 0 && Vv <= SEL_IT * 4096; }
+__device__ __forceinline__ f32x4 ld_nt4(const float* p) { return __builtin_nontemporal_load(reinterpret_cast<const f32x4*>(p)); }
+__device__ __forceinline__ void sel_strip_load(f32x4 (&x)[SEL_IT][SEL_NS], f32x4 (&b)[SEL_IT], float (&tx)[SEL_NS], float& tb,
+                                               const float* l, int ns, size_t slab_stride, const float* bias, int Vv, int V, int tid) {
+#pragma unroll
+    for (int i = 0; i < SEL_IT; ++i) {
+        const int v = tid * 4 + 4096 * i, vc = v < Vv ? v : 0;
+#pragma unroll
+        for (int z = 0; z < SEL_NS; ++z)
+            if (z < ns) x[i][z] = ld_nt4(l + (size_t)z * slab_stride + vc);
+        if (bias) b[i] = *reinterpret_cast<const f32x4*>(bias + vc);
+    }
+    const int tv = Vv + tid < V ? Vv + tid : 0;
+#pragma unroll
+    for (int z = 0; z < SEL_NS; ++z)
+        if (z < ns) tx[z] = __builtin_nontemporal_load(l + (size_t)z * slab_stride + tv);
+    if (bias) tb = bias[tv];
+    __builtin_amdgcn_sched_barrier(0);
+}
+__device__ __forceinline__ f32x4 sel_strip_sum4(const f32x4 (&x)[SEL_NS], const f32x4& b, int ns, bool has_bias) {
+    f32x4 s = x[0];
+#pragma unroll
+    for (int z = 1; z < SEL_NS; ++z)
+        if (z < ns) s += x[z];
+    if (has_bias) s += b;
+    return s;
+}
+__device__ __forceinline__ float sel_strip_sum1(const float (&x)[SEL_NS], float b, int ns, bool has_bias) {
+    float s = x[0];
+#pragma unroll
+    for (int z = 1; z < SEL_NS; ++z)
+        if (z < ns) s += x[z];
+    if (has_bias) s += b;
+    return s;
+}
+
+template <bool LEAN>
 __global__ __launch_bounds__(1024) void greedy_select_kernel(const float* __restrict__ logits, int V, int ldl, int ns, size_t slab_stride,
                                                             const float* __restrict__ bias, const float* __restrict__ table, int E,
                                                             float* __restrict__ emb, int64_t* __restrict__ it_next,
                                                             int64_t* __restrict__ ids_out, int ids_stride, int t, int relu = 1,
-                                                            uint8_t* __restrict__ unfinished = nullptr, int* __restrict__ n_unfinished = nullptr) {
+                                                            uint8_t* __restrict__ unfinished = nullptr, int* __restrict__ n_unfinished = nullptr
+                                                            ICZ_STAMPS_PARAM) {
     __shared__ float sv[16];
     __shared__ int si[16];
     const int row = blockIdx.x, tid = threadIdx.x, lane = tid & 63, wave = tid >> 6;
+    ICZ_STAMP(blockIdx.x, 0);
     if (n_unfinished && t > 0 && n_unfinished[t - 1] == 0) {
         if (tid == 0 && ids_out) ids_out[(size_t)row * ids_stride + t] = 0;
         return;
@@ -685,24 +804,47 @@
     int bi = 0x7fffffff;
     const bool vec = ((ldl | (int)(slab_stride & 3)) & 3) == 0 && (((uintptr_t)logits | (uintptr_t)bias) & 15) == 0;
     const int Vv = vec ? (V & ~3) : 0;
-    for (int v = tid * 4; v < Vv; v += 4096) {
-        f32x4 x = *reinterpret_cast<const f32x4*>(l + v);
-        for (int z = 1; z < ns; ++z) x += *reinterpret_cast<const f32x4*>(l + (size_t)z * slab_stride + v);
-        if (bias) x += *reinterpret_cast<const f32x4*>(bias + v);
-#pragma unroll
-        for (int j = 0; j < 4; ++j)
-            if (x[j] > best) { best = x[j]; bi = v + j; }
-    }
-    for (int v = Vv + tid; v < V; v += 1024) {
-        float x = l[v];
-        for (int z = 1; z < ns; ++z) x += l[(size_t)z * slab_stride + v];
-        if (bias) x += bias[v];
-        if (x > best || (x == best && v < bi)) { best = x; bi = v; }
-    }
+    if (LEAN && sel_strip_fits(vec, ns, Vv)) {
+        f32x4 xs[SEL_IT][SEL_NS], bs[SEL_IT];
+        float tx[SEL_NS], tb = 0.f;
+        sel_strip_load(xs, bs, tx, tb, l, ns, slab_stride, bias, Vv, V, tid);
+#pragma unroll
+        for (int i = 0; i < SEL_IT; ++i) {
+            const int v = tid * 4 + 4096 * i;
+            if (v < Vv) {
+                const f32x4 x = sel_strip_sum4(xs[i], bs[i], ns, bias != nullptr);
+#pragma unroll
+                for (int j = 0; j < 4; ++j)
+                    if (x[j] > best) { best = x[j]; bi = v + j; }
+            }
+        }
+        if (Vv + tid < V) {
+            const int v = Vv + tid;
+            const float x = sel_strip_sum1(tx, tb, ns, bias != nullptr);
+            if (x > best || (x == best && v < bi)) { best = x; bi = v; }
+        }
+    } else {
+        for (int v = tid * 4; v < Vv; v += 4096) {
+            f32x4 x = *reinterpret_cast<const f32x4*>(l + v);
+            for (int z = 1; z < ns; ++z) x += *reinterpret_cast<const f32x4*>(l + (size_t)z * slab_stride + v);
+            if (bias) x += *reinterpret_cast<const f32x4*>(bias + v);
+#pragma unroll
+            for (int j = 0; j < 4; ++j)
+                if (x[j] > best) { best = x[j]; bi = v + j; }
+        }
+        for (int v = Vv + tid; v < V; v += 1024) {
+            float x = l[v];
+            for (int z = 1; z < ns; ++z) x += l[(size_t)z * slab_stride + v];
+            if (bias) x += bias[v];
+            if (x > best || (x == best && v < bi)) { best = x; bi = v; }
+        }
+    }
+    ICZ_STAMP(blockIdx.x, 1);
 #pragma unroll
     for (int o = 32; o > 0; o >>= 1) argmax_combine(best, bi, __shfl_xor(best, o, 64), __shfl_xor(bi, o, 64));
     if (lane == 0) { sv[wave] = best; si[wave] = bi; }
     __syncthreads();
+    ICZ_STAMP(blockIdx.x, 2);
     best = sv[0]; bi = si[0];
 #pragma unroll
     for (int w = 1; w < 16; ++w) argmax_combine(best, bi, sv[w], si[w]);
@@ -716,12 +858,14 @@
             if (unf) atomicAdd(&n_unfinished[t], 1);
         }
     }
+    ICZ_STAMP(blockIdx.x, 3);
     for (int e = tid * 4; e < E; e += 4096) {
         f32x4 x = *reinterpret_cast<const f32x4*>(table + (size_t)bi * E + e);
 #pragma unroll
         for (int j = 0; j < 4; ++j) x[j] = relu ? fmaxf(x[j], 0.f) : x[j];
         *reinterpret_cast<f32x4*>(emb + (size_t)row * E + e) = x;
     }
+    ICZ_STAMP(blockIdx.x, 4);
 }
 
 __global__ void set_scalars_kernel(uint64_t* seed_p, uint64_t seed, float* f_p, float f) {
@@ -845,6 +989,9 @@
     int ns; size_t slab_stride; const float* bias; float* logits_store;
     int* live_rows;
     int row0; int64_t* ids_out; uint8_t* g_unfinished; int* n_any;
+#ifdef ICZ_DEV
+    unsigned long long* stamps;
+#endif
 };
 constexpr int SEL_THREADS = 1024;
 __device__ __forceinline__ float block_max_n(float v, float* sm, int nw) {
@@ -955,7 +1102,7 @@
     hipLaunchKernelGGL(ss_select_kernel, dim3(rows), dim3(SEL_THREADS), sizeof(float) * V, st, sa);
     return ICZ_OK;
 }
-template <bool MG>
+template <bool MG, bool LEAN>
 __global__ __launch_bounds__(SEL_THREADS) void sample_select_kernel(SampleSelArgs a) {
     extern __shared__ __attribute__((aligned(16))) float srow[];
     __shared__ float smf[16];
@@ -963,6 +1110,10 @@
     __shared__ int smi[16];
     constexpr int NW = SEL_THREADS / 64;
     const int row = blockIdx.x, tid = threadIdx.x, lane = tid & 63, wave = tid >> 6;
+#ifdef ICZ_DEV
+    unsigned long long* const stamps_ = a.stamps;
+#endif
+    ICZ_STAMP(blockIdx.x, 0);
     const int sr = MG ? row - a.row0 : row;
     const bool greedy_row = MG && sr < 0;
     const float sc = a.emb_drop.mode ? 2.0f : 1.0f;
@@ -995,24 +1146,48 @@
         const bool vec = ((a.ldl | (int)(a.slab_stride & 3)) & 3) == 0 &&
                          (((uintptr_t)a.logits | (uintptr_t)a.bias | (uintptr_t)a.logits_store) & 15) == 0;
         const int Vv = vec ? (a.V & ~3) : 0;
-        for (int v = tid * 4; v < Vv; v += 4 * SEL_THREADS) {
-            f32x4 x = *reinterpret_cast<const f32x4*>(l + v);
-            for (int z = 1; z < a.ns; ++z) x += *reinterpret_cast<const f32x4*>(l + (size_t)z * a.slab_stride + v);
-            x += *reinterpret_cast<const f32x4*>(a.bias + v);
-            *reinterpret_cast<f32x4*>(ls + v) = x;
-            *reinterpret_cast<f32x4*>(srow + v) = x;
-            mx = fmaxf(mx, fmaxf(fmaxf(x[0], x[1]), fmaxf(x[2], x[3])));
-        }
-        for (int v = Vv + tid; v < a.V; v += SEL_THREADS) {
-            float x = l[v];
-            for (int z = 1; z < a.ns; ++z) x += l[(size_t)z * a.slab_stride + v];
-            x += a.bias[v];
-            ls[v] = x; srow[v] = x; mx = fmaxf(mx, x);
+        if (LEAN && sel_strip_fits(vec, a.ns, Vv)) {
+            static_assert(SEL_THREADS * 4 == 4096, "sel_strip_load strides a row by 4096 columns");
+            f32x4 xs[SEL_IT][SEL_NS], bs[SEL_IT];
+            float tx[SEL_NS], tb = 0.f;
+            sel_strip_load(xs, bs, tx, tb, l, a.ns, a.slab_stride, a.bias, Vv, a.V, tid);
+#pragma unroll
+            for (int i = 0; i < SEL_IT; ++i) {
+                const int v = tid * 4 + 4 * SEL_THREADS * i;
+                if (v < Vv) {
+                    const f32x4 x = sel_strip_sum4(xs[i], bs[i], a.ns, true);
+                    __builtin_nontemporal_store(x, reinterpret_cast<f32x4*>(ls + v));
+                    *reinterpret_cast<f32x4*>(srow + v) = x;
+                    mx = fmaxf(mx, fmaxf(fmaxf(x[0], x[1]), fmaxf(x[2], x[3])));
+                }
+            }
+            if (Vv + tid < a.V) {
+                const int v = Vv + tid;
+                const float x = sel_strip_sum1(tx, tb, a.ns, true);
+                ls[v] = x; srow[v] = x; mx = fmaxf(mx, x);
+            }
+        } else {
+            for (int v = tid * 4; v < Vv; v += 4 * SEL_THREADS) {
+                f32x4 x = *reinterpret_cast<const f32x4*>(l + v);
+                for (int z = 1; z < a.ns; ++z) x += *reinterpret_cast<const f32x4*>(l + (size_t)z * a.slab_stride + v);
+                x += *reinterpret_cast<const f32x4*>(a.bias + v);
+                *reinterpret_cast<f32x4*>(ls + v) = x;
+                *reinterpret_cast<f32x4*>(srow + v) = x;
+                mx = fmaxf(mx, fmaxf(fmaxf(x[0], x[1]), fmaxf(x[2], x[3])));
+            }
+            for (int v = Vv + tid; v < a.V; v += SEL_THREADS) {
+                float x = l[v];
+                for (int z = 1; z < a.ns; ++z) x += l[(size_t)z * a.slab_stride + v];
+                x += a.bias[v];
+                ls[v] = x; srow[v] = x; mx = fmaxf(mx, x);
+            }
         }
     } else {
         for (int v = tid; v < a.V; v += SEL_THREADS) { const float x = l[v]; srow[v] = x; mx = fmaxf(mx, x); }
     }
+    ICZ_STAMP(blockIdx.x, 1);
     mx = block_max_n(mx, smf, NW);
+    ICZ_STAMP(blockIdx.x, 2);
     if (greedy_row) {
         const int per = (a.V + SEL_THREADS - 1) / SEL_THREADS;
         const int v0 = min(a.V, tid * per), v1 = min(a.V, v0 + per);
@@ -1106,6 +1281,7 @@
             }
         }
     }
+    ICZ_STAMP(blockIdx.x, 3);
     if (a.emb_next)
         for (int e = tid * 4; e < a.E; e += 4 * SEL_THREADS) {
             f32x4 x = *reinterpret_cast<const f32x4*>(a.emb_table + (size_t)tok * a.E + e);
@@ -1114,10 +1290,22 @@
             for (int j = 0; j < 4; ++j) x[j] = ((k >> j) & 1u) ? fmaxf(x[j], 0.f) * sc : 0.f;
             *reinterpret_cast<f32x4*>(a.emb_next + (size_t)row * a.E + e) = x;
         }
-}
-inline void launch_sample_select(hipStream_t st, int rows, const SampleSelArgs& a) {
-    if (a.row0 > 0) hipLaunchKernelGGL(sample_select_kernel<true>, dim3(rows), dim3(SEL_THREADS), sizeof(float) * a.V, st, a);
-    else hipLaunchKernelGGL(sample_select_kernel<false>, dim3(rows), dim3(SEL_THREADS), sizeof(float) * a.V, st, a);
+    ICZ_STAMP(blockIdx.x, 4);
+}
+inline void launch_sample_select(hipStream_t st, int rows, const SampleSelArgs& a_in) {
+    SampleSelArgs a = a_in;
+#ifdef ICZ_DEV
+    a.stamps = step_stamps(SS_SAMPLE_SELECT);
+#endif
+    const dim3 grid(rows), block(SEL_THREADS);
+    const size_t lds = sizeof(float) * a.V;
+    if (lean_step(LEAN_SELECT)) {
+        if (a.row0 > 0) hipLaunchKernelGGL((sample_select_kernel<true, true>), grid, block, lds, st, a);
+        else hipLaunchKernelGGL((sample_select_kernel<false, true>), grid, block, lds, st, a);
+    } else {
+        if (a.row0 > 0) hipLaunchKernelGGL((sample_select_kernel<true, false>), grid, block, lds, st, a);
+        else hipLaunchKernelGGL((sample_select_kernel<false, false>), grid, block, lds, st, a);
+    }
 }
 
 __global__ __launch_bounds__(256) void reinforce_loss_kernel(const float* __restrict__ logp, const int64_t* __restrict__ seq,
diff --git a/simpleimagecaptionzoo_amd/csrc/decoder_core.hip b/simpleimagecaptionzoo_amd/csrc/decoder_core.hip
--- a/simpleimagecaptionzoo_amd/csrc/decoder_core.hip
+++ b/simpleimagecaptionzoo_amd/csrc/decoder_core.hip
@@ -154,11 +154,39 @@
     return ICZ_OK;
 }
 
+bool lean_step(int part) {
+    static const int mask = [] {
+        const char* e = getenv("ICZ_LEAN_STEP");
+        int m = (e ? atoi(e) != 0 : true) ? ~0 : 0;
+#ifdef ICZ_DEV
+        if (const char* p = getenv("ICZ_DEV_LEAN_PARTS")) m &= atoi(p);
+#endif
+        return m;
+    }();
+    return (mask & part) != 0;
+}
+
+#ifdef ICZ_DEV
+static unsigned long long* g_step_stamps = nullptr;
+unsigned long long* step_stamps(int kernel) {
+    static const bool on = [] { const char* e = getenv("ICZ_DEV_STAMPS"); return e && atoi(e) != 0; }();
+    if (!on) return nullptr;
+    if (!g_step_stamps) {
+        const size_t bytes = sizeof(unsigned long long) * SS_KERNELS * SS_MAX_WGS * SS_SLOTS;
+        if (hipMalloc((void**)&g_step_stamps, bytes) != hipSuccess || hipMemset(g_step_stamps, 0, bytes) != hipSuccess) return nullptr;
+    }
+    return g_step_stamps + (size_t)kernel * SS_MAX_WGS * SS_SLOTS;
+}
+#endif
+
 void launch_greedy_select(const LogitsView& lv, const DecodeMember::EmbSlot& e, int rows, int V, float* amax_val, int* amax_idx, int64_t* it,
                           int64_t* ids_out, int T, int t, uint8_t* gunf, int* gn, hipStream_t st) {
-    if (lv.ns > 1)
-        hipLaunchKernelGGL(greedy_select_kernel, dim3(rows), dim3(1024), 0, st, lv.p, V, lv.ld, lv.ns, lv.slab_stride, lv.bias, e.table, e.E, e.emb,
-                           it, ids_out, T, t, e.relu, gunf, gn);
+    if (lv.ns > 1 && lean_step(LEAN_SELECT))
+        hipLaunchKernelGGL(greedy_select_kernel<true>, dim3(rows), dim3(1024), 0, st, lv.p, V, lv.ld, lv.ns, lv.slab_stride, lv.bias, e.table, e.E,
+                           e.emb, it, ids_out, T, t, e.relu, gunf, gn ICZ_STAMPS_ARG(SS_GREEDY_SELECT));
+    else if (lv.ns > 1)
+        hipLaunchKernelGGL(greedy_select_kernel<false>, dim3(rows), dim3(1024), 0, st, lv.p, V, lv.ld, lv.ns, lv.slab_stride, lv.bias, e.table, e.E,
+                           e.emb, it, ids_out, T, t, e.relu, gunf, gn ICZ_STAMPS_ARG(SS_GREEDY_SELECT));
     else {
         hipLaunchKernelGGL(argmax_part_kernel, dim3(rows, ARGMAX_PARTS), dim3(256), 0, st, lv.p, V, lv.ld, ARGMAX_PARTS, amax_val, amax_idx);
         hipLaunchKernelGGL(embed_argmax_kernel, dim3(cdiv(e.E, 1024), rows), dim3(256), 0, st, (const float*)amax_val, (const int*)amax_idx,
@@ -190,6 +218,14 @@
 
 }
 
+#ifdef ICZ_DEV
+extern "C" int icz_debug_step_stamps(unsigned long long* out_host, int kernel, int n_workgroups) {
+    if (!icz::g_step_stamps || kernel < 0 || kernel >= icz::SS_KERNELS || n_workgroups > icz::SS_MAX_WGS) return -1;
+    const unsigned long long* src = icz::g_step_stamps + (size_t)kernel * icz::SS_MAX_WGS * icz::SS_SLOTS;
+    return hipMemcpy(out_host, src, sizeof(unsigned long long) * icz::SS_SLOTS * n_workgroups, hipMemcpyDeviceToHost) == hipSuccess ? 0 : -2;
+}
+#endif
+
 extern "C" {
 const char* icz_last_error(void) { return icz::g_err; }
 const char* icz_version(void) { return "libicz 0.1 (gfx950)"; }
diff --git a/simpleimagecaptionzoo_amd/csrc/gemm_f32.h b/simpleimagecaptionzoo_amd/csrc/gemm_f32.h
--- a/simpleimagecaptionzoo_amd/csrc/gemm_f32.h
+++ b/simpleimagecaptionzoo_amd/csrc/gemm_f32.h
@@ -33,6 +33,7 @@
 
 int gemm_f32(GemmLayout layout, const GemmArgs& a, hipStream_t stream);
 int gemm_route(GemmLayout layout, const GemmArgs& a);
+bool gemm_nt_narrow_fits(const GemmArgs& a);
 int gemm_pick_split(const GemmArgs& a, int target_wgs, GemmLayout layout = GEMM_NT);
 int gemm_pick_split_balanced(const GemmArgs& a, GemmLayout layout, size_t slab_capacity_floats);
 size_t gemm_slab_floats(int M, int N, int nsplit);
diff --git a/simpleimagecaptionzoo_amd/csrc/gemm_f32.hip b/simpleimagecaptionzoo_amd/csrc/gemm_f32.hip
--- a/simpleimagecaptionzoo_amd/csrc/gemm_f32.hip
+++ b/simpleimagecaptionzoo_amd/csrc/gemm_f32.hip
@@ -870,6 +870,12 @@
     return tiles * (tot / per > 0 ? tot / per : 1) >= 128;
 }
 static int nt_tile_n(const GemmArgs& a) { return 64; }
+bool gemm_nt_narrow_fits(const GemmArgs& a) {
+    if (!lean_step(LEAN_DEC_ATT) || a.M <= 32 || a.M > 64 || a.nseg != 1 || a.seg[0].K % 128 || a.nsplit < 4) return false;
+    if (nt_x3big(a) || gemm_resident_x3_fits(a)) return false;
+    const int wide = cdiv(a.N, 64) * a.nsplit, narrow = cdiv(a.N, 32) * a.nsplit;
+    return wide >= 64 && narrow <= 256;
+}
 
 int gemm_pick_split(const GemmArgs& a, int target_wgs, GemmLayout layout) {
     if (layout == GEMM_NT && gemm_resident_x3_fits(a)) return gemm_resident_x3_nsplit(a);
@@ -1027,6 +1033,8 @@
         }
         if (mt == 1) ICZ_NT(1, 1, 64);
         else if (mt == 2) ICZ_NT(2, 1, 64);
+        else if (gemm_nt_narrow_fits(a))
+            hipLaunchKernelGGL((gemm_nt_kernel<4, 1, false, 128, 2, true>), dim3(cdiv(a.N, 32), grid.y, grid.z), dim3(128), 0, stream, a);
         else if (nt_stage_k(a) == 128 && nt_spread(a)) hipLaunchKernelGGL((gemm_nt_kernel<4, 1, false, 128, 4, true>), grid, block, 0, stream, a);
         else if (nt_stage_k(a) == 128) ICZ_NT(4, 1, 128);
         else ICZ_NT(4, 1, 64);
@@ -1288,6 +1296,20 @@
     return gemm_route((GemmLayout)layout, g);
 }
 
+int icz_gemm_nt_narrow_fits(int32_t M, int32_t N, int32_t nseg, const int32_t* K, int32_t nsplit) {
+    if (M <= 0 || N <= 0 || nseg < 1 || nseg > GEMM_MAX_SEG || !K || nsplit < 0) return -1;
+    GemmArgs g = {};
+    g.nseg = nseg;
+    for (int s = 0; s < nseg; ++s) {
+        if (K[s] <= 0) return -1;
+        g.seg[s].K = K[s];
+    }
+    g.M = M; g.N = N;
+    g.nsplit = nsplit > 0 ? nsplit : gemm_pick_split(g, 256, GEMM_NT);
+    if (gemm_route(GEMM_NT, g) != 2) return 0;
+    return gemm_nt_narrow_fits(g) ? 1 : 0;
+}
+
 int icz_gemm_tn_split_pick(int32_t M, int32_t N, int32_t K) {
     if (M <= 0 || N <= 0 || K <= 0) return -1;
     return gemm_tn_split_pick(M, N, K);
diff --git a/simpleimagecaptionzoo_amd/csrc/icz_common.h b/simpleimagecaptionzoo_amd/csrc/icz_common.h
--- a/simpleimagecaptionzoo_amd/csrc/icz_common.h
+++ b/simpleimagecaptionzoo_amd/csrc/icz_common.h
@@ -34,11 +34,32 @@
     } while (0)
 
 static inline int cdiv(int a, int b) { return (a + b - 1) / b; }
+enum { LEAN_ATT_SCORES = 1, LEAN_DEC_ATT = 2, LEAN_SELECT = 4, LEAN_MEAN_FEATS = 8 };
+bool lean_step(int part);
 enum { KP_ATTENTION = 0, KP_GREEDY_SELECT = 1, KP_SAMPLE_SELECT = 2, KP_LSTM_POINT = 3, KP_GROUPS = 4 };
 void kprof_mark(int group, bool begin, hipStream_t st);
 static inline int pad_vocab(int V) { return (V + 63) & ~63; }
 
 typedef float f32x4 __attribute__((ext_vector_type(4)));
+
+#ifdef ICZ_DEV
+enum { SS_ATT_SCORES = 0, SS_GREEDY_SELECT = 1, SS_SAMPLE_SELECT = 2, SS_MEAN_FEATS = 3, SS_KERNELS = 4 };
+constexpr int SS_SLOTS = 8, SS_MAX_WGS = 1024;
+unsigned long long* step_stamps(int kernel);
+#define ICZ_STAMPS_PARAM , unsigned long long* stamps_ = nullptr
+#define ICZ_STAMPS_ARG(k) , step_stamps(k)
+#define ICZ_STAMP(wg, i)                                                                                                  \
+    do {                                                                                                                  \
+        __builtin_amdgcn_sched_barrier(0);                                                                                \
+        const unsigned long long t_ = __builtin_amdgcn_s_memtime();                                                       \
+        if (stamps_ && threadIdx.x == 0 && (int)(wg) < SS_MAX_WGS) stamps_[(size_t)(wg) * SS_SLOTS + (i)] = t_;           \
+        __builtin_amdgcn_sched_barrier(0);                                                                                \
+    } while (0)
+#else
+#define ICZ_STAMPS_PARAM
+#define ICZ_STAMPS_ARG(k)
+#define ICZ_STAMP(wg, i) do { } while (0)
+#endif
 
 __device__ __forceinline__ float wave_sum(float v) {
 #pragma unroll
```

Measured after the change: 12040, median of 6. No clear change (+0.6%).
